# jkulhanek/viewformer

Hardware: AMD Instinct MI355X
Metric: novel views/sec (encode->AR transformer->decode), 128px 6-ctx (higher is better)
Workload: dtype bf16

## Files before the change

include/vf_hip.h:

```cpp
#ifndef VF_HIP_H
#define VF_HIP_H

#include <stddef.h>
#include <stdint.h>

#ifdef __cplusplus
extern "C" {
#endif

#define VF_OK 0
#define VF_ERR_BAD_ARG (-1)
#define VF_ERR_UNSUPPORTED (-2)

int vf_abi_version(void);
size_t vf_sizeof_igemm_args(void);
size_t vf_sizeof_pack_desc(void);
const char* vf_build_arch(void);
int vf_build_flags(void);
const char* vf_build_flag_name(int i);
enum { VF_SEL_ATTN_DMA = 0,
       VF_SEL_GEMM_G256 = 1,
       VF_SEL_LN_BWD_TWO_ROWS = 2,
       VF_SEL_ATTN_Q32 = 3,
       VF_SEL_CONV_X3H_K32 = 4,
       VF_SEL_GEMM_TAIL = 5,
       VF_SEL_COUNT = 6 };
int vf_select(int which, int value);
int vf_selected(int which);

enum { VF_MODE_GEMM = 0, VF_MODE_CONV3_S1 = 1, VF_MODE_CONV3_S2PAD = 2, VF_MODE_CONV3_UP2 = 3 };
enum { VF_EPI_NONE = 0, VF_EPI_GELU_ERF = 1,
       VF_EPI_GELU_BWD = 2,
       VF_EPI_GELU_DUAL = 3 };

typedef struct vf_igemm_args {
    const float* x;
    const float* w_packed;
    const float* bias;
    const float* res;
    float* out;
    const float* pro_mean;
    const float* pro_scale;
    const float* pro_beta;
    int32_t pro_swish;
    int32_t pro_rows_per_img;
    int32_t mode;
    int32_t epilogue;
    int32_t M;
    int32_t Cin, Cout;
    int32_t Hin, Win, Hout, Wout;
    int32_t lda, ldc, ldr;
    int32_t batch;
    int64_t stride_x, stride_w, stride_out, stride_res;
    float* gn_part;
    int32_t gn_slots;
    int32_t reserved0;
    void* out_aux;
    float drop_rate;
    uint32_t drop_seed, drop_site;
    int32_t drop_row0;
} vf_igemm_args;

size_t vf_igemm_packed_floats(int K, int N, int taps);
int vf_igemm_pack_f32(const float* src, float* dst, int K, int N, int taps,
                      int64_t sk, int64_t sn, int64_t st, int batch, int64_t src_bstride, void* stream);
int vf_igemm_f32(const vf_igemm_args* args , void* stream);

int vf_conv_in_u8_f32(const uint8_t* img_u8, const float* img_f32, const float* w_oihw, const float* bias,
                      float* out, int n_img, int H, int W, int Cout, void* stream);
size_t vf_conv_in_x3h_packed_elems(int Cout);
int vf_conv_in_x3h_pack(const float* w_oihw, void* dst, int Cout, void* stream);
int vf_conv_in_x3h(const uint8_t* img_u8, const float* img_f32, const void* w_packed, const float* bias, float* out, float* gn_part,
                   int gn_slots, int n_img, int H, int W, int Cout, void* stream);

int vf_conv3_small_cout_f32(const float* x, const float* w_oihw, const float* bias, const float* pro_mean,
                            const float* pro_scale, const float* pro_beta, int pro_swish, float* out, int n_img, int H, int W,
                            int Cin, int Cout, int x_bf16, void* stream);

size_t vf_groupnorm_workspace_bytes(int n_img, int HW, int C);
int vf_groupnorm_stats_f32(const float* x, const float* gamma, int n_img, int HW, int C, int groups, float eps,
                           float* mean_c, float* scale_c, void* ws, void* stream);
int vf_groupnorm_finalize_f32(const float* part, const float* gamma, int n_img, int HW, int C, int groups, int nslots,
                              float eps, float* mean_c, float* scale_c, void* stream);
int vf_groupnorm_apply_f32(const float* x, const float* mean_c, const float* scale_c, const float* beta,
                           float* out, int n_img, int HW, int C, int swish, void* stream);

size_t vf_vq_packed_floats(int D, int Kc);
int vf_vq_pack_codebook_f32(const float* E , float* dst, int D, int Kc, void* stream);
int vf_colsumsq_f32(const float* E , float* e_sq , int D, int Kc, void* stream);
int vf_vq_argmin_f32(const float* z, const float* E_packed, const float* e_sq, int64_t M, int D, int Kc,
                     int64_t* idx, void* stream);
size_t vf_vq_filter_packed_bytes(int D, int Kc);
int vf_vq_filter_pack(const float* E , void* dst, int D, int Kc, void* stream);
int vf_vq_argmin_filtered_f32(const float* z, const void* packed, int64_t M, int D, int Kc, int64_t* idx, uint32_t* stats4,
                              void* stream);
int vf_codebook_gather_f32(const float* E , const int64_t* idx, float* out ,
                           int64_t M, int D, int Kc, void* stream);

int vf_attn_blockcausal_f32(const float* q, const float* k, const float* v, float* out,
                            int B, int H, int T, int L, int ldq, int ldk, int ldv, int ldo,
                            float scale, int skip_masked, int twin_view, void* stream);
int vf_attn_blockcausal_bf16_v2(const void* q, const void* k, const void* v, int in_bf16, void* out, int out_bf16, int B, int H, int T, int L,
                                int ldq, int ldk, int ldv, int ldo, float scale, int skip_masked, int twin_view, void* stream);
int vf_attn_blockcausal_fp8(const void* q, const void* k, const void* v, int in_bf16, void* out, int out_bf16, int B, int H, int T, int L,
                            int ldq, int ldk, int ldv, int ldo, float scale, int skip_masked, int twin_view, void* stream);
int vf_attn_blockcausal_x6(const float* q, const float* k, const float* v, float* out,
                           int B, int H, int T, int L, int ldq, int ldk, int ldv, int ldo,
                           float scale, int skip_masked, int twin_view, void* stream);
int vf_attn_prefix_bf16(const void* q, const void* k, const void* v, const void* kp, const void* vp, int in_bf16, void* out, int out_bf16,
                        int B, int H, int C, int N, int L, int dh, int ldq, int ldk, int ldv, int ldkp, int ldvp, int64_t prefix_stride,
                        int ldo, void* stream);
int vf_attn_prefix_f32eq(const float* q, const float* k, const float* v, const float* kp, const float* vp, float* out,
                         int B, int H, int C, int N, int L, int dh, int ldq, int ldk, int ldv, int ldkp, int ldvp, int64_t prefix_stride,
                         int ldo, void* stream);
int vf_attn_spatial_f32(const float* qkv, float* out, int n_img, int HW, int C, int64_t ld, int64_t ldo, float scale, void* stream);
int vf_attn_spatial_x3h(const float* qkv, float* out, int n_img, int HW, int C, int64_t ld, int64_t ldo, float scale, void* stream);
int vf_softmax_rows_f32(float* x, int64_t rows, int n, float scale, void* stream);

int vf_layernorm_f32(const float* x, const float* gamma, const float* beta, float* out,
                     int64_t rows, int d, float eps, void* stream);
int vf_layernorm_bf16out_f32(const float* x, const float* gamma, const float* beta, void* out_bf16, int64_t rows, int d, float eps,
                             void* stream);
int vf_embed_sum_f32(const int32_t* ids, const float* wte, const float* wpe, const float* add,
                     float* out, int64_t BS, int L, int d, int vocab, void* stream);
int vf_dense_small_k_gelu_f32(const float* x, const float* W, const float* b, float* out,
                              int64_t rows, int K, int N, int gelu, void* stream);
int vf_argmax_rows_f32(const float* x, int64_t rows, int n, int ld, int64_t* idx, void* stream);
int vf_lmhead_argmax_bf16(const void* h, int h_bf16, int64_t ldh, const void* w_packed, int64_t M, int K, int N, int64_t* idx,
                          float* max_logit, void* stream);
int vf_lmhead_score_bf16(const void* h, int h_bf16, int64_t ldh, const void* w_packed, int64_t M, int K, int N, const int32_t* target,
                         int64_t* idx, float* max_logit, float* lse, float* target_logit, float* entropy, void* stream);
int vf_logits_score_f32(const float* logits, int64_t rows, int N, int64_t ld, const int32_t* target, int64_t* idx, float* max_logit,
                        float* lse, float* target_logit, float* entropy, void* stream);
int vf_score_views_f32(const float* target_logit, const float* lse, const float* max_logit, const int64_t* idx, const int32_t* target,
                       int64_t views, int L, float* token_log_prob, float* confidence, float* log_likelihood, float* accuracy, void* stream);
int vf_sample_rows_f32(const float* logits, int64_t rows, int N, int64_t ld, float temperature, int top_k, float top_p, uint32_t seed,
                       const int64_t* row_id, int S, int64_t* idx, float* logp, int32_t* kept, float* thr, void* stream);
int vf_sample_views_f32(const float* logp, int64_t views, int L, int S, float* log_likelihood, void* stream);
uint32_t vf_crc32c(const void* data, size_t n, uint32_t crc);
int vf_postprocess_u8(const float* x, uint8_t* out, int64_t n, void* stream);
int vf_resize_u8(const uint8_t* src, uint8_t* dst, int n_img, int Hin, int Win, int Hout, int Wout, int C, int bilinear, void* stream);
size_t vf_image_metrics_workspace_bytes(int n_img, int H, int W, int C);
int vf_image_metrics_u8(const uint8_t* a, const uint8_t* b, int n_img, int H, int W, int C, int64_t* sums, double* ssim, void* workspace,
                        void* stream);
size_t vf_camera_knn_workspace_bytes(int64_t N, int Q, int k);
int vf_camera_knn_f32(const float* db, int64_t N, const float* queries, int Q, int k, float pos_weight, int32_t* idx, float* dist,
                      void* workspace, void* stream);
int vf_pose_tail_f32(const float* x, int64_t ldx, const float* W, const float* b, float position_multiplier, int64_t views, int L, int K,
                     float* raw, float* tokens, float* cameras, void* stream);

size_t vf_gemm_bf16_packed_elems(int K, int N);
int vf_gemm_bf16_pack(const float* src, void* dst, int K, int N, int64_t sk, int64_t sn, int batch,
                      int64_t src_bstride, void* stream);
typedef struct vf_pack_desc {
    const float* src;
    void* dst;
    int32_t K, N;
    int64_t sk, sn;
} vf_pack_desc;
int vf_gemm_bf16_pack_multi(const vf_pack_desc* descs_device, int n, void* stream);
int vf_gemm_bf16(const vf_igemm_args* args , void* stream);
size_t vf_conv3_bf16_packed_elems(int Cin, int Cout);
int vf_conv3_bf16_pack(const float* w_oihw, void* dst, int Cin, int Cout, void* stream);
int vf_conv3_halo_bf16(const vf_igemm_args* args , void* stream);

int vf_conv3_halo_gn_slots(int Hout, int Wout);
size_t vf_conv3_x6_packed_elems(int Cin, int Cout);
int vf_conv3_x6_pack(const float* w_oihw, void* dst, int Cin, int Cout, void* stream);
int vf_conv3_halo_x6(const vf_igemm_args* args , void* stream);
size_t vf_conv3_x3h_packed_elems(int Cin, int Cout);
int vf_conv3_x3h_pack(const float* w_oihw, void* dst, int Cin, int Cout, void* stream);
int vf_conv3_halo_x3h(const vf_igemm_args* args , void* stream);
size_t vf_gemm_x3h_packed_elems(int K, int N);
int vf_gemm_x3h_pack(const float* src, void* dst, int K, int N, int64_t sk, int64_t sn, void* stream);
int vf_gemm_x3h(const vf_igemm_args* args , void* stream);
size_t vf_gemm_x6_packed_elems(int K, int N);
int vf_gemm_x6_pack(const float* src, void* dst, int K, int N, int64_t sk, int64_t sn, void* stream);
int vf_gemm_x6(const vf_igemm_args* args , void* stream);
int vf_sum_slabs_f32(const float* slabs, int nslabs, int64_t stride, int64_t n, float* dst, int accumulate, void* stream);

int vf_vq_ema_accumulate_f32(const float* z, const int64_t* idx, int64_t M, int D, int Kc, float* counts, float* embed_sum,
                             void* stream);
int vf_vq_ema_update_f32(const float* counts, const float* embed_sum, float* cluster_size_hidden, float* dw_hidden,
                         float* embeddings, int D, int Kc, float decay, float eps, float corr, void* stream);

int vf_gather_transpose_f32(const float* src, float* dst, int n_img, int Hin, int Win, int C, int Hout, int Wout, int stride, int oy,
                            int ox, int64_t ld_dst, void* stream);
size_t vf_conv3_wgrad_x6_rows(int Cin);
int vf_conv3_wgrad_x6(const float* x, const void* dy_packed, float* slabs, int n_img, int Hin, int Win, int Cin, int Hout, int Wout,
                      int Cout, int mode, int splits, void* stream);
int vf_upsample2_bwd_f32(const float* du, float* dx, int n_img, int H, int W, int C, void* stream);
size_t vf_groupnorm_bwd_workspace_bytes(int n_img, int HW, int C, int groups);
int vf_groupnorm_bwd_f32(const float* x, const float* da, const float* mean_c, const float* scale_c, const float* gamma,
                         const float* beta, float* dx, float* chan_sums, int n_img, int HW, int C, int groups, float eps, int swish,
                         int accumulate, void* ws, void* stream);
int vf_softmax_rows_bwd_f32(const float* p, float* dp, int64_t rows, int n, float scale, void* stream);
int vf_l1_loss_partials(int64_t n);
int vf_l1_loss_f32(const float* x, const float* y, float* dy, float* part, int64_t n, float grad_weight, void* stream);

int vf_lpips_scaling_f32(const float* x, float* y, int64_t npix, const float* shift3, const float* scale3, int backward, void* stream);
int vf_relu_f32(float* x, int64_t n, void* stream);
int vf_relu_bwd_f32(float* dy, const float* y, int64_t n, void* stream);
int vf_maxpool2_f32(const float* x, float* y, int n_img, int Hout, int Wout, int C, void* stream);
int vf_maxpool2_bwd_f32(const float* x, const float* dy, float* dx, int n_img, int Hout, int Wout, int C, void* stream);
int vf_lpips_head_blocks(int HW);
int vf_lpips_head_f32(const float* f0, const float* f1, const float* w, float* part, int n_img, int HW, int C, void* stream);
int vf_lpips_head_bwd_f32(const float* f0, const float* f1, const float* w, float* df1, int64_t npix, int C, float gscale,
                          int accumulate, void* stream);

int vf_attn_blockcausal_lse_f32(const float* q, const float* k, const float* v, float* out, float* lse,
                                int B, int H, int T, int L, int ldq, int ldk, int ldv, int ldo,
                                float scale, int skip_masked, int twin_view, float drop_rate, uint32_t drop_seed,
                                uint32_t drop_site, uint32_t drop_plane0, void* stream);
int vf_attn_bwd_prep_f32(const float* dout, const float* out, float* D, int B, int H, int T, int lddo, int ldo, void* stream);
int vf_attn_bwd_f32(const float* q, const float* k, const float* v, const float* dout, const float* lse, const float* D,
                    float* dq, float* dk, float* dv, int B, int H, int T, int L, int ldq, int ldk, int ldv, int lddo,
                    int lddq, int lddk, int lddv, float scale, int twin_view, float drop_rate, uint32_t drop_seed,
                    uint32_t drop_site, uint32_t drop_plane0, void* stream);
int vf_gemm_tn_bf16(const void* x_bf16, int ldx, const void* dy, int dy_is_bf16, int ldy, int M, int K, int N, int splits, float* w_slabs,
                    float* b_slabs, int64_t slab_stride, void* stream);
int vf_attn_blockcausal_bf16_lse(const void* q, const void* k, const void* v, void* out, float* lse, int B, int H, int T, int L,
                                 int ldq, int ldk, int ldv, int ldo, float scale, int twin_view, float drop_rate, uint32_t drop_seed,
                                 uint32_t drop_site, uint32_t drop_plane0, void* stream);
int vf_attn_bwd_prep_bf16(const void* dout, const void* out, float* D, int B, int H, int T, int lddo, int ldo, void* stream);
int vf_attn_bwd_bf16(const void* q, const void* k, const void* v, const void* dout, const float* lse, const float* D, void* dq, void* dk,
                     void* dv, int out_bf16 , int B, int H, int T, int L,
                     int ldq, int ldk, int ldv, int lddo, int lddq, int lddk, int lddv, float scale, int twin_view, float drop_rate,
                     uint32_t drop_seed, uint32_t drop_site, uint32_t drop_plane0, void* stream);
int vf_dropout_add_f32(const float* x, const float* res, float* out, int64_t rows, int cols, int64_t row0, float rate, uint32_t seed, uint32_t site,
                       void* stream);

int vf_transpose_f32(const float* src, float* dst, int rows, int cols, int64_t ld_src, int64_t ld_dst, int batch,
                     int64_t bs_src, int64_t bs_dst, void* stream);
int vf_transpose_bf16_f32(const void* src_bf16, float* dst, int rows, int cols, int64_t ld_src, int64_t ld_dst, int batch,
                          int64_t bs_src, int64_t bs_dst, void* stream);
size_t vf_colsum_workspace_bytes(int N);
int vf_colsum_f32(const float* x, float* out, int64_t M, int N, int64_t ld, int accumulate, void* ws, void* stream);
size_t vf_layernorm_bwd_workspace_bytes(int64_t rows, int d);
int vf_layernorm_bwd_f32(const float* dy, const float* x, const float* gamma, float* dx, float* dgamma, float* dbeta,
                         int64_t rows, int d, float eps, int accumulate, const float* res ,
                         void* dx_bf16 ,
                         float drop_rate, uint32_t drop_seed, uint32_t drop_site, int64_t drop_row0 , void* ws, void* stream);
int vf_gelu_f32(const float* u, float* f, int64_t n, void* stream);
int vf_gelu_bf16out_f32(const float* u, void* f_bf16, int64_t n, void* stream);
int vf_gelu_bwd_f32(const float* u, const float* df, float* du, int64_t n, void* stream);
int vf_gelu_bwd_bf16out_f32(const float* u, const float* df, void* du_bf16, int64_t n, void* stream);
int vf_softmax_mask_f32(float* s, int64_t batch, int T, int L, int mask_spec, float scale, void* stream);
int vf_softmax_mask_bwd_f32(const float* p, float* dp, int64_t batch, int T, int L, int mask_spec, float scale, void* stream);
int vf_softmax_ce_f32(const float* logits, const int32_t* target, const float* row_weight, float* loss, float* dlogits,
                      int64_t rows, int V, float label_smoothing, void* stream);
int vf_pose_mse_f32(const float* raw, const float* gt, const float* w_pos, const float* w_ori, const float* xyz_div, float* pos_loss,
                    float* ori_loss, float* draw, int64_t rows, int L, float position_multiplier, void* stream);
size_t vf_embed_bwd_workspace_bytes(int d, int vocab);
int vf_embed_bwd_f32(const float* dh, const int32_t* ids, float* dwte, float* dwpe, float* dadd, int64_t BS, int L, int d,
                     int vocab, void* workspace, void* stream);
int vf_dense_small_k_bwd_f32(const float* x, const float* dy, float* dW, float* db, int64_t rows, int K, int N, void* stream);
int vf_dense_small_n_f32(const float* x, const float* W, const float* b, float* out, int64_t rows, int K, int N, int64_t ldx, void* stream);
int vf_dense_small_n_wgrad_slabs(int64_t rows);
int vf_dense_small_n_wgrad_f32(const float* x, const float* dy, float* dW, float* ws, int64_t rows, int K, int N, int64_t ldx, int accumulate,
                               void* stream);
int vf_adamw_f32(float* param, const float* grad, float* m, float* v, int64_t n, float lr_decay, float lr_adam, float beta1,
                 float beta2, float eps, void* stream);
int vf_adamw_flat_f32(float* param, const float* grad, float* m, float* v, int64_t n, const int64_t* nodecay_ranges, int nranges,
                      float lr_decay, float lr_adam, float beta1, float beta2, float eps, void* stream);
typedef struct vf_adamw_pack_desc {
    int64_t offset;
    void* dst_kn;
    void* dst_nk;
    int32_t rows, cols;
    int32_t nodecay;
    int32_t reserved;
} vf_adamw_pack_desc;
size_t vf_sizeof_adamw_pack_desc(void);
int vf_adamw_pack_check(const vf_adamw_pack_desc* descs_host, int ndesc, int64_t n);
int vf_adamw_flat_pack_f32(float* param, const float* grad, float* m, float* v, int64_t n, const int64_t* nodecay_ranges, int nranges,
                           float lr_decay, float lr_adam, float beta1, float beta2, float eps, const vf_adamw_pack_desc* descs_device, int ndesc,
                           void* stream);
int vf_add_inplace_f32(float* a, const float* b, int64_t n, void* stream);
int vf_axpby_f32(float a, const float* x, float b, const float* y, float* out, int64_t n, void* stream);
int vf_clip_scratch_floats(void);
int vf_clip_by_norm_f32(float* x, int64_t n, float clip, float* scratch, void* stream);
int vf_clip_grad_norm_f32(float* x, int64_t n, float max_norm, float* scratch, void* stream);

#ifdef __cplusplus
}
#endif
#endif
```

viewformer_amd/_lib.py:

```python
import ctypes
import os
from ctypes import c_int, c_int32, c_int64, c_float, c_void_p, c_size_t, c_char_p, POINTER

HERE = os.path.dirname(os.path.abspath(__file__))
LIB_PATH = os.environ.get('VF_HIP_LIB') or os.path.join(HERE, 'libvf_hip.so')


class VfIgemmArgs(ctypes.Structure):
    _fields_ = [
        ('x', c_void_p), ('w_packed', c_void_p), ('bias', c_void_p), ('res', c_void_p), ('out', c_void_p),
        ('pro_mean', c_void_p), ('pro_scale', c_void_p), ('pro_beta', c_void_p),
        ('pro_swish', c_int32), ('pro_rows_per_img', c_int32), ('mode', c_int32), ('epilogue', c_int32),
        ('M', c_int32), ('Cin', c_int32), ('Cout', c_int32),
        ('Hin', c_int32), ('Win', c_int32), ('Hout', c_int32), ('Wout', c_int32),
        ('lda', c_int32), ('ldc', c_int32), ('ldr', c_int32), ('batch', c_int32),
        ('stride_x', c_int64), ('stride_w', c_int64), ('stride_out', c_int64), ('stride_res', c_int64),
        ('gn_part', c_void_p), ('gn_slots', c_int32), ('reserved0', c_int32),
        ('out_aux', c_void_p),
        ('drop_rate', c_float), ('drop_seed', ctypes.c_uint32), ('drop_site', ctypes.c_uint32), ('drop_row0', c_int32),
    ]


SEL_ATTN_DMA, SEL_GEMM_G256, SEL_LN_BWD_TWO_ROWS, SEL_ATTN_Q32 = 0, 1, 2, 3
SEL_CONV_X3H_K32 = 4
SEL_GEMM_TAIL = 5
_ENV_SELECT = {'VF_ATTN_DMA': SEL_ATTN_DMA, 'VF_GEMM_G256': SEL_GEMM_G256, 'VF_LN_BWD_TWO_ROWS': SEL_LN_BWD_TWO_ROWS, 'VF_ATTN_Q32': SEL_ATTN_Q32,
               'VF_CONV_X3H_K32': SEL_CONV_X3H_K32, 'VF_GEMM_TAIL': SEL_GEMM_TAIL}

ADAMW_PACK_DESC_BYTES = 40
PACK_DESC_BYTES = 40
P = c_void_p
EXPORTS = {
    'vf_abi_version': (c_int, []),
    'vf_sizeof_igemm_args': (c_size_t, []),
    'vf_sizeof_pack_desc': (c_size_t, []),
    'vf_build_arch': (c_char_p, []),
    'vf_build_flags': (c_int, []),
    'vf_build_flag_name': (c_char_p, [c_int]),
    'vf_select': (c_int, [c_int, c_int]),
    'vf_selected': (c_int, [c_int]),
    'vf_igemm_packed_floats': (c_size_t, [c_int, c_int, c_int]),
    'vf_igemm_pack_f32': (c_int, [P, P, c_int, c_int, c_int, c_int64, c_int64, c_int64, c_int, c_int64, P]),
    'vf_igemm_f32': (c_int, [POINTER(VfIgemmArgs), P]),
    'vf_conv_in_u8_f32': (c_int, [P, P, P, P, P, c_int, c_int, c_int, c_int, P]),
    'vf_conv_in_x3h_packed_elems': (c_size_t, [c_int]),
    'vf_conv_in_x3h_pack': (c_int, [P, P, c_int, P]),
    'vf_conv_in_x3h': (c_int, [P, P, P, P, P, P, c_int, c_int, c_int, c_int, c_int, P]),
    'vf_crc32c': (ctypes.c_uint32, [P, c_size_t, ctypes.c_uint32]),
    'vf_conv3_small_cout_f32': (c_int, [P, P, P, P, P, P, c_int, P, c_int, c_int, c_int, c_int, c_int, c_int, P]),
    'vf_groupnorm_workspace_bytes': (c_size_t, [c_int, c_int, c_int]),
    'vf_groupnorm_stats_f32': (c_int, [P, P, c_int, c_int, c_int, c_int, c_float, P, P, P, P]),
    'vf_groupnorm_finalize_f32': (c_int, [P, P, c_int, c_int, c_int, c_int, c_int, c_float, P, P, P]),
    'vf_conv3_halo_gn_slots': (c_int, [c_int, c_int]),
    'vf_groupnorm_apply_f32': (c_int, [P, P, P, P, P, c_int, c_int, c_int, c_int, P]),
    'vf_vq_packed_floats': (c_size_t, [c_int, c_int]),
    'vf_vq_pack_codebook_f32': (c_int, [P, P, c_int, c_int, P]),
    'vf_colsumsq_f32': (c_int, [P, P, c_int, c_int, P]),
    'vf_vq_argmin_f32': (c_int, [P, P, P, c_int64, c_int, c_int, P, P]),
    'vf_vq_filter_packed_bytes': (c_size_t, [c_int, c_int]),
    'vf_vq_filter_pack': (c_int, [P, P, c_int, c_int, P]),
    'vf_vq_argmin_filtered_f32': (c_int, [P, P, c_int64, c_int, c_int, P, P, P]),
    'vf_gather_transpose_f32': (c_int, [P, P, c_int, c_int, c_int, c_int, c_int, c_int, c_int, c_int, c_int, c_int64, P]),
    'vf_upsample2_bwd_f32': (c_int, [P, P, c_int, c_int, c_int, c_int, P]),
    'vf_groupnorm_bwd_workspace_bytes': (c_size_t, [c_int, c_int, c_int, c_int]),
    'vf_groupnorm_bwd_f32': (c_int, [P, P, P, P, P, P, P, P, c_int, c_int, c_int, c_int, c_float, c_int, c_int, P, P]),
    'vf_softmax_rows_bwd_f32': (c_int, [P, P, c_int64, c_int, c_float, P]),
    'vf_l1_loss_partials': (c_int, [c_int64]),
    'vf_l1_loss_f32': (c_int, [P, P, P, P, c_int64, c_float, P]),
    'vf_conv3_wgrad_x6_rows': (c_size_t, [c_int]),
    'vf_conv3_wgrad_x6': (c_int, [P, P, P, c_int, c_int, c_int, c_int, c_int, c_int, c_int, c_int, c_int, P]),
    'vf_lpips_scaling_f32': (c_int, [P, P, c_int64, P, P, c_int, P]),
    'vf_relu_f32': (c_int, [P, c_int64, P]),
    'vf_relu_bwd_f32': (c_int, [P, P, c_int64, P]),
    'vf_maxpool2_f32': (c_int, [P, P, c_int, c_int, c_int, c_int, P]),
    'vf_maxpool2_bwd_f32': (c_int, [P, P, P, c_int, c_int, c_int, c_int, P]),
    'vf_lpips_head_blocks': (c_int, [c_int]),
    'vf_lpips_head_f32': (c_int, [P, P, P, P, c_int, c_int, c_int, P]),
    'vf_lpips_head_bwd_f32': (c_int, [P, P, P, P, c_int64, c_int, c_float, c_int, P]),
    'vf_vq_ema_accumulate_f32': (c_int, [P, P, c_int64, c_int, c_int, P, P, P]),
    'vf_vq_ema_update_f32': (c_int, [P, P, P, P, P, c_int, c_int, c_float, c_float, c_float, P]),
    'vf_codebook_gather_f32': (c_int, [P, P, P, c_int64, c_int, c_int, P]),
    'vf_attn_blockcausal_f32': (c_int, [P, P, P, P, c_int, c_int, c_int, c_int, c_int, c_int, c_int, c_int,
                                        c_float, c_int, c_int, P]),
    'vf_attn_blockcausal_bf16_v2': (c_int, [P, P, P, c_int, P, c_int] + [c_int] * 8 + [c_float, c_int, c_int, P]),
    'vf_attn_blockcausal_fp8': (c_int, [P, P, P, c_int, P, c_int] + [c_int] * 8 + [c_float, c_int, c_int, P]),
    'vf_attn_blockcausal_x6': (c_int, [P, P, P, P, c_int, c_int, c_int, c_int, c_int, c_int, c_int, c_int,
                                       c_float, c_int, c_int, P]),
    'vf_attn_prefix_bf16': (c_int, [P, P, P, P, P, c_int, P, c_int] + [c_int] * 11 + [c_int64, c_int, P]),
    'vf_attn_prefix_f32eq': (c_int, [P, P, P, P, P, P] + [c_int] * 11 + [c_int64, c_int, P]),
    'vf_attn_blockcausal_lse_f32': (c_int, [P, P, P, P, P, c_int, c_int, c_int, c_int, c_int, c_int, c_int, c_int,
                                            c_float, c_int, c_int, c_float, ctypes.c_uint32, ctypes.c_uint32, ctypes.c_uint32, P]),
    'vf_dropout_add_f32': (c_int, [P, P, P, c_int64, c_int, c_int64, c_float, ctypes.c_uint32, ctypes.c_uint32, P]),
    'vf_attn_bwd_prep_f32': (c_int, [P, P, P, c_int, c_int, c_int, c_int, c_int, P]),
    'vf_attn_bwd_f32': (c_int, [P, P, P, P, P, P, P, P, P, c_int, c_int, c_int, c_int, c_int, c_int, c_int, c_int, c_int,
                                c_int, c_int, c_float, c_int, c_float, ctypes.c_uint32, ctypes.c_uint32, ctypes.c_uint32, P]),
    'vf_gemm_tn_bf16': (c_int, [P, c_int, P, c_int, c_int, c_int, c_int, c_int, c_int, P, P, c_int64, P]),
    'vf_attn_blockcausal_bf16_lse': (c_int, [P, P, P, P, P, c_int, c_int, c_int, c_int, c_int, c_int, c_int, c_int, c_float, c_int,
                                             c_float, ctypes.c_uint32, ctypes.c_uint32, ctypes.c_uint32, P]),
    'vf_attn_bwd_prep_bf16': (c_int, [P, P, P, c_int, c_int, c_int, c_int, c_int, P]),
    'vf_attn_bwd_bf16': (c_int, [P, P, P, P, P, P, P, P, P, c_int, c_int, c_int, c_int, c_int, c_int, c_int, c_int, c_int, c_int, c_int, c_int,
                                 c_float, c_int, c_float, ctypes.c_uint32, ctypes.c_uint32, ctypes.c_uint32, P]),
    'vf_attn_spatial_f32': (c_int, [P, P, c_int, c_int, c_int, c_int64, c_int64, c_float, P]),
    'vf_attn_spatial_x3h': (c_int, [P, P, c_int, c_int, c_int, c_int64, c_int64, c_float, P]),
    'vf_softmax_rows_f32': (c_int, [P, c_int64, c_int, c_float, P]),
    'vf_layernorm_f32': (c_int, [P, P, P, P, c_int64, c_int, c_float, P]),
    'vf_layernorm_bf16out_f32': (c_int, [P, P, P, P, c_int64, c_int, c_float, P]),
    'vf_embed_sum_f32': (c_int, [P, P, P, P, P, c_int64, c_int, c_int, c_int, P]),
    'vf_dense_small_k_gelu_f32': (c_int, [P, P, P, P, c_int64, c_int, c_int, c_int, P]),
    'vf_lmhead_argmax_bf16': (c_int, [P, c_int, c_int64, P, c_int64, c_int, c_int, P, P, P]),
    'vf_lmhead_score_bf16': (c_int, [P, c_int, c_int64, P, c_int64, c_int, c_int, P, P, P, P, P, P, P]),
    'vf_logits_score_f32': (c_int, [P, c_int64, c_int, c_int64, P, P, P, P, P, P, P]),
    'vf_score_views_f32': (c_int, [P, P, P, P, P, c_int64, c_int, P, P, P, P, P]),
    'vf_sample_rows_f32': (c_int, [P, c_int64, c_int, c_int64, c_float, c_int, c_float, ctypes.c_uint32, P, c_int, P, P, P, P, P]),
    'vf_sample_views_f32': (c_int, [P, c_int64, c_int, c_int, P, P]),
    'vf_argmax_rows_f32': (c_int, [P, c_int64, c_int, c_int, P, P]),
    'vf_postprocess_u8': (c_int, [P, P, c_int64, P]),
    'vf_resize_u8': (c_int, [P, P, c_int, c_int, c_int, c_int, c_int, c_int, c_int, P]),
    'vf_image_metrics_workspace_bytes': (c_size_t, [c_int, c_int, c_int, c_int]),
    'vf_image_metrics_u8': (c_int, [P, P, c_int, c_int, c_int, c_int, P, P, P, P]),
    'vf_camera_knn_workspace_bytes': (c_size_t, [c_int64, c_int, c_int]),
    'vf_camera_knn_f32': (c_int, [P, c_int64, P, c_int, c_int, c_float, P, P, P, P]),
    'vf_pose_tail_f32': (c_int, [P, c_int64, P, P, c_float, c_int64, c_int, c_int, P, P, P, P]),
    'vf_gemm_bf16_packed_elems': (c_size_t, [c_int, c_int]),
    'vf_gemm_bf16_pack': (c_int, [P, P, c_int, c_int, c_int64, c_int64, c_int, c_int64, P]),
    'vf_gemm_bf16_pack_multi': (c_int, [P, c_int, P]),
    'vf_gemm_bf16': (c_int, [POINTER(VfIgemmArgs), P]),
    'vf_conv3_bf16_packed_elems': (c_size_t, [c_int, c_int]),
    'vf_conv3_bf16_pack': (c_int, [P, P, c_int, c_int, P]),
    'vf_conv3_halo_bf16': (c_int, [POINTER(VfIgemmArgs), P]),
    'vf_conv3_x6_packed_elems': (c_size_t, [c_int, c_int]),
    'vf_conv3_x6_pack': (c_int, [P, P, c_int, c_int, P]),
    'vf_conv3_halo_x6': (c_int, [POINTER(VfIgemmArgs), P]),
    'vf_conv3_x3h_packed_elems': (c_size_t, [c_int, c_int]),
    'vf_conv3_x3h_pack': (c_int, [P, P, c_int, c_int, P]),
    'vf_conv3_halo_x3h': (c_int, [POINTER(VfIgemmArgs), P]),
    'vf_gemm_x3h_packed_elems': (c_size_t, [c_int, c_int]),
    'vf_gemm_x3h_pack': (c_int, [P, P, c_int, c_int, c_int64, c_int64, P]),
    'vf_gemm_x3h': (c_int, [POINTER(VfIgemmArgs), P]),
    'vf_gemm_x6_packed_elems': (c_size_t, [c_int, c_int]),
    'vf_gemm_x6_pack': (c_int, [P, P, c_int, c_int, c_int64, c_int64, P]),
    'vf_gemm_x6': (c_int, [POINTER(VfIgemmArgs), P]),
    'vf_sum_slabs_f32': (c_int, [P, c_int, c_int64, c_int64, P, c_int, P]),
    'vf_transpose_f32': (c_int, [P, P, c_int, c_int, c_int64, c_int64, c_int, c_int64, c_int64, P]),
    'vf_transpose_bf16_f32': (c_int, [P, P, c_int, c_int, c_int64, c_int64, c_int, c_int64, c_int64, P]),
    'vf_colsum_workspace_bytes': (c_size_t, [c_int]),
    'vf_colsum_f32': (c_int, [P, P, c_int64, c_int, c_int64, c_int, P, P]),
    'vf_layernorm_bwd_workspace_bytes': (c_size_t, [c_int64, c_int]),
    'vf_layernorm_bwd_f32': (c_int, [P, P, P, P, P, P, c_int64, c_int, c_float, c_int, P, P, c_float, ctypes.c_uint32, ctypes.c_uint32, c_int64, P, P]),
    'vf_gelu_f32': (c_int, [P, P, c_int64, P]),
    'vf_gelu_bf16out_f32': (c_int, [P, P, c_int64, P]),
    'vf_gelu_bwd_bf16out_f32': (c_int, [P, P, P, c_int64, P]),
    'vf_gelu_bwd_f32': (c_int, [P, P, P, c_int64, P]),
    'vf_softmax_mask_f32': (c_int, [P, c_int64, c_int, c_int, c_int, c_float, P]),
    'vf_softmax_mask_bwd_f32': (c_int, [P, P, c_int64, c_int, c_int, c_int, c_float, P]),
    'vf_softmax_ce_f32': (c_int, [P, P, P, P, P, c_int64, c_int, c_float, P]),
    'vf_pose_mse_f32': (c_int, [P, P, P, P, P, P, P, P, c_int64, c_int, c_float, P]),
    'vf_embed_bwd_workspace_bytes': (c_size_t, [c_int, c_int]),
    'vf_embed_bwd_f32': (c_int, [P, P, P, P, P, c_int64, c_int, c_int, c_int, P, P]),
    'vf_dense_small_k_bwd_f32': (c_int, [P, P, P, P, c_int64, c_int, c_int, P]),
    'vf_dense_small_n_f32': (c_int, [P, P, P, P, c_int64, c_int, c_int, c_int64, P]),
    'vf_dense_small_n_wgrad_slabs': (c_int, [c_int64]),
    'vf_dense_small_n_wgrad_f32': (c_int, [P, P, P, P, c_int64, c_int, c_int, c_int64, c_int, P]),
    'vf_adamw_f32': (c_int, [P, P, P, P, c_int64, c_float, c_float, c_float, c_float, c_float, P]),
    'vf_adamw_flat_f32': (c_int, [P, P, P, P, c_int64, P, c_int, c_float, c_float, c_float, c_float, c_float, P]),
    'vf_sizeof_adamw_pack_desc': (c_size_t, []),
    'vf_adamw_pack_check': (c_int, [P, c_int, c_int64]),
    'vf_adamw_flat_pack_f32': (c_int, [P, P, P, P, c_int64, P, c_int, c_float, c_float, c_float, c_float, c_float, P, c_int, P]),
    'vf_axpby_f32': (c_int, [c_float, P, c_float, P, P, c_int64, P]),
    'vf_add_inplace_f32': (c_int, [P, P, c_int64, P]),
    'vf_clip_scratch_floats': (c_int, []),
    'vf_clip_by_norm_f32': (c_int, [P, c_int64, c_float, P, P]),
    'vf_clip_grad_norm_f32': (c_int, [P, c_int64, c_float, P, P]),
}

_lib = None


class VfError(RuntimeError):
    pass


def _bind(path):
    lib = ctypes.CDLL(path)
    for name, (res, args) in EXPORTS.items():
        fn = getattr(lib, name)
        fn.restype = res
        fn.argtypes = args
    return lib


def load_variant(path):
    return _bind(os.path.abspath(path))


class use:

    def __init__(self, handle):
        self.handle = handle

    def __enter__(self):
        global _lib
        load()
        self.prev, _lib = _lib, self.handle
        return self.handle

    def __exit__(self, *exc):
        global _lib
        _lib = self.prev
        return False


def load():
    global _lib
    if _lib is not None:
        return _lib
    if not os.path.exists(LIB_PATH):
        raise VfError(f'{LIB_PATH} not found — run `python -m viewformer_amd.build` (hipcc --offload-arch=gfx950). '
                      'There is no CPU/PyTorch fallback for the hot path.')
    lib = _bind(LIB_PATH)
    if int(lib.vf_sizeof_igemm_args()) != ctypes.sizeof(VfIgemmArgs):
        raise VfError(f'vf_igemm_args is {int(lib.vf_sizeof_igemm_args())} bytes in {LIB_PATH} and {ctypes.sizeof(VfIgemmArgs)} in '
                      'viewformer_amd/_lib.py: rebuild the library or update the mirror')
    if int(lib.vf_sizeof_pack_desc()) != PACK_DESC_BYTES:
        raise VfError(f'vf_pack_desc is {int(lib.vf_sizeof_pack_desc())} bytes in {LIB_PATH}, {PACK_DESC_BYTES} expected')
    if int(lib.vf_sizeof_adamw_pack_desc()) != ADAMW_PACK_DESC_BYTES:
        raise VfError(f'vf_adamw_pack_desc is {int(lib.vf_sizeof_adamw_pack_desc())} bytes in {LIB_PATH}, {ADAMW_PACK_DESC_BYTES} expected')
    for env, which in _ENV_SELECT.items():
        if os.environ.get(env) in ('0', '1'):
            lib.vf_select(which, int(os.environ[env]))
    _lib = lib
    return lib


def select(which, value):
    prev = load().vf_select(int(which), 1 if value else 0)
    if prev < 0:
        raise VfError(f'vf_select({which}, {value}): bad argument')
    return prev


def check(status: int, what: str):
    if status == 0:
        return
    if status < 0:
        msg = {-1: 'bad argument', -2: 'unsupported shape'}.get(status, 'error')
        raise VfError(f'{what}: {msg} ({status})')
    raise VfError(f'{what}: HIP error {status}')
```

viewformer_amd/csrc/conv3_halo_x3h.hip:

```cpp
#include <type_traits>
#include "halo_common.h"

namespace {

typedef _Float16 f16x8 __attribute__((ext_vector_type(8)));
typedef _Float16 f16x4 __attribute__((ext_vector_type(4)));

typedef unsigned u32x4_t __attribute__((ext_vector_type(4)));
__device__ __forceinline__ f16x8 wbuf_load(__amdgpu_buffer_rsrc_t r, unsigned voff, unsigned soff) {
    return __builtin_bit_cast(f16x8, __builtin_amdgcn_raw_buffer_load_b128(r, voff, soff, 0));
}

constexpr int CK = 32;
constexpr int P_LDB = 144;
constexpr int TH = 8, TW = 16;
constexpr int BN = 128;
constexpr int PLANE_BYTES = 2 * BN * 16;
constexpr int KS_BYTES = 2 * PLANE_BYTES;
constexpr int TAP_BYTES = 2 * KS_BYTES;
constexpr int TAIL_BYTES = 16;

template <bool UP2, bool PAIR = false>
struct Geo {
    static constexpr int PH = UP2 ? (TH / 2 + 2) : (TH + 2);
    static constexpr int PW = PAIR ? 20 : (UP2 ? (TW / 2 + 2) : (TW + 2));
    static constexpr int NPIX = PH * PW;
    static constexpr int SLOTS = (NPIX * 8 + 255) / 256;
    static constexpr int BUF = (NPIX + 1) * P_LDB;
};

__device__ __forceinline__ void split2(float x, _Float16& h, _Float16& l) {
    h = (_Float16)x;
    l = (_Float16)((x - (float)h) * 2048.f);
}

template <bool UP2, bool PRO, bool SWISH, bool PAIR = false>
__global__ __launch_bounds__(256, 2) void conv3_halo_x3h_kernel(vf_igemm_args p) {
    using G = Geo<UP2, PAIR>;
    extern __shared__ __attribute__((aligned(16))) unsigned char smem_h[];

    const int tid = threadIdx.x;
    const int lane = tid & 63;
    const int wave = __builtin_amdgcn_readfirstlane(tid >> 6);
    constexpr int MI = 4, NJ = 1;
    const int wave_m = 0, wave_n = wave;
    const int half = lane >> 5, l31 = lane & 31;

    const int nb = p.Cout / BN;
    const int tilesX = p.Wout / TW, tilesY = p.Hout / TH;
    int bid = (int)vf_xcd_bid();
    const int nblk = bid % nb; bid /= nb;
    int tx = 0, ty = 0, img;
    if (PAIR) { img = bid * 2; }
    else { tx = bid % tilesX; bid /= tilesX; ty = bid % tilesY; img = bid / tilesY; }
    const int n_img_total = p.M / (p.Hout * p.Wout);
    const int img1 = PAIR ? min(img + 1, n_img_total - 1) : img;
    const int pair_pix = (img1 - img) * p.Hin * p.Win;
    const int y0 = ty * TH, x0 = tx * TW;
    const int sy0 = UP2 ? (y0 / 2 - 1) : (y0 - 1);
    const int sx0 = UP2 ? (x0 / 2 - 1) : (x0 - 1);

    const float* __restrict__ X = p.x + (size_t)img * p.Hin * p.Win * p.Cin;
    const int nchunks = p.Cin / CK;
    const int last_stage = nchunks * 9 - 1;

    const int c4 = tid & 7;
    int s_off[G::SLOTS];
    unsigned ok_mask = 0, sel_mask = 0;
    const int lds0 = (tid >> 3) * P_LDB + c4 * 8;
    int lds_last = 0;
#pragma unroll
    for (int q = 0; q < G::SLOTS; ++q) {
        const int pix = (tid >> 3) + 32 * q;
        const int pixc = pix < G::NPIX ? pix : G::NPIX;
        const int pr = pixc / G::PW, pc0 = pixc - pr * G::PW;
        const int sel = PAIR ? (pc0 >= 10) : 0;
        const int pc = pc0 - 10 * sel;
        sel_mask |= (unsigned)sel << q;
        const int sy = sy0 + pr, sx = sx0 + pc;
        const bool ok = pix < G::NPIX && sy >= 0 && sy < p.Hin && sx >= 0 && sx < p.Win;
        ok_mask |= (unsigned)ok << q;
        s_off[q] = ok ? (sel * pair_pix + sy * p.Win + sx) * p.Cin + c4 * 4 : c4 * 4;
        if (q == G::SLOTS - 1) lds_last = pixc * P_LDB + c4 * 8;
    }

    f32x4 preg[G::SLOTS];
    f32x4 pmean, pscale, pbeta, pmean1, pscale1;
    const __amdgpu_buffer_rsrc_t x_rs = __builtin_amdgcn_make_buffer_rsrc(const_cast<float*>(X), 0, 0x7fffffff, 0x00020000);
    auto patch_load = [&](int chunk) {
#pragma unroll
        for (int q = 0; q < G::SLOTS; ++q)
            preg[q] = __builtin_bit_cast(f32x4, __builtin_amdgcn_raw_buffer_load_b128(x_rs, (unsigned)s_off[q] * 4u, (unsigned)(chunk * CK * 4), 0));
        if (PRO) {
            pmean = *reinterpret_cast<const f32x4*>(p.pro_mean + (size_t)img * p.Cin + chunk * CK + c4 * 4);
            pscale = *reinterpret_cast<const f32x4*>(p.pro_scale + (size_t)img * p.Cin + chunk * CK + c4 * 4);
            pbeta = *reinterpret_cast<const f32x4*>(p.pro_beta + chunk * CK + c4 * 4);
            if (PAIR) {
                pmean1 = *reinterpret_cast<const f32x4*>(p.pro_mean + (size_t)img1 * p.Cin + chunk * CK + c4 * 4);
                pscale1 = *reinterpret_cast<const f32x4*>(p.pro_scale + (size_t)img1 * p.Cin + chunk * CK + c4 * 4);
            }
        }
    };
    auto patch_store_slot = [&](int buf, int q) {
        unsigned char* dst = smem_h + buf * G::BUF + (q == G::SLOTS - 1 ? lds_last : lds0 + q * 32 * P_LDB);
        f16x4 oh, ol;
#pragma unroll
        for (int e = 0; e < 4; ++e) {
            float t = preg[q][e];
            if (PRO) {
                const float mu = (PAIR && ((sel_mask >> q) & 1u)) ? pmean1[e] : pmean[e];
                const float sc = (PAIR && ((sel_mask >> q) & 1u)) ? pscale1[e] : pscale[e];
                t = (t - mu) * sc + pbeta[e];
                if (SWISH) t = vf_swish_1ulp(t);
            }
            _Float16 h, l;
            split2(((ok_mask >> q) & 1u) ? t : 0.f, h, l);
            oh[e] = h; ol[e] = l;
        }
        *reinterpret_cast<f16x4*>(dst) = oh;
        *reinterpret_cast<f16x4*>(dst + 64) = ol;
    };

    const int trow = vf_perm_row(l31), tpx = vf_perm_px(l31);
    int a_base[MI], a_r[MI];
#pragma unroll
    for (int mi = 0; mi < MI; ++mi) {
        const int a0 = wave_m * 4 + mi * 2 + trow;
        a_r[mi] = a0;
        const int tcol = PAIR ? (tpx >> 3) * 10 + (tpx & 7) : tpx;
        a_base[mi] = (a0 * G::PW + tcol) * P_LDB + half * 16;
    }

    const unsigned char* __restrict__ Wb = reinterpret_cast<const unsigned char*>(p.w_packed) + (size_t)nblk * TAP_BYTES;
    const size_t tap_stride = (size_t)nb * TAP_BYTES;
    const int b_lane = (half * BN + wave_n * (32 * NJ) + l31) * 16;
    constexpr int BD = 2, RING = BD + 1;
    static_assert(18 % RING == 0, "ring indices must repeat per chunk");
    f16x8 bring[RING][2][NJ];
    f16x8 aring[2][MI][2];
    const int last_g = nchunks * 18 - 1;
    const __amdgpu_buffer_rsrc_t w_rs = __builtin_amdgcn_make_buffer_rsrc(const_cast<unsigned char*>(Wb), 0, 0x7fffffff, 0x00020000);
    auto b_load = [&](f16x8 (&dst)[2][NJ], int g) {
        g = min(g, last_g);
        const unsigned soff = (unsigned)((size_t)(g >> 1) * tap_stride + (g & 1) * KS_BYTES);
#pragma unroll
        for (int pl = 0; pl < 2; ++pl)
#pragma unroll
            for (int j = 0; j < NJ; ++j) dst[pl][j] = wbuf_load(w_rs, (unsigned)(b_lane + pl * PLANE_BYTES + j * 32 * 16), soff);
    };
    auto a_load = [&](f16x8 (&dst)[MI][2], const unsigned char* patch, int s) {
        const int tap = s >> 1, ks = s & 1;
        const int dy = tap / 3, dx = tap % 3;
#pragma unroll
        for (int mi = 0; mi < MI; ++mi) {
            int aoff;
            if (UP2) {
                const int pr = (a_r[mi] + dy + 1) >> 1, pc = (tpx + dx + 1) >> 1;
                aoff = (pr * G::PW + pc) * P_LDB + half * 16;
            } else {
                aoff = a_base[mi] + (dy * G::PW + dx) * P_LDB;
            }
#pragma unroll
            for (int pl = 0; pl < 2; ++pl) dst[mi][pl] = *reinterpret_cast<const f16x8*>(patch + aoff + pl * 64 + ks * 32);
        }
    };

    f32x16 acc[MI][NJ], accx[MI][NJ];
#pragma unroll
    for (int i = 0; i < MI; ++i)
#pragma unroll
        for (int j = 0; j < NJ; ++j)
#pragma unroll
            for (int r = 0; r < 16; ++r) { acc[i][j][r] = 0.f; accx[i][j][r] = 0.f; }

    patch_load(0);
#pragma unroll
    for (int g = 0; g < BD; ++g) b_load(bring[g], g);
#pragma unroll
    for (int q = 0; q < G::SLOTS; ++q) patch_store_slot(0, q);
    __syncthreads();

    for (int chunk = 0; chunk < nchunks; ++chunk) {
        const unsigned char* patch = smem_h + (chunk & 1) * G::BUF;
        b_load(bring[BD % RING], chunk * 18 + BD);
        const bool more = UP2 || PAIR || chunk + 1 < nchunks;
        if (more) patch_load(min(chunk + 1, nchunks - 1));
        a_load(aring[0], patch, 0);
#pragma unroll
        for (int s = 0; s < 18; ++s) {
            if (s > 0) b_load(bring[(s + BD) % RING], chunk * 18 + s + BD);
            if (s + 1 < 18) a_load(aring[(s + 1) & 1], patch, s + 1);
#pragma unroll
            for (int t = 0; t < 3; ++t) {
#pragma unroll
                for (int mi = 0; mi < MI; ++mi)
#pragma unroll
                    for (int j = 0; j < NJ; ++j) {
                        if (t == 0) accx[mi][j] = __builtin_amdgcn_mfma_f32_32x32x16_f16(aring[s & 1][mi][1], bring[s % RING][0][j], accx[mi][j], 0, 0, 0);
                        else if (t == 1) accx[mi][j] = __builtin_amdgcn_mfma_f32_32x32x16_f16(aring[s & 1][mi][0], bring[s % RING][1][j], accx[mi][j], 0, 0, 0);
                        else acc[mi][j] = __builtin_amdgcn_mfma_f32_32x32x16_f16(aring[s & 1][mi][0], bring[s % RING][0][j], acc[mi][j], 0, 0, 0);
                    }
            }
            __builtin_amdgcn_sched_barrier(0);
            if ((s & 1) && (s >> 1) < G::SLOTS && more) patch_store_slot((chunk + 1) & 1, s >> 1);
        }
        __syncthreads();
    }

    const float inv_s = *reinterpret_cast<const float*>(reinterpret_cast<const unsigned char*>(p.w_packed) + (size_t)nchunks * 9 * nb * TAP_BYTES);
#pragma unroll
    for (int i = 0; i < MI; ++i)
#pragma unroll
        for (int j = 0; j < NJ; ++j)
#pragma unroll
            for (int r = 0; r < 16; ++r) acc[i][j][r] = __builtin_fmaf(accx[i][j][r], 4.8828125e-4f, acc[i][j][r]) * inv_s;
    vf_halo_epilogue_t<PAIR, MI, NJ>(p, acc, img, img1, y0, x0, PAIR ? 0 : (ty * tilesX + tx) * 2, nblk, wave_m, wave_n, half, l31);
}


constexpr int S2_PH = 2 * TH + 1, S2_PW = 2 * TW + 1;
constexpr int S2_NPIX = S2_PH * S2_PW;
constexpr int S2_LDB = 80;
constexpr int S2_SLOTS = (S2_NPIX * 4 + 255) / 256;
constexpr int S2_BUF = (S2_NPIX + 1) * S2_LDB;

template <bool P8>
__global__ __launch_bounds__(256, 2) void conv3_s2_x3h_kernel(vf_igemm_args p) {
    extern __shared__ __attribute__((aligned(16))) unsigned char smem_h[];
    constexpr int PW = P8 ? 34 : S2_PW;
    constexpr int NPIX = S2_PH * PW;
    constexpr int SLOTS = (NPIX * 4 + 255) / 256;
    const int tid = threadIdx.x;
    const int lane = tid & 63;
    const int wave = __builtin_amdgcn_readfirstlane(tid >> 6);
    constexpr int MI = 4, NJ = 1;
    const int wave_m = 0, wave_n = wave;
    const int half = lane >> 5, l31 = lane & 31;

    const int nb = p.Cout / BN;
    const int tilesX = P8 ? 1 : p.Wout / TW, tilesY = P8 ? 1 : p.Hout / TH;
    int bid = (int)vf_xcd_bid();
    const int nblk = bid % nb; bid /= nb;
    const int tx = bid % tilesX; bid /= tilesX;
    const int ty = bid % tilesY;
    const int img = P8 ? (bid / tilesY) * 2 : bid / tilesY;
    const int n_img_total = p.M / (p.Hout * p.Wout);
    const int img1 = P8 ? min(img + 1, n_img_total - 1) : img;
    const int pair_pix = (img1 - img) * p.Hin * p.Win;
    const int y0 = ty * TH, x0 = tx * TW;
    const float* __restrict__ X = p.x + (size_t)img * p.Hin * p.Win * p.Cin;
    const int nchunks = p.Cin / 16;

    const int c4 = tid & 3;
    int s_off[SLOTS], s_lds[SLOTS];
    bool s_ok[SLOTS];
#pragma unroll
    for (int q = 0; q < SLOTS; ++q) {
        const int pix = (tid >> 2) + 64 * q;
        const int pixc = pix < NPIX ? pix : 0;
        const int pr = pixc / PW, pc0 = pixc - pr * PW;
        const int sel = P8 ? (pc0 >= 17) : 0;
        const int pc = pc0 - 17 * sel;
        const int sy = 2 * y0 + pr, sx = 2 * x0 + pc;
        const bool ok = pix < NPIX && sy < p.Hin && sx < p.Win;
        s_ok[q] = ok;
        s_off[q] = ok ? (sel * pair_pix + sy * p.Win + sx) * p.Cin + c4 * 4 : c4 * 4;
        int slot;
        if (P8) slot = pr * PW + ((pc & 1) ? 18 + sel * 8 + (pc >> 1) : sel * 9 + (pc >> 1));
        else slot = pr * PW + (pc & 1) * (TW + 1) + (pc >> 1);
        s_lds[q] = (pix < NPIX ? slot : NPIX) * S2_LDB + c4 * 8;
    }
    f32x4 preg[SLOTS];
    auto patch_load = [&](int chunk) {
#pragma unroll
        for (int q = 0; q < SLOTS; ++q) preg[q] = *reinterpret_cast<const f32x4*>(X + chunk * 16 + s_off[q]);
    };
    auto patch_park = [&]() {
#pragma unroll
        for (int q = 0; q < SLOTS; ++q) {
            f16x4 oh, ol;
#pragma unroll
            for (int e = 0; e < 4; ++e) {
                _Float16 h, l;
                split2(s_ok[q] ? preg[q][e] : 0.f, h, l);
                oh[e] = h; ol[e] = l;
            }
            unsigned char* dst = smem_h + s_lds[q];
            *reinterpret_cast<f16x4*>(dst) = oh;
            *reinterpret_cast<f16x4*>(dst + 32) = ol;
        }
    };

    const int trow = vf_perm_row(l31), tpx = vf_perm_px(l31);
    int a_base[MI], a_base_o[MI];
#pragma unroll
    for (int mi = 0; mi < MI; ++mi) {
        const int row2 = 2 * (wave_m * 4 + mi * 2 + trow) * PW;
        if (P8) {
            a_base[mi] = (row2 + (tpx >> 3) * 9 + (tpx & 7)) * S2_LDB + half * 16;
            a_base_o[mi] = (row2 + 18 + (tpx >> 3) * 8 + (tpx & 7)) * S2_LDB + half * 16;
        } else {
            a_base[mi] = (row2 + tpx) * S2_LDB + half * 16;
            a_base_o[mi] = a_base[mi] + (TW + 1) * S2_LDB;
        }
    }

    const unsigned char* __restrict__ Wb = reinterpret_cast<const unsigned char*>(p.w_packed) + (size_t)nblk * TAP_BYTES;
    const size_t tap_stride = (size_t)nb * TAP_BYTES;
    const int b_lane = (half * BN + wave_n * (32 * NJ) + l31) * 16;
    const int last_g = nchunks * 9 - 1;
    constexpr int S2_BR = 3;
    f16x8 bring[S2_BR][2][NJ];
    f16x8 aring[2][MI][2];
    auto b_load = [&](f16x8 (&dst)[2][NJ], int g) {
        g = min(g, last_g);
        const int c = g / 9, tap = g - c * 9;
        const unsigned char* src = Wb + (size_t)((c >> 1) * 9 + tap) * tap_stride + (c & 1) * KS_BYTES + b_lane;
#pragma unroll
        for (int pl = 0; pl < 2; ++pl)
#pragma unroll
            for (int j = 0; j < NJ; ++j) dst[pl][j] = *reinterpret_cast<const f16x8*>(src + pl * PLANE_BYTES + j * 32 * 16);
    };
    auto a_load = [&](f16x8 (&dst)[MI][2], int tap) {
        const int dy = tap / 3, dx = tap % 3;
        const int off = (dy * PW + (dx >> 1)) * S2_LDB;
#pragma unroll
        for (int mi = 0; mi < MI; ++mi)
#pragma unroll
            for (int pl = 0; pl < 2; ++pl) dst[mi][pl] = *reinterpret_cast<const f16x8*>(smem_h + ((dx & 1) ? a_base_o[mi] : a_base[mi]) + off + pl * 32);
    };

    f32x16 acc[MI][NJ], accx[MI][NJ];
#pragma unroll
    for (int i = 0; i < MI; ++i)
#pragma unroll
        for (int j = 0; j < NJ; ++j)
#pragma unroll
            for (int r = 0; r < 16; ++r) { acc[i][j][r] = 0.f; accx[i][j][r] = 0.f; }

    patch_load(0);
    b_load(bring[0], 0);
    if (S2_BR > 2) b_load(bring[1], 1);
    for (int chunk = 0; chunk < nchunks; ++chunk) {
        __syncthreads();
        patch_park();
        b_load(bring[(S2_BR - 1) % S2_BR], chunk * 9 + S2_BR - 1);
        if (chunk + 1 < nchunks) patch_load(min(chunk + 1, nchunks - 1));
        __syncthreads();
        a_load(aring[0], 0);
#pragma unroll
        for (int t = 0; t < 9; ++t) {
            if (t > 0) b_load(bring[(t + S2_BR - 1) % S2_BR], chunk * 9 + t + S2_BR - 1);
            if (t + 1 < 9) a_load(aring[(t + 1) & 1], t + 1);
#pragma unroll
            for (int mi = 0; mi < MI; ++mi)
#pragma unroll
                for (int j = 0; j < NJ; ++j) accx[mi][j] = __builtin_amdgcn_mfma_f32_32x32x16_f16(aring[t & 1][mi][1], bring[t % S2_BR][0][j], accx[mi][j], 0, 0, 0);
#pragma unroll
            for (int mi = 0; mi < MI; ++mi)
#pragma unroll
                for (int j = 0; j < NJ; ++j) accx[mi][j] = __builtin_amdgcn_mfma_f32_32x32x16_f16(aring[t & 1][mi][0], bring[t % S2_BR][1][j], accx[mi][j], 0, 0, 0);
#pragma unroll
            for (int mi = 0; mi < MI; ++mi)
#pragma unroll
                for (int j = 0; j < NJ; ++j) acc[mi][j] = __builtin_amdgcn_mfma_f32_32x32x16_f16(aring[t & 1][mi][0], bring[t % S2_BR][0][j], acc[mi][j], 0, 0, 0);
            __builtin_amdgcn_sched_barrier(0);
        }
    }
    const float inv_s = *reinterpret_cast<const float*>(reinterpret_cast<const unsigned char*>(p.w_packed) + (size_t)(p.Cin / CK) * 9 * nb * TAP_BYTES);
#pragma unroll
    for (int i = 0; i < MI; ++i)
#pragma unroll
        for (int j = 0; j < NJ; ++j)
#pragma unroll
            for (int r = 0; r < 16; ++r) acc[i][j][r] = __builtin_fmaf(accx[i][j][r], 4.8828125e-4f, acc[i][j][r]) * inv_s;
    vf_halo_epilogue_t<P8, MI, NJ, false>(p, acc, img, img1, y0, x0, P8 ? 0 : (ty * tilesX + tx) * 2, nblk, wave_m, wave_n, half, l31);
}



typedef float f32x4v __attribute__((ext_vector_type(4)));

template <bool PRO, bool SWISH>
__global__ __launch_bounds__(256, 2) void conv3_halo_x3h16_kernel(vf_igemm_args p) {
    using G = Geo<false, false>;
    extern __shared__ __attribute__((aligned(16))) unsigned char smem_h[];
    constexpr int RT = 8, CT = 2;

    const int tid = threadIdx.x;
    const int lane = tid & 63;
    const int wave = __builtin_amdgcn_readfirstlane(tid >> 6);
    const int lm = lane & 15, lg = lane >> 4;

    const int nb = p.Cout / BN;
    const int tilesX = p.Wout / TW, tilesY = p.Hout / TH;
    int bid = (int)vf_xcd_bid();
    const int nblk = bid % nb; bid /= nb;
    const int tx = bid % tilesX; bid /= tilesX;
    const int ty = bid % tilesY;
    const int img = bid / tilesY;
    const int y0 = ty * TH, x0 = tx * TW;
    const int sy0 = y0 - 1, sx0 = x0 - 1;
    const float* __restrict__ X = p.x + (size_t)img * p.Hin * p.Win * p.Cin;
    const int nchunks = p.Cin / CK;

    const int c4 = tid & 7;
    unsigned ok_mask = 0;
    const int c4s = (((c4 >> 1) & 1) * 2 + (c4 >> 2)) * 16 + (c4 & 1) * 8;
    const int lds0 = (tid >> 3) * P_LDB + c4s;
    int lds_last = 0;
    int pix0 = tid >> 3;
    auto slot_src = [&](int q, bool& ok) {
        const int pix = pix0 + 32 * q;
        const int pixc = min(pix, (int)G::NPIX);
        const int pr = (pixc * 3641) >> 16, pc = pixc - pr * G::PW;
        const int sy = sy0 + pr, sx = sx0 + pc;
        ok = (pix < G::NPIX) & ((unsigned)sy < (unsigned)p.Hin) & ((unsigned)sx < (unsigned)p.Win);
        const int off = (sy * p.Win + sx) * p.Cin;
        return (ok ? off : 0) + c4 * 4;
    };
#pragma unroll
    for (int q = 0; q < G::SLOTS; ++q) {
        bool ok;
        (void)slot_src(q, ok);
        ok_mask |= (unsigned)ok << q;
        if (q == G::SLOTS - 1) { const int pix = (tid >> 3) + 32 * q; lds_last = (pix < G::NPIX ? pix : G::NPIX) * P_LDB + c4s; }
    }
    unsigned char* __restrict__ raw_l = smem_h + 2 * G::BUF;
    const __amdgpu_buffer_rsrc_t x_rs = __builtin_amdgcn_make_buffer_rsrc(const_cast<float*>(X), 0, 0x7fffffff, 0x00020000);
    float* __restrict__ pro_l = reinterpret_cast<float*>(smem_h + 2 * G::BUF + G::SLOTS * 4096 - 1024);
    if (PRO) {
        for (int i = tid; i < p.Cin; i += 256) {
            pro_l[i] = p.pro_mean[(size_t)img * p.Cin + i];
            pro_l[p.Cin + i] = p.pro_scale[(size_t)img * p.Cin + i];
            pro_l[2 * p.Cin + i] = p.pro_beta[i];
        }
    }
    int pro_chunk = 0;
    auto patch_load = [&](int chunk) {
        asm volatile("" : "+v"(pix0));
#pragma unroll
        for (int q = 0; q < G::SLOTS; ++q) {
            bool ok;
            const int off = slot_src(q, ok);
            if (q == G::SLOTS - 1 && wave == 3) continue;
            __builtin_amdgcn_raw_ptr_buffer_load_lds(x_rs, (__attribute__((address_space(3))) void*)(raw_l + q * 4096 + wave * 1024), 16, (unsigned)off * 4u,
                                                     (unsigned)(chunk * CK * 4), 0, 0);
        }
        pro_chunk = chunk;
    };
    auto patch_store_slot = [&](int buf, int q) {
        unsigned char* dst = smem_h + buf * G::BUF + (q == G::SLOTS - 1 ? lds_last : lds0 + q * 32 * P_LDB);
        f32x4 pmean, pscale, pbeta;
        if (PRO) {
            const float* pl = pro_l + pro_chunk * CK + c4 * 4;
            pmean = *reinterpret_cast<const f32x4*>(pl);
            pscale = *reinterpret_cast<const f32x4*>(pl + p.Cin);
            pbeta = *reinterpret_cast<const f32x4*>(pl + 2 * p.Cin);
        }
        f32x4 raw = {0.f, 0.f, 0.f, 0.f};
        if (!(q == G::SLOTS - 1 && wave == 3)) raw = *reinterpret_cast<const f32x4*>(raw_l + q * 4096 + tid * 16);
        f16x4 oh, ol;
#pragma unroll
        for (int e = 0; e < 4; ++e) {
            float t = raw[e];
            if (PRO) {
                t = (t - pmean[e]) * pscale[e] + pbeta[e];
                if (SWISH) t = vf_swish_1ulp(t);
            }
            _Float16 h, l;
            split2(((ok_mask >> q) & 1u) ? t : 0.f, h, l);
            oh[e] = h; ol[e] = l;
        }
        *reinterpret_cast<f16x4*>(dst) = oh;
        *reinterpret_cast<f16x4*>(dst + 64) = ol;
    };

    const int lpix = lm < 4 ? 2 * lm : lm < 12 ? 2 * lm - 7 : 2 * lm - 16;
    const int a_lane = lpix * P_LDB + (((lg & 1) * 2) + (lg >> 1)) * 16;
    const unsigned char* __restrict__ Wb = reinterpret_cast<const unsigned char*>(p.w_packed) + (size_t)nblk * TAP_BYTES;
    const size_t tap_stride = (size_t)nb * TAP_BYTES;
    const int b_lane = ((lg >> 1) * 4 + (lg & 1)) * (BN * 16) + (wave * 32 + lm) * 16;
    const int last_tap = nchunks * 9 - 1;
    const __amdgpu_buffer_rsrc_t w_rs = __builtin_amdgcn_make_buffer_rsrc(const_cast<unsigned char*>(Wb), 0, 0x7fffffff, 0x00020000);
    f16x8 bring[2][4];
    constexpr int AR = 3;
    f16x8 aring[AR][2];
    auto b_load = [&](f16x8 (&dst)[4], int gtap) {
        const unsigned soff = (unsigned)((size_t)min(gtap, last_tap) * tap_stride);
#pragma unroll
        for (int pl = 0; pl < 2; ++pl)
#pragma unroll
            for (int ct = 0; ct < CT; ++ct) dst[pl * 2 + ct] = wbuf_load(w_rs, (unsigned)(b_lane + pl * PLANE_BYTES + ct * 256), soff);
    };
    auto a_load = [&](f16x8 (&dst)[2], const unsigned char* patch, int step) {
        const int tap = step >> 3, rt = step & 7;
        const int off = ((rt + tap / 3) * G::PW + tap % 3) * P_LDB;
        dst[0] = *reinterpret_cast<const f16x8*>(patch + a_lane + off);
        dst[1] = *reinterpret_cast<const f16x8*>(patch + a_lane + off + 64);
    };

    f32x4v acc[RT][CT], accx[RT][CT];
#pragma unroll
    for (int i = 0; i < RT; ++i)
#pragma unroll
        for (int j = 0; j < CT; ++j)
#pragma unroll
            for (int r = 0; r < 4; ++r) { acc[i][j][r] = 0.f; accx[i][j][r] = 0.f; }

    patch_load(0);
    b_load(bring[0], 0);
    asm volatile("s_waitcnt vmcnt(0)" ::: "memory");
    if (PRO) __syncthreads();
#pragma unroll
    for (int q = 0; q < G::SLOTS; ++q) patch_store_slot(0, q);
    __syncthreads();

    auto chunk_body = [&](int chunk, auto parity) {
        constexpr int P0 = decltype(parity)::value;
        const unsigned char* patch = smem_h + P0 * G::BUF;
        const bool more = chunk + 1 < nchunks;
        b_load(bring[(P0 + 1) & 1], chunk * 9 + 1);
        unsigned pad[G::SLOTS];
#pragma unroll
        for (int q = 0; q < G::SLOTS; ++q) pad[q] = __builtin_amdgcn_raw_buffer_load_b32(w_rs, (unsigned)(q * 256), 0u, 0);
        if (more) patch_load(chunk + 1);
#pragma unroll
        for (int i = 0; i < AR - 1; ++i) a_load(aring[i], patch, i);
#pragma unroll
        for (int t = 0; t < 9; ++t) {
            if (t > 0) b_load(bring[(P0 + t + 1) & 1], chunk * 9 + t + 1);
            if (t == 2) {
#pragma unroll
                for (int q = 0; q < G::SLOTS; ++q) asm volatile("" :: "v"(pad[q]));
            }
            const f16x8 (&B)[4] = bring[(P0 + t) & 1];
#pragma unroll
            for (int rt = 0; rt < RT; ++rt) {
                const int step = t * 8 + rt;
                if (step + AR - 1 < 72) a_load(aring[(step + AR - 1) % AR], patch, step + AR - 1);
                const f16x8 ah = aring[step % AR][0], al = aring[step % AR][1];
                accx[rt][0] = __builtin_amdgcn_mfma_f32_16x16x32_f16(al, B[0], accx[rt][0], 0, 0, 0);
                accx[rt][1] = __builtin_amdgcn_mfma_f32_16x16x32_f16(al, B[1], accx[rt][1], 0, 0, 0);
                acc[rt][0] = __builtin_amdgcn_mfma_f32_16x16x32_f16(ah, B[0], acc[rt][0], 0, 0, 0);
                acc[rt][1] = __builtin_amdgcn_mfma_f32_16x16x32_f16(ah, B[1], acc[rt][1], 0, 0, 0);
                accx[rt][0] = __builtin_amdgcn_mfma_f32_16x16x32_f16(ah, B[2], accx[rt][0], 0, 0, 0);
                accx[rt][1] = __builtin_amdgcn_mfma_f32_16x16x32_f16(ah, B[3], accx[rt][1], 0, 0, 0);
                __builtin_amdgcn_sched_barrier(0);
            }
            if (t >= 1 && t <= G::SLOTS && more) {
                if (t == 1) asm volatile("s_waitcnt vmcnt(8)" ::: "memory");
                patch_store_slot((P0 + 1) & 1, t - 1);
            }
        }
        __syncthreads();
    };
    for (int chunk = 0; chunk < nchunks; chunk += 2) {
        chunk_body(chunk, std::integral_constant<int, 0>{});
        chunk_body(chunk + 1, std::integral_constant<int, 1>{});
    }

    const float inv_s = *reinterpret_cast<const float*>(reinterpret_cast<const unsigned char*>(p.w_packed) + (size_t)nchunks * 9 * nb * TAP_BYTES);
    const __amdgpu_buffer_rsrc_t o_rs = __builtin_amdgcn_make_buffer_rsrc(p.out + (size_t)img * p.Hout * p.Wout * p.ldc, 0, 0x7fffffff, 0x00020000);
    const __amdgpu_buffer_rsrc_t r_rs = __builtin_amdgcn_make_buffer_rsrc(const_cast<float*>(p.res ? p.res + (size_t)img * p.Hout * p.Wout * p.ldr : p.out), 0, 0x7fffffff, 0x00020000);
    const bool Res = p.res != nullptr;
    const bool stats = p.gn_part != nullptr;
    const int cg = p.Cout >> 5;
    const int tile_slot = (ty * tilesX + tx) * 2;
    const int pbase = lg == 0 ? 0 : lg == 1 ? 1 : lg == 2 ? 9 : 8;
    auto spix = [&](int rt, int r) { return (y0 + rt) * p.Wout + x0 + 2 * r; };
#pragma unroll
    for (int rt = 0; rt < RT; ++rt)
#pragma unroll
        for (int ct = 0; ct < CT; ++ct)
#pragma unroll
            for (int r = 0; r < 4; ++r) acc[rt][ct][r] = __builtin_fmaf(accx[rt][ct][r], 4.8828125e-4f, acc[rt][ct][r]) * inv_s;
    __builtin_amdgcn_sched_barrier(0);
    float rr[CT][RT][4];
    if (Res) {
#pragma unroll
        for (int ct = 0; ct < CT; ++ct) {
            const int n = nblk * BN + wave * 32 + ct * 16 + lm;
            const unsigned rv = (unsigned)(pbase * p.ldr + n) * 4u;
#pragma unroll
            for (int rt = 0; rt < RT; ++rt)
#pragma unroll
                for (int r = 0; r < 4; ++r)
                    rr[ct][rt][r] = __builtin_bit_cast(float, __builtin_amdgcn_raw_buffer_load_b32(r_rs, rv, (unsigned)(spix(rt, r) * p.ldr) * 4u, 0));
        }
    }
#pragma unroll
    for (int ct = 0; ct < CT; ++ct) {
        const int n = nblk * BN + wave * 32 + ct * 16 + lm;
        const float bias = p.bias ? p.bias[n] : 0.f;
        const unsigned ov = (unsigned)(pbase * p.ldc + n) * 4u;
#pragma unroll
        for (int sl = 0; sl < 2; ++sl) {
            float s32 = 0.f, q32 = 0.f;
#pragma unroll
            for (int k = 0; k < 4; ++k) {
                const int rt = sl * 4 + k;
#pragma unroll
                for (int r = 0; r < 4; ++r) {
                    float v = acc[rt][ct][r] + bias;
                    if (Res) v += rr[ct][rt][r];
                    __builtin_amdgcn_raw_buffer_store_b32(__builtin_bit_cast(unsigned, v), o_rs, ov, (unsigned)(spix(rt, r) * p.ldc) * 4u, 0);
                    s32 += v;
                    q32 = __builtin_fmaf(v, v, q32);
                }
            }
            if (stats) {
                vf_gn_acc_t s = (vf_gn_acc_t)s32, q = (vf_gn_acc_t)q32;
                for (int o = 1; o < cg; o <<= 1) { s += __shfl_xor(s, o, 64); q += __shfl_xor(q, o, 64); }
                s += __shfl_xor(s, 16, 64); q += __shfl_xor(q, 16, 64);
                s += __shfl_xor(s, 32, 64); q += __shfl_xor(q, 32, 64);
                if (lg == 0 && (lm & (cg - 1)) == 0) {
                    float* dst = p.gn_part + ((((size_t)img * p.gn_slots) + tile_slot + sl) * 32 + n / cg) * 2;
                    dst[0] = (float)s;
                    dst[1] = (float)q;
                }
            }
        }
    }
}

__global__ void absmax_kernel(const float* __restrict__ w, long long n, unsigned* __restrict__ out) {
    float m = 0.f;
    for (long long i = blockIdx.x * (long long)blockDim.x + threadIdx.x; i < n; i += (long long)gridDim.x * blockDim.x) m = fmaxf(m, fabsf(w[i]));
    vf_block_max_atomic(m, out);
}

__global__ void pack_conv_x3h_kernel(const float* __restrict__ w, _Float16* __restrict__ dst, int Cin, int Cout, int nb, int nchunks,
                                     unsigned char* __restrict__ tail) {
    const float amax = __uint_as_float(*reinterpret_cast<const unsigned*>(tail + 4));
    const int ex = amax > 0.f ? ilogbf(amax) : 13;
    const float S = ldexpf(1.f, 13 - ex);
    if (blockIdx.x == 0 && threadIdx.x == 0) *reinterpret_cast<float*>(tail) = ldexpf(1.f, ex - 13);
    const long long total = (long long)nchunks * 9 * nb * CK * BN;
    for (long long idx = blockIdx.x * (long long)blockDim.x + threadIdx.x; idx < total; idx += (long long)gridDim.x * blockDim.x) {
        const int e = (int)(idx & 7);
        long long t = idx >> 3;
        const int nl = (int)(t % BN); t /= BN;
        const int half = (int)(t & 1);
        const int ks = (int)((t >> 1) & 1);
        t >>= 2;
        const int nblk = (int)(t % nb); t /= nb;
        const int tap = (int)(t % 9);
        const int chunk = (int)(t / 9);
        const int c = chunk * CK + ks * 16 + half * 8 + e;
        const int n = nblk * BN + nl;
        float v = 0.f;
        if (c < Cin && n < Cout) v = w[((size_t)n * Cin + c) * 9 + tap] * S;
        _Float16 h, l;
        split2(v, h, l);
        const size_t base = ((((size_t)(chunk * 9 + tap) * nb + nblk) * 2 + ks) * 2) * (2 * BN * 8) + ((size_t)half * BN + nl) * 8 + e;
        dst[base] = h;
        dst[base + 2 * BN * 8] = l;
    }
}

template <bool UP2, bool PRO, bool SWISH, bool PAIR>
int launch_halo(const vf_igemm_args& a, hipStream_t stream) {
    using G = Geo<UP2, PAIR>;
    const size_t smem = (size_t)2 * G::BUF;
    const int n_img = a.M / (a.Hout * a.Wout);
    const long long blocks = PAIR ? (long long)((n_img + 1) / 2) * (a.Cout / BN)
                                  : (long long)n_img * (a.Hout / TH) * (a.Wout / TW) * (a.Cout / BN);
    hipLaunchKernelGGL((conv3_halo_x3h_kernel<UP2, PRO, SWISH, PAIR>), dim3((unsigned)blocks), dim3(256), smem, stream, a);
    return vf_last_status();
}

static inline size_t vf_x3h16_lds_bytes(int pro_cin) { return (size_t)2 * Geo<false, false>::BUF + Geo<false, false>::SLOTS * 4096 - 1024 + (size_t)3 * pro_cin * 4; }

template <bool PRO, bool SWISH>
int launch_halo16(const vf_igemm_args& a, hipStream_t stream) {
    using G = Geo<false, false>;
    const int n_img = a.M / (a.Hout * a.Wout);
    const long long blocks = (long long)n_img * (a.Hout / TH) * (a.Wout / TW) * (a.Cout / BN);
    const size_t smem = vf_x3h16_lds_bytes(PRO ? a.Cin : 0);
    static unsigned long long attr_devs = 0;
    if (vf_attr_needed(&attr_devs)) {
        const hipError_t e = hipFuncSetAttribute(reinterpret_cast<const void*>(conv3_halo_x3h16_kernel<PRO, SWISH>), hipFuncAttributeMaxDynamicSharedMemorySize, 80 * 1024);
        if (e != hipSuccess) return (int)e;
        vf_attr_done(&attr_devs);
    }
    hipLaunchKernelGGL((conv3_halo_x3h16_kernel<PRO, SWISH>), dim3((unsigned)blocks), dim3(256), smem, stream, a);
    return vf_last_status();
}

template <bool UP2, bool PAIR>
int dispatch_pro(const vf_igemm_args& a, hipStream_t s) {
    if (!UP2 && !PAIR && (a.Cin / CK) % 2 == 0 && (!a.gn_part || a.Cout / 32 <= 16) && vf_x3h16_lds_bytes(a.pro_mean ? a.Cin : 0) <= 80 * 1024 &&
        vf_selected(VF_SEL_CONV_X3H_K32)) {
        if (!a.pro_mean) return launch_halo16<false, false>(a, s);
        return a.pro_swish ? launch_halo16<true, true>(a, s) : launch_halo16<true, false>(a, s);
    }
    if (!a.pro_mean) return launch_halo<UP2, false, false, PAIR>(a, s);
    return a.pro_swish ? launch_halo<UP2, true, true, PAIR>(a, s) : launch_halo<UP2, true, false, PAIR>(a, s);
}

}

extern "C" {

size_t vf_conv3_x3h_packed_elems(int Cin, int Cout) {
    if (Cin <= 0 || Cout <= 0) return 0;
    return (size_t)((Cin + CK - 1) / CK) * 9 * ((Cout + BN - 1) / BN) * CK * BN * 2 + TAIL_BYTES / 2;
}

int vf_conv3_x3h_pack(const float* w_oihw, void* dst, int Cin, int Cout, void* stream) {
    if (!w_oihw || !dst || Cin <= 0 || Cout <= 0) return VF_ERR_BAD_ARG;
    const int nb = (Cout + BN - 1) / BN, nchunks = (Cin + CK - 1) / CK;
    const long long total = (long long)nchunks * 9 * nb * CK * BN;
    unsigned char* tail = reinterpret_cast<unsigned char*>(dst) + (size_t)total * 2 * sizeof(_Float16);
    hipStream_t s = (hipStream_t)stream;
    if (hipMemsetAsync(tail, 0, TAIL_BYTES, s) != hipSuccess) return vf_last_status();
    const long long nw = (long long)Cout * Cin * 9;
    hipLaunchKernelGGL(absmax_kernel, dim3((unsigned)((nw + 2047) / 2048 > 128 ? 128 : (nw + 2047) / 2048)), dim3(256), 0, s, w_oihw, nw,
                       reinterpret_cast<unsigned*>(tail + 4));
    const int blocks = (int)((total + 255) / 256 > 4096 ? 4096 : (total + 255) / 256);
    hipLaunchKernelGGL(pack_conv_x3h_kernel, dim3(blocks), dim3(256), 0, s, w_oihw, (_Float16*)dst, Cin, Cout, nb, nchunks, tail);
    return vf_last_status();
}

int vf_conv3_halo_x3h(const vf_igemm_args* args, void* stream) {
    if (!args) return VF_ERR_BAD_ARG;
    const vf_igemm_args& a = *args;
    if (!a.x || !a.w_packed || !a.out || a.M <= 0) return VF_ERR_BAD_ARG;
    if (a.drop_rate != 0.f || a.out_aux) return VF_ERR_UNSUPPORTED;
    if (a.mode == VF_MODE_CONV3_S2PAD) {
        const bool p8 = a.Hout == 8 && a.Wout == 8;
        if (a.Cout % BN != 0 || a.Cin % CK != 0 || (!p8 && (a.Hout % TH != 0 || a.Wout % TW != 0)) || a.pro_mean) return VF_ERR_UNSUPPORTED;
        if (a.Hin != a.Hout * 2 || a.Win != a.Wout * 2 || a.M % (a.Hout * a.Wout) != 0) return VF_ERR_BAD_ARG;
        if (a.batch > 1 || a.epilogue != VF_EPI_NONE || a.ldc < a.Cout || (a.res && a.ldr < a.Cout)) return VF_ERR_BAD_ARG;
        if ((long long)a.Hin * a.Win * a.Cin >= (1ll << 31)) return VF_ERR_UNSUPPORTED;
        if (int st = vf_halo_gn_check(a)) return st;
        if (p8) {
            const long long blocks = (long long)((a.M / 64 + 1) / 2) * (a.Cout / BN);
            hipLaunchKernelGGL(conv3_s2_x3h_kernel<true>, dim3((unsigned)blocks), dim3(256), (size_t)(S2_PH * 34 + 1) * S2_LDB, (hipStream_t)stream, a);
            return vf_last_status();
        }
        const long long blocks = (long long)(a.M / (a.Hout * a.Wout)) * (a.Hout / TH) * (a.Wout / TW) * (a.Cout / BN);
        hipLaunchKernelGGL(conv3_s2_x3h_kernel<false>, dim3((unsigned)blocks), dim3(256), (size_t)S2_BUF, (hipStream_t)stream, a);
        return vf_last_status();
    }
    if (a.mode != VF_MODE_CONV3_S1 && a.mode != VF_MODE_CONV3_UP2) return VF_ERR_UNSUPPORTED;
    const bool pair = a.mode == VF_MODE_CONV3_S1 && a.Hout == 8 && a.Wout == 8;
    if (a.Cout % BN != 0 || a.Cin % CK != 0 || (!pair && (a.Hout % TH != 0 || a.Wout % TW != 0))) return VF_ERR_UNSUPPORTED;
    if (a.Hin <= 0 || a.Win <= 0 || a.M % (a.Hout * a.Wout) != 0) return VF_ERR_BAD_ARG;
    if (a.mode == VF_MODE_CONV3_S1 && (a.Hout != a.Hin || a.Wout != a.Win)) return VF_ERR_BAD_ARG;
    if (a.mode == VF_MODE_CONV3_UP2 && (a.Hout != a.Hin * 2 || a.Wout != a.Win * 2)) return VF_ERR_BAD_ARG;
    if (a.batch > 1 || a.epilogue != VF_EPI_NONE || a.ldc < a.Cout || (a.res && a.ldr < a.Cout)) return VF_ERR_BAD_ARG;
    if ((a.pro_mean || a.pro_scale || a.pro_beta) && !(a.pro_mean && a.pro_scale && a.pro_beta)) return VF_ERR_BAD_ARG;
    if ((long long)a.Hin * a.Win * a.Cin >= (1ll << 31)) return VF_ERR_UNSUPPORTED;
    if (int st = vf_halo_gn_check(a)) return st;
    hipStream_t s = (hipStream_t)stream;
    if (pair) return dispatch_pro<false, true>(a, s);
    return (a.mode == VF_MODE_CONV3_UP2) ? dispatch_pro<true, false>(a, s) : dispatch_pro<false, false>(a, s);
}

}
```

viewformer_amd/csrc/gemm_bf16.hip:

```cpp
#include "vf_common.h"
#include "epilogue.h"
#include "../../include/vf_hip.h"

namespace {

typedef __bf16 bf16x8 __attribute__((ext_vector_type(8)));
typedef __bf16 bf16x4 __attribute__((ext_vector_type(4)));

constexpr int CK = 64;
constexpr int BM = 128, BN = 128;
constexpr int A_LDB = 144;
constexpr int A_BYTES = BM * A_LDB;
constexpr int B_BYTES = CK * BN * 2;

__global__ __launch_bounds__(256, 2) void gemm_bf16_kernel(vf_igemm_args p) {
    extern __shared__ __attribute__((aligned(16))) unsigned char smem_b[];
    unsigned char* As = smem_b;
    unsigned char* Bs = smem_b + 2 * A_BYTES;

    const int tid = threadIdx.x;
    const int lane = tid & 63;
    const int wave = __builtin_amdgcn_readfirstlane(tid >> 6);
    const int wave_m = wave >> 1, wave_n = wave & 1;
    const int half = lane >> 5, l31 = lane & 31;

    const int nb = (p.Cout + BN - 1) / BN;
    const unsigned lbid = vf_xcd_bid();
    const int nblk = lbid % nb;
    const int mtile = lbid / nb;
    const int bz = blockIdx.z;
    const float* __restrict__ X = p.x + (size_t)bz * p.stride_x;
    const unsigned char* __restrict__ Wp = reinterpret_cast<const unsigned char*>(p.w_packed) + (size_t)bz * p.stride_w * 2
                                           + (size_t)nblk * B_BYTES;
    const size_t stage_stride = (size_t)nb * B_BYTES;
    const int nstages = p.Cin / CK;

    const int a_c4 = tid & 15, a_r0 = tid >> 4;
    const float* arow[8];
#pragma unroll
    for (int q = 0; q < 8; ++q) {
        int m = mtile * BM + a_r0 + 16 * q;
        m = m < p.M ? m : p.M - 1;
        arow[q] = X + (size_t)m * p.lda + a_c4 * 4;
    }
    f32x4 areg[8];
    f32x4 breg[4];
    auto load_stage = [&](int s) {
#pragma unroll
        for (int q = 0; q < 8; ++q) areg[q] = *reinterpret_cast<const f32x4*>(arow[q] + s * CK);
        const unsigned char* src = Wp + (size_t)s * stage_stride;
#pragma unroll
        for (int q = 0; q < 4; ++q) breg[q] = *reinterpret_cast<const f32x4*>(src + (size_t)(tid + 256 * q) * 16);
    };
    auto store_stage = [&](int buf) {
        unsigned char* a_dst = As + buf * A_BYTES;
#pragma unroll
        for (int q = 0; q < 8; ++q) {
            bf16x4 v;
#pragma unroll
            for (int e = 0; e < 4; ++e) v[e] = (__bf16)areg[q][e];
            *reinterpret_cast<bf16x4*>(a_dst + (a_r0 + 16 * q) * A_LDB + a_c4 * 8) = v;
        }
        unsigned char* b_dst = Bs + buf * B_BYTES;
#pragma unroll
        for (int q = 0; q < 4; ++q) *reinterpret_cast<f32x4*>(b_dst + (size_t)(tid + 256 * q) * 16) = breg[q];
    };

    f32x16 acc[2][2];
#pragma unroll
    for (int i = 0; i < 2; ++i)
#pragma unroll
        for (int j = 0; j < 2; ++j)
#pragma unroll
            for (int r = 0; r < 16; ++r) acc[i][j][r] = 0.f;

    load_stage(0);
    store_stage(0);
    __syncthreads();
    for (int s = 0; s < nstages; ++s) {
        load_stage(min(s + 1, nstages - 1));
        const unsigned char* a_src = As + (s & 1) * A_BYTES + (wave_m * 64 + l31) * A_LDB + half * 16;
        const unsigned char* b_src = Bs + (s & 1) * B_BYTES + (half * BN + wave_n * 64 + l31) * 16;
#pragma unroll
        for (int ks = 0; ks < 4; ++ks) {
            bf16x8 a[2], b[2];
#pragma unroll
            for (int i = 0; i < 2; ++i) a[i] = *reinterpret_cast<const bf16x8*>(a_src + i * 32 * A_LDB + ks * 32);
#pragma unroll
            for (int j = 0; j < 2; ++j) b[j] = *reinterpret_cast<const bf16x8*>(b_src + (ks * 2 * BN + j * 32) * 16);
#pragma unroll
            for (int i = 0; i < 2; ++i)
#pragma unroll
                for (int j = 0; j < 2; ++j)
                    acc[i][j] = __builtin_amdgcn_mfma_f32_32x32x16_bf16(a[i], b[j], acc[i][j], 0, 0, 0);
        }
        store_stage((s + 1) & 1);
        __syncthreads();
    }

    float* __restrict__ Out = p.out + (size_t)bz * p.stride_out;
    const float* __restrict__ Res = p.res ? p.res + (size_t)bz * p.stride_res : nullptr;
    const bool full = (mtile * BM + BM <= p.M) && (nblk * BN + BN <= p.Cout);
    const long long ldc = p.ldc, ldr = p.ldr;
    const bool gelu = p.epilogue == VF_EPI_GELU_ERF;
#pragma unroll
    for (int j = 0; j < 2; ++j) {
        const int n = nblk * BN + wave_n * 64 + j * 32 + l31;
        const bool nok = n < p.Cout;
        const float bias = (nok && p.bias) ? p.bias[n] : 0.f;
#pragma unroll
        for (int i = 0; i < 2; ++i) {
            const int m0 = mtile * BM + wave_m * 64 + i * 32 + 4 * half;
            const int nn = nok ? n : 0;
            float* o = Out + (size_t)(m0 < p.M ? m0 : 0) * ldc + nn;
            const float* rs = Res ? Res + (size_t)(m0 < p.M ? m0 : 0) * ldr + nn : nullptr;
            const int rows_left = nok ? p.M - m0 : 0;
            if (full) {
                auto oo = [&](int r) { return (long long)((r & 3) + 8 * (r >> 2)) * ldc; };
                auto ro = [&](int r) { return (long long)((r & 3) + 8 * (r >> 2)) * ldr; };
                if (gelu) {
                    if (Res) vf_store_tile<2, true>(acc[i][j], bias, o, rs, oo, ro);
                    else vf_store_tile<2, false>(acc[i][j], bias, o, rs, oo, ro);
                } else {
                    if (Res) vf_store_tile<0, true>(acc[i][j], bias, o, rs, oo, ro);
                    else vf_store_tile<0, false>(acc[i][j], bias, o, rs, oo, ro);
                }
            } else if (gelu) {
                if (Res) vf_store_tile_ragged<2, true>(acc[i][j], bias, o, rs, ldc, ldr, rows_left);
                else vf_store_tile_ragged<2, false>(acc[i][j], bias, o, rs, ldc, ldr, rows_left);
            } else {
                if (Res) vf_store_tile_ragged<0, true>(acc[i][j], bias, o, rs, ldc, ldr, rows_left);
                else vf_store_tile_ragged<0, false>(acc[i][j], bias, o, rs, ldc, ldr, rows_left);
            }
        }
    }
}

template <bool A16, bool O16>
__global__ __launch_bounds__(256, 2) void gemm_bf16_direct_kernel(vf_igemm_args p) {
    extern __shared__ __attribute__((aligned(16))) unsigned char smem_b[];
    unsigned char* As = smem_b;

    const int tid = threadIdx.x;
    const int lane = tid & 63;
    const int wave = __builtin_amdgcn_readfirstlane(tid >> 6);
    constexpr int MI = 2, NJ = 2;
    const int wave_m = wave >> 1, wave_n = wave & 1;
    const int half = lane >> 5, l31 = lane & 31;

    const int nb = (p.Cout + BN - 1) / BN;
    const unsigned lbid = vf_xcd_bid();
    const int nblk = lbid % nb;
    const int mtile = lbid / nb;
    const float* __restrict__ X = p.x;
    const unsigned char* __restrict__ Wp = reinterpret_cast<const unsigned char*>(p.w_packed) + (size_t)nblk * B_BYTES;
    const size_t stage_stride = (size_t)nb * B_BYTES;
    const int nstages = p.Cin / CK;

    const int a_c4 = A16 ? (tid & 7) : (tid & 15), a_r0 = A16 ? (tid >> 3) : (tid >> 4);
    constexpr int NQ = A16 ? 4 : 8, RSTEP = A16 ? 32 : 16;
    const float* arow[NQ];
#pragma unroll
    for (int q = 0; q < NQ; ++q) {
        int m = mtile * BM + a_r0 + RSTEP * q;
        m = m < p.M ? m : p.M - 1;
        arow[q] = A16 ? reinterpret_cast<const float*>(reinterpret_cast<const __bf16*>(X) + (size_t)m * p.lda + a_c4 * 8)
                      : X + (size_t)m * p.lda + a_c4 * 4;
    }
    f32x4 areg[NQ];
    auto a_fetch = [&](int s) {
#pragma unroll
        for (int q = 0; q < NQ; ++q)
            areg[q] = A16 ? *reinterpret_cast<const f32x4*>(reinterpret_cast<const __bf16*>(arow[q]) + s * CK)
                          : *reinterpret_cast<const f32x4*>(arow[q] + s * CK);
    };
    auto a_park = [&](int buf, int q) {
        if (A16) {
            if (q < NQ) *reinterpret_cast<f32x4*>(As + buf * A_BYTES + (a_r0 + RSTEP * q) * A_LDB + a_c4 * 16) = areg[q < NQ ? q : 0];
        } else {
            bf16x4 v;
#pragma unroll
            for (int e = 0; e < 4; ++e) v[e] = (__bf16)areg[q < NQ ? q : 0][e];
            *reinterpret_cast<bf16x4*>(As + buf * A_BYTES + (a_r0 + RSTEP * q) * A_LDB + a_c4 * 8) = v;
        }
    };
    const int b_lane = (half * BN + wave_n * (32 * NJ) + l31) * 16;
    bf16x8 bring[2][4][NJ];
    auto b_load = [&](bf16x8 (&dst)[4][NJ], int s) {
        const unsigned char* src = Wp + (size_t)min(s, nstages - 1) * stage_stride + b_lane;
#pragma unroll
        for (int ks = 0; ks < 4; ++ks)
#pragma unroll
            for (int j = 0; j < NJ; ++j) dst[ks][j] = *reinterpret_cast<const bf16x8*>(src + (ks * 2 * BN + j * 32) * 16);
    };

    f32x16 acc[MI][NJ];
#pragma unroll
    for (int i = 0; i < MI; ++i)
#pragma unroll
        for (int j = 0; j < NJ; ++j)
#pragma unroll
            for (int r = 0; r < 16; ++r) acc[i][j][r] = 0.f;

    a_fetch(0);
    b_load(bring[0], 0);
#pragma unroll
    for (int q = 0; q < NQ; ++q) a_park(0, q);
    __syncthreads();

    auto stage_body = [&](int s, bf16x8 (&bcur)[4][NJ], bf16x8 (&bnext)[4][NJ]) {
        const unsigned char* a_src = As + (s & 1) * A_BYTES + (wave_m * 64 + l31) * A_LDB + half * 16;
        a_fetch(min(s + 1, nstages - 1));
        b_load(bnext, s + 1);
        bf16x8 a[4][MI];
#pragma unroll
        for (int ks = 0; ks < 4; ++ks)
#pragma unroll
            for (int i = 0; i < MI; ++i) a[ks][i] = *reinterpret_cast<const bf16x8*>(a_src + i * 32 * A_LDB + ks * 32);
#pragma unroll
        for (int ks = 0; ks < 4; ++ks) {
#pragma unroll
            for (int i = 0; i < MI; ++i)
#pragma unroll
                for (int j = 0; j < NJ; ++j)
                    acc[i][j] = __builtin_amdgcn_mfma_f32_32x32x16_bf16(a[ks][i], bcur[ks][j], acc[i][j], 0, 0, 0);
            if (A16) a_park((s + 1) & 1, ks);
            else { a_park((s + 1) & 1, ks * 2); a_park((s + 1) & 1, ks * 2 + 1); }
        }
        __builtin_amdgcn_sched_barrier(0);
        __syncthreads();
    };
    for (int s = 0; s < nstages; s += 2) {
        stage_body(s, bring[0], bring[1]);
        stage_body(s + 1, bring[1], bring[0]);
    }

    if (O16) {
        typedef __bf16 bf16x2_t __attribute__((ext_vector_type(2)));
        const bool gelu16 = p.epilogue == VF_EPI_GELU_ERF;
        const bool gbwd = p.epilogue == VF_EPI_GELU_BWD;
        __bf16* __restrict__ O = reinterpret_cast<__bf16*>(p.out);
        const bool pairs = (p.ldc & 1) == 0 && (p.Cout & 1) == 0;
        const int odd = l31 & 1;
#pragma unroll
        for (int j = 0; j < NJ; ++j) {
            const int n = nblk * BN + wave_n * (32 * NJ) + j * 32 + l31;
            const float bias = (n < p.Cout && p.bias) ? p.bias[n] : 0.f;
#pragma unroll
            for (int i = 0; i < MI; ++i) {
                const int m0 = mtile * BM + wave_m * 64 + i * 32 + 4 * half;
                float t[16];
                if (gbwd) {
                    float uu[16];
#pragma unroll
                    for (int r = 0; r < 16; ++r) {
                        const int m = m0 + (r & 3) + 8 * (r >> 2);
                        uu[r] = p.res[(size_t)(m < p.M ? m : 0) * p.ldr + (n < p.Cout ? n : 0)];
                    }
#pragma unroll
                    for (int r = 0; r < 16; ++r) t[r] = __fmul_rn(__fadd_rn(acc[i][j][r], bias), vf_gelu_grad_fast(uu[r]));
                } else {
#pragma unroll
                    for (int r = 0; r < 16; ++r) {
                        t[r] = acc[i][j][r] + bias;
                        if (gelu16) t[r] = vf_gelu_erf_fast(t[r]);
                    }
                }
                if (pairs) {
#pragma unroll
                    for (int r = 0; r < 16; r += 2) {
                        const float give = odd ? t[r] : t[r + 1];
                        const float got = vf_lane_xor1(give);
                        const int m = m0 + ((r + odd) & 3) + 8 * ((r + odd) >> 2);
                        bf16x2_t v;
                        v[0] = (__bf16)(odd ? got : t[r]);
                        v[1] = (__bf16)(odd ? t[r + 1] : got);
                        const int n0 = n - odd;
                        if (m < p.M && n0 < p.Cout) *reinterpret_cast<bf16x2_t*>(O + (size_t)m * p.ldc + n0) = v;
                    }
                } else {
#pragma unroll
                    for (int r = 0; r < 16; ++r) {
                        const int m = m0 + (r & 3) + 8 * (r >> 2);
                        if (m < p.M && n < p.Cout) O[(size_t)m * p.ldc + n] = (__bf16)t[r];
                    }
                }
            }
        }
        return;
    }
    float* __restrict__ Out = p.out;
    const float* __restrict__ Res = p.res;
    const bool full = (mtile * BM + BM <= p.M) && (nblk * BN + BN <= p.Cout);
    const long long ldc = p.ldc, ldr = p.ldr;
    const bool gelu = p.epilogue == VF_EPI_GELU_ERF;
#pragma unroll
    for (int j = 0; j < NJ; ++j) {
        const int n = nblk * BN + wave_n * (32 * NJ) + j * 32 + l31;
        const bool nok = n < p.Cout;
        const float bias = (nok && p.bias) ? p.bias[n] : 0.f;
#pragma unroll
        for (int i = 0; i < MI; ++i) {
            const int m0 = mtile * BM + wave_m * 64 + i * 32 + 4 * half;
            const int nn = nok ? n : 0;
            float* o = Out + (size_t)(m0 < p.M ? m0 : 0) * ldc + nn;
            const float* rs = Res ? Res + (size_t)(m0 < p.M ? m0 : 0) * ldr + nn : nullptr;
            const int rows_left = nok ? p.M - m0 : 0;
            if (full) {
                auto oo = [&](int r) { return (long long)((r & 3) + 8 * (r >> 2)) * ldc; };
                auto ro = [&](int r) { return (long long)((r & 3) + 8 * (r >> 2)) * ldr; };
                if (gelu) {
                    if (Res) vf_store_tile<2, true>(acc[i][j], bias, o, rs, oo, ro);
                    else vf_store_tile<2, false>(acc[i][j], bias, o, rs, oo, ro);
                } else {
                    if (Res) vf_store_tile<0, true>(acc[i][j], bias, o, rs, oo, ro);
                    else vf_store_tile<0, false>(acc[i][j], bias, o, rs, oo, ro);
                }
            } else if (gelu) {
                if (Res) vf_store_tile_ragged<2, true>(acc[i][j], bias, o, rs, ldc, ldr, rows_left);
                else vf_store_tile_ragged<2, false>(acc[i][j], bias, o, rs, ldc, ldr, rows_left);
            } else {
                if (Res) vf_store_tile_ragged<0, true>(acc[i][j], bias, o, rs, ldc, ldr, rows_left);
                else vf_store_tile_ragged<0, false>(acc[i][j], bias, o, rs, ldc, ldr, rows_left);
            }
        }
    }
}

__global__ void pack_bf16_kernel(const float* __restrict__ src, __bf16* __restrict__ dst, int K, int N, long long sk,
                                 long long sn, int nb, int nchunks, long long src_bstride, long long dst_bstride) {
    const long long total = (long long)nchunks * nb * CK * BN;
    const int bz = blockIdx.y;
    for (long long idx = blockIdx.x * (long long)blockDim.x + threadIdx.x; idx < total; idx += (long long)gridDim.x * blockDim.x) {
        const int e = (int)(idx & 7);
        long long t = idx >> 3;
        const int nl = (int)(t % BN); t /= BN;
        const int half = (int)(t & 1);
        const int ks = (int)((t >> 1) & 3);
        t >>= 3;
        const int nblk = (int)(t % nb);
        const int chunk = (int)(t / nb);
        const int k = chunk * CK + ks * 16 + half * 8 + e;
        const int n = nblk * BN + nl;
        float v = 0.f;
        if (k < K && n < N) v = src[(size_t)bz * src_bstride + k * sk + n * sn];
        dst[(size_t)bz * dst_bstride + idx] = (__bf16)v;
    }
}

__global__ void pack_bf16_multi_kernel(const vf_pack_desc* __restrict__ descs) {
    const vf_pack_desc d = descs[blockIdx.y];
    const int nb = (d.N + BN - 1) / BN, nchunks = (d.K + CK - 1) / CK;
    const long long groups = (long long)nchunks * nb * (CK * BN / 8);
    __bf16* __restrict__ dst = reinterpret_cast<__bf16*>(d.dst);
    typedef __bf16 bf16x8_t __attribute__((ext_vector_type(8)));
    for (long long gi = blockIdx.x * (long long)blockDim.x + threadIdx.x; gi < groups; gi += (long long)gridDim.x * blockDim.x) {
        long long t = gi;
        const int nl = (int)(t % BN); t /= BN;
        const int half = (int)(t & 1);
        const int ks = (int)((t >> 1) & 3);
        t >>= 3;
        const int nblk = (int)(t % nb);
        const int chunk = (int)(t / nb);
        const int k0 = chunk * CK + ks * 16 + half * 8;
        const int n = nblk * BN + nl;
        float v[8];
#pragma unroll
        for (int e = 0; e < 8; ++e) v[e] = 0.f;
        if (n < d.N) {
            const float* sp = d.src + (long long)k0 * d.sk + (long long)n * d.sn;
            if (d.sk == 1 && k0 + 8 <= d.K && ((reinterpret_cast<uintptr_t>(sp) & 15) == 0)) {
                const f32x4 a = *reinterpret_cast<const f32x4*>(sp), b = *reinterpret_cast<const f32x4*>(sp + 4);
#pragma unroll
                for (int e = 0; e < 4; ++e) { v[e] = a[e]; v[4 + e] = b[e]; }
            } else {
#pragma unroll
                for (int e = 0; e < 8; ++e)
                    if (k0 + e < d.K) v[e] = sp[(long long)e * d.sk];
            }
        }
        bf16x8_t o;
#pragma unroll
        for (int e = 0; e < 8; ++e) o[e] = (__bf16)v[e];
        *reinterpret_cast<bf16x8_t*>(dst + gi * 8) = o;
    }
}

}

int vf_gemm_bf16_g256_launch(const vf_igemm_args& a, hipStream_t stream);

extern "C" {

size_t vf_gemm_bf16_packed_elems(int K, int N) {
    if (K <= 0 || N <= 0) return 0;
    return (size_t)((K + CK - 1) / CK) * ((N + BN - 1) / BN) * CK * BN;
}

int vf_gemm_bf16_pack(const float* src, void* dst, int K, int N, int64_t sk, int64_t sn, int batch, int64_t src_bstride,
                      void* stream) {
    if (!src || !dst || K <= 0 || N <= 0 || batch < 1) return VF_ERR_BAD_ARG;
    const int nb = (N + BN - 1) / BN, nchunks = (K + CK - 1) / CK;
    const long long total = (long long)nchunks * nb * CK * BN;
    const int blocks = (int)((total + 255) / 256 > 4096 ? 4096 : (total + 255) / 256);
    hipLaunchKernelGGL(pack_bf16_kernel, dim3(blocks, batch), dim3(256), 0, (hipStream_t)stream, src, (__bf16*)dst, K, N,
                       (long long)sk, (long long)sn, nb, nchunks, (long long)src_bstride, total);
    return vf_last_status();
}

int vf_gemm_bf16_pack_multi(const vf_pack_desc* descs_device, int n, void* stream) {
    if (!descs_device || n <= 0) return VF_ERR_BAD_ARG;
    hipLaunchKernelGGL(pack_bf16_multi_kernel, dim3(128, (unsigned)n), dim3(256), 0, (hipStream_t)stream, descs_device);
    return vf_last_status();
}

int vf_gemm_bf16(const vf_igemm_args* args, void* stream) {
    if (!args) return VF_ERR_BAD_ARG;
    const vf_igemm_args& a = *args;
    if (!a.x || !a.w_packed || !a.out || a.M <= 0 || a.Cin <= 0 || a.Cout <= 0) return VF_ERR_BAD_ARG;
    if (a.gn_part) return VF_ERR_UNSUPPORTED;
    if (a.mode != VF_MODE_GEMM || a.pro_mean) return VF_ERR_UNSUPPORTED;
    if (a.Cin % CK != 0) return VF_ERR_UNSUPPORTED;
    if (a.epilogue == VF_EPI_GELU_BWD && !(a.reserved0 & 2)) return VF_ERR_UNSUPPORTED;
    if ((a.epilogue == VF_EPI_GELU_DUAL) != (a.out_aux != nullptr)) return VF_ERR_BAD_ARG;
    if (a.lda < a.Cin || (a.lda & 3) || a.ldc < a.Cout || (a.res && a.ldr < a.Cout)) return VF_ERR_BAD_ARG;
    if (a.epilogue == VF_EPI_GELU_DUAL) {
        if (!(a.reserved0 & 1) || a.batch > 1 || a.Cin % (2 * CK) != 0) return VF_ERR_UNSUPPORTED;
        const int rc = vf_gemm_bf16_g256_launch(a, (hipStream_t)stream);
        return rc;
    }
    if (a.drop_rate != 0.f) {
        if (!(a.reserved0 & 1) || (a.reserved0 & 2) || a.batch > 1 || a.Cin % (2 * CK) != 0) return VF_ERR_UNSUPPORTED;
        return vf_gemm_bf16_g256_launch(a, (hipStream_t)stream);
    }
    const size_t smem = (size_t)2 * (A_BYTES + B_BYTES);
    static unsigned long long attr_devs = 0;
    if (vf_attr_needed(&attr_devs)) {
        hipError_t e = hipFuncSetAttribute(reinterpret_cast<const void*>(gemm_bf16_kernel),
                                           hipFuncAttributeMaxDynamicSharedMemorySize, (int)smem);
        if (e != hipSuccess) return (int)e;
        vf_attr_done(&attr_devs);
    }
    const int nb = (a.Cout + BN - 1) / BN, mt = (a.M + BM - 1) / BM;
    const bool a16 = a.reserved0 & 1, o16 = a.reserved0 & 2;
    if (a16 || o16) {
        if (a.Cin % (2 * CK) != 0 || a.batch > 1) return VF_ERR_UNSUPPORTED;
        if ((a16 && (a.lda & 7)) || (o16 && a.res && a.epilogue != VF_EPI_GELU_BWD)) return VF_ERR_BAD_ARG;
        if (a.epilogue == VF_EPI_GELU_BWD && !(o16 && a.res && a.ldr >= a.Cout)) return VF_ERR_BAD_ARG;
        if (a.reserved0 & 4) {
            if (a.epilogue != VF_EPI_GELU_BWD) return VF_ERR_BAD_ARG;
            return vf_gemm_bf16_g256_launch(a, (hipStream_t)stream);
        }
        if (vf_selected(VF_SEL_GEMM_G256)) {
            const int rc = vf_gemm_bf16_g256_launch(a, (hipStream_t)stream);
            if (rc != VF_ERR_UNSUPPORTED) return rc;
        }
        const dim3 g((unsigned)(mt * nb));
        hipStream_t st = (hipStream_t)stream;
        if (a16 && o16) hipLaunchKernelGGL((gemm_bf16_direct_kernel<true, true>), g, dim3(256), (size_t)2 * A_BYTES, st, a);
        else if (a16) hipLaunchKernelGGL((gemm_bf16_direct_kernel<true, false>), g, dim3(256), (size_t)2 * A_BYTES, st, a);
        else hipLaunchKernelGGL((gemm_bf16_direct_kernel<false, true>), g, dim3(256), (size_t)2 * A_BYTES, st, a);
        return vf_last_status();
    }
    if (a.Cin % (2 * CK) == 0 && a.batch <= 1) {
        hipLaunchKernelGGL((gemm_bf16_direct_kernel<false, false>), dim3((unsigned)(mt * nb)), dim3(256), (size_t)2 * A_BYTES, (hipStream_t)stream, a);
        return vf_last_status();
    }
    dim3 grid((unsigned)(mt * nb), 1, (unsigned)(a.batch > 0 ? a.batch : 1));
    hipLaunchKernelGGL(gemm_bf16_kernel, grid, dim3(256), smem, (hipStream_t)stream, a);
    return vf_last_status();
}

}
```

viewformer_amd/csrc/gemm_bf16_g256.hip:

```cpp
#include "vf_common.h"
#include "epilogue.h"
#include "../../include/vf_hip.h"

namespace {

typedef __bf16 bf16x8 __attribute__((ext_vector_type(8)));
typedef __bf16 bf16x2_t __attribute__((ext_vector_type(2)));

constexpr int GM = 256, GN = 256, GK = 64;
constexpr int GA_BYTES = GM * GK * 2;
constexpr int GB_BYTES = GN * GK * 2;
constexpr int GSTAGE = GA_BYTES + GB_BYTES;

__device__ __forceinline__ void bufds16(__amdgpu_buffer_rsrc_t r, void* l, unsigned voff, unsigned soff) {
    __builtin_amdgcn_raw_ptr_buffer_load_lds(r, (__attribute__((address_space(3))) void*)l, 16, voff, soff, 0, 0);
}

template <bool DROP, int IC>
__device__ __forceinline__ void g256_store_f32(const vf_igemm_args& p, const f32x16 (&acc)[IC][2], int m_tile0, int n_tile0, int wrow0,
                                               int wave_n, int half, int l31, bool full, bool gelu) {
    const long long ldc = p.ldc, ldr = p.ldr;
    const bool has_res = p.res != nullptr;
    const bool dual = p.epilogue == VF_EPI_GELU_DUAL;
    const int odd = l31 & 1;
    const uint32_t drop_thresh = vf_dropout_thresh(p.drop_rate), drop_key = vf_dropout_key(p.drop_seed, p.drop_site, 0u);
    const float drop_scale = 1.0f / (1.0f - p.drop_rate);
#pragma unroll
    for (int j = 0; j < 2; ++j) {
        const int n = n_tile0 + wave_n * 64 + j * 32 + l31;
        const float bias = p.bias ? p.bias[n] : 0.f;
#pragma unroll
        for (int i = 0; i < IC; ++i) {
            int m0 = m_tile0 + wrow0 + i * 32 + 4 * half;
            if constexpr (DROP) asm volatile("" : "+v"(m0) :: "memory");
            const int rows_left = p.M - m0;
            float* o = p.out + (size_t)(rows_left > 0 ? m0 : 0) * ldc + n;
            float v[16];
#pragma unroll
            for (int r = 0; r < 16; ++r) v[r] = acc[i][j][r] + bias;
            if (gelu) {
#pragma unroll
                for (int r = 0; r < 16; ++r) v[r] = vf_gelu_erf_fast(v[r]);
            }
            if constexpr (DROP) {
#pragma unroll
                for (int g = 0; g < 4; ++g) {
                    const uint32_t w = vf_dropout_word(drop_key, (uint32_t)(((m0 + p.drop_row0) >> 2) + 2 * g) * (uint32_t)p.Cout + (uint32_t)n);
#pragma unroll
                    for (int e = 0; e < 4; ++e) v[4 * g + e] = vf_dropout_keep(w, e, drop_thresh) ? v[4 * g + e] * drop_scale : 0.f;
                }
            }
            if (has_res) {
                const float* rs = p.res + (size_t)(rows_left > 0 ? m0 : 0) * ldr + n;
                float rr[16];
#pragma unroll
                for (int r = 0; r < 16; ++r) {
                    const int row = (r & 3) + 8 * (r >> 2);
                    rr[r] = rs[(long long)(full || row < rows_left ? row : 0) * ldr];
                }
#pragma unroll
                for (int r = 0; r < 16; ++r) v[r] += rr[r];
            }
            if (full) {
#pragma unroll
                for (int r = 0; r < 16; ++r) o[(long long)((r & 3) + 8 * (r >> 2)) * ldc] = v[r];
            } else if (rows_left > 0) {
#pragma unroll
                for (int r = 0; r < 16; ++r) {
                    const int row = (r & 3) + 8 * (r >> 2);
                    if (row < rows_left) o[(long long)row * ldc] = v[r];
                }
            }
            if (dual) {
                __builtin_amdgcn_sched_barrier(0);
                __bf16* o16 = reinterpret_cast<__bf16*>(p.out_aux) + (size_t)(rows_left > 0 ? m0 : 0) * ldc + (n - odd);
#pragma unroll
                for (int r = 0; r < 16; ++r) v[r] = vf_gelu_erf_fast(v[r]);
#pragma unroll
                for (int r = 0; r < 16; r += 2) {
                    const float give = odd ? v[r] : v[r + 1];
                    const float got = vf_lane_xor1(give);
                    const int row = ((r + odd) & 3) + 8 * ((r + odd) >> 2);
                    bf16x2_t h;
                    h[0] = (__bf16)(odd ? got : v[r]);
                    h[1] = (__bf16)(odd ? v[r + 1] : got);
                    if (full || row < rows_left) *reinterpret_cast<bf16x2_t*>(o16 + (long long)row * ldc) = h;
                }
            }
            __builtin_amdgcn_sched_barrier(0);
        }
    }
}

template <int EPI, bool FULL, int IC>
__device__ __forceinline__ void g256_store_bf16(const vf_igemm_args& p, const f32x16 (&acc)[IC][2], int m_tile0, int n_tile0, int wrow0,
                                                int wave_n, int half, int l31) {
    __bf16* __restrict__ O = reinterpret_cast<__bf16*>(p.out);
    const int odd = l31 & 1;
#pragma unroll
    for (int j = 0; j < 2; ++j) {
        const int n = n_tile0 + wave_n * 64 + j * 32 + l31;
        const float bias = p.bias ? p.bias[n] : 0.f;
#pragma unroll
        for (int i = 0; i < IC; ++i) {
            const int m0 = m_tile0 + wrow0 + i * 32 + 4 * half;
            float t[16];
            if (EPI == 2 || EPI == 4) {
                const bool u16 = p.reserved0 & 4;
                const unsigned esz = u16 ? 2u : 4u;
                const __amdgpu_buffer_rsrc_t u_rs = __builtin_amdgcn_make_buffer_rsrc(
                    const_cast<unsigned char*>(reinterpret_cast<const unsigned char*>(p.res) + (size_t)m_tile0 * p.ldr * esz), 0,
                    (int)min((long long)0x7fffffff, (long long)(p.M - m_tile0) * p.ldr * esz), 0x00020000);
                float uu[16];
                if (u16) {
                    const unsigned voff = ((unsigned)(m0 - m_tile0) * (unsigned)p.ldr + (unsigned)(n - odd)) * 2u;
                    unsigned w[8];
#pragma unroll
                    for (int r = 0; r < 16; r += 2) {
                        const int row = ((r + odd) & 3) + 8 * ((r + odd) >> 2);
                        w[r >> 1] = __builtin_amdgcn_raw_buffer_load_b32(u_rs, voff + (unsigned)row * (unsigned)p.ldr * 2u, 0, 0);
                    }
#pragma unroll
                    for (int r = 0; r < 16; r += 2) {
                        const unsigned mine = w[r >> 1];
                        const unsigned give = odd ? (mine << 16) : (mine & 0xffff0000u);
                        const unsigned got = vf_lane_xor1(give);
                        uu[r] = __builtin_bit_cast(float, odd ? got : (mine << 16));
                        uu[r + 1] = __builtin_bit_cast(float, odd ? (mine & 0xffff0000u) : got);
                    }
                } else {
                    const unsigned voff = ((unsigned)(m0 - m_tile0) * (unsigned)p.ldr + (unsigned)n) * 4u;
#pragma unroll
                    for (int r = 0; r < 16; ++r) {
                        const unsigned soff = (unsigned)((r & 3) + 8 * (r >> 2)) * (unsigned)p.ldr * 4u;
                        uu[r] = __builtin_bit_cast(float, __builtin_amdgcn_raw_buffer_load_b32(u_rs, voff, soff, 0));
                    }
                }
                __builtin_amdgcn_sched_barrier(0);
#pragma unroll
                for (int q = 0; q < 4; ++q) {
#pragma unroll
                    for (int e = 0; e < 4; ++e)
                        t[4 * q + e] = __fmul_rn(__fadd_rn(acc[i][j][4 * q + e], bias), EPI == 4 ? uu[4 * q + e] : vf_gelu_grad_fast(uu[4 * q + e]));
                    __builtin_amdgcn_sched_barrier(0);
                }
            } else {
#pragma unroll
                for (int r = 0; r < 16; ++r) {
                    t[r] = acc[i][j][r] + bias;
                    if (EPI == 1) t[r] = vf_gelu_erf_fast(t[r]);
                }
            }
            float gq[EPI == 5 ? 16 : 1];
            if (EPI == 5) {
#pragma unroll
                for (int r = 0; r < 16; ++r) { float f, g; vf_gelu_and_grad_fast(t[r], f, g); t[r] = f; gq[r] = g; }
            }
#pragma unroll
            for (int pass = 0; pass < ((EPI == 3 || EPI == 5) ? 2 : 1); ++pass) {
                __bf16* __restrict__ dst = pass == 0 ? O : reinterpret_cast<__bf16*>(p.out_aux);
                if (EPI == 3 && pass == 1) {
                    __builtin_amdgcn_sched_barrier(0);
#pragma unroll
                    for (int r = 0; r < 16; ++r) t[r] = vf_gelu_erf_fast(t[r]);
                }
#pragma unroll
                for (int r = 0; r < 16; r += 2) {
                    const float lo = (EPI == 5 && pass == 0) ? gq[r] : t[r], hi = (EPI == 5 && pass == 0) ? gq[r + 1] : t[r + 1];
                    const float give = odd ? lo : hi;
                    const float got = vf_lane_xor1(give);
                    const int m = m0 + ((r + odd) & 3) + 8 * ((r + odd) >> 2);
                    bf16x2_t v;
                    v[0] = (__bf16)(odd ? got : lo);
                    v[1] = (__bf16)(odd ? hi : got);
                    if (FULL || m < p.M) *reinterpret_cast<bf16x2_t*>(dst + (size_t)m * p.ldc + (n - odd)) = v;
                }
            }
        }
    }
}

template <bool O16, bool DROP, int IC>
__device__ __forceinline__ void g256_tile(const vf_igemm_args& p, unsigned char* smem_b, int m_tile0, int nblk, int tid) {
    constexpr int TROWS = 2 * IC * 32;
    const int lane = tid & 63;
    const int wave = __builtin_amdgcn_readfirstlane(tid >> 6);
    const int wave_m = wave >> 2, wave_n = wave & 3;
    const int half = lane >> 5, l31 = lane & 31;
    const int wrow0 = wave_m * (IC * 32);
    const int n_tile0 = nblk * GN;
    const int nstages = p.Cin / GK;

    const bool a_mover = wave * 32 < TROWS;
    const __amdgpu_buffer_rsrc_t a_rsrc = __builtin_amdgcn_make_buffer_rsrc(const_cast<float*>(p.x), 0, 0x7fffffff, 0x00020000);
    const __amdgpu_buffer_rsrc_t w_rsrc = __builtin_amdgcn_make_buffer_rsrc(const_cast<float*>(p.w_packed), 0, 0x7fffffff, 0x00020000);
    unsigned avoff[4];
#pragma unroll
    for (int q = 0; q < 4; ++q) {
        const int r = wave * 32 + q * 8 + (lane >> 3);
        const int c = (lane & 7) ^ ((r >> 1) & 7);
        int m = m_tile0 + r;
        m = m < p.M ? m : p.M - 1;
        avoff[q] = (unsigned)(((size_t)m * p.lda) * 2 + c * 16);
    }
    const unsigned wvoff = (unsigned)((size_t)nblk * GB_BYTES + wave * 4096 + lane * 16);
    const size_t w_stage_stride = (size_t)(p.Cout / 128) * (GK * 128 * 2);
    auto issue = [&](int s) {
        unsigned char* dst = smem_b + (s & 1) * GSTAGE;
        if (IC == 4 || a_mover) {
#pragma unroll
            for (int q = 0; q < 4; ++q) bufds16(a_rsrc, dst + (wave * 32 + q * 8) * 128, avoff[q], (unsigned)(s * (GK * 2)));
        }
#pragma unroll
        for (int q = 0; q < 4; ++q) bufds16(w_rsrc, dst + GA_BYTES + wave * 4096 + q * 1024, wvoff + q * 1024, (unsigned)((size_t)s * w_stage_stride));
    };

    const unsigned a_row_off = (unsigned)((wrow0 + l31) * 128);
    const unsigned a_swz = (unsigned)((l31 >> 1) & 7);
    unsigned a_off[4];
#pragma unroll
    for (int ks = 0; ks < 4; ++ks) a_off[ks] = a_row_off + ((((unsigned)(ks * 2 + half)) ^ a_swz) << 4);
    const unsigned b_off = (unsigned)(GA_BYTES + (wave_n >> 1) * (GK * 128 * 2) + ((half * 128) + (wave_n & 1) * 64 + l31) * 16);

    f32x16 acc[IC][2];
#pragma unroll
    for (int i = 0; i < IC; ++i)
#pragma unroll
        for (int j = 0; j < 2; ++j)
#pragma unroll
            for (int r = 0; r < 16; ++r) acc[i][j][r] = 0.f;

    issue(0);
    for (int s = 0; s < nstages; ++s) {
        asm volatile("s_waitcnt vmcnt(0) lgkmcnt(0)" ::: "memory");
        __builtin_amdgcn_s_barrier();
        if (s + 1 < nstages) issue(s + 1);
        const unsigned char* buf = smem_b + (s & 1) * GSTAGE;
        bf16x8 a[2][IC], b[2][2];
        auto frags = [&](int ks, bf16x8 (&af)[IC], bf16x8 (&bf)[2]) {
#pragma unroll
            for (int j = 0; j < 2; ++j) bf[j] = *reinterpret_cast<const bf16x8*>(buf + b_off + (ks * 2 * 128 + j * 32) * 16);
#pragma unroll
            for (int i = 0; i < IC; ++i) af[i] = *reinterpret_cast<const bf16x8*>(buf + a_off[ks] + i * (32 * 128));
        };
        frags(0, a[0], b[0]);
#pragma unroll
        for (int ks = 0; ks < 4; ++ks) {
            if (ks < 3) frags(ks + 1, a[(ks + 1) & 1], b[(ks + 1) & 1]);
            __builtin_amdgcn_sched_barrier(0);
#pragma unroll
            for (int i = 0; i < IC; ++i)
#pragma unroll
                for (int j = 0; j < 2; ++j)
                    acc[i][j] = __builtin_amdgcn_mfma_f32_32x32x16_bf16(a[ks & 1][i], b[ks & 1][j], acc[i][j], 0, 0, 0);
            __builtin_amdgcn_sched_barrier(0);
        }
    }

    const bool full = m_tile0 + TROWS <= p.M;
    const bool gelu = p.epilogue == VF_EPI_GELU_ERF;
    if (O16) {
        const bool gbwd = p.epilogue == VF_EPI_GELU_BWD;
        const bool dual16 = p.epilogue == VF_EPI_GELU_DUAL;
        const bool deriv = p.reserved0 & 8;
        if (dual16 && deriv) {
            if (full) g256_store_bf16<5, true, IC>(p, acc, m_tile0, n_tile0, wrow0, wave_n, half, l31);
            else g256_store_bf16<5, false, IC>(p, acc, m_tile0, n_tile0, wrow0, wave_n, half, l31);
        } else if (gbwd && deriv) {
            if (full) g256_store_bf16<4, true, IC>(p, acc, m_tile0, n_tile0, wrow0, wave_n, half, l31);
            else g256_store_bf16<4, false, IC>(p, acc, m_tile0, n_tile0, wrow0, wave_n, half, l31);
        } else if (dual16) {
            if (full) g256_store_bf16<3, true, IC>(p, acc, m_tile0, n_tile0, wrow0, wave_n, half, l31);
            else g256_store_bf16<3, false, IC>(p, acc, m_tile0, n_tile0, wrow0, wave_n, half, l31);
        } else if (full) {
            if (gbwd) g256_store_bf16<2, true, IC>(p, acc, m_tile0, n_tile0, wrow0, wave_n, half, l31);
            else if (gelu) g256_store_bf16<1, true, IC>(p, acc, m_tile0, n_tile0, wrow0, wave_n, half, l31);
            else g256_store_bf16<0, true, IC>(p, acc, m_tile0, n_tile0, wrow0, wave_n, half, l31);
        } else {
            if (gbwd) g256_store_bf16<2, false, IC>(p, acc, m_tile0, n_tile0, wrow0, wave_n, half, l31);
            else if (gelu) g256_store_bf16<1, false, IC>(p, acc, m_tile0, n_tile0, wrow0, wave_n, half, l31);
            else g256_store_bf16<0, false, IC>(p, acc, m_tile0, n_tile0, wrow0, wave_n, half, l31);
        }
    } else {
        g256_store_f32<DROP, IC>(p, acc, m_tile0, n_tile0, wrow0, wave_n, half, l31, full, gelu);
    }
}

__device__ __forceinline__ void g256_panel_order(unsigned lbid, int mt, int nb, int& mtile, int& nblk) {
    constexpr int PANEL = 4;
    const int sn = nb <= PANEL ? nb : nb % PANEL == 0 ? PANEL : nb % 3 == 0 ? 3 : nb % 2 == 0 ? 2 : 1;
    const int per_panel = mt * sn;
    const int panel = (int)(lbid / (unsigned)per_panel);
    const int in_panel = (int)(lbid - (unsigned)panel * per_panel);
    nblk = panel * sn + in_panel % sn;
    mtile = in_panel / sn;
}

template <bool O16, bool DROP = false, bool TAIL = false>
__global__ __launch_bounds__(512, 1) void gemm_bf16_g256_kernel(vf_igemm_args p, int f_rows, int h_rows, int tail_ic) {
    extern __shared__ __attribute__((aligned(16))) unsigned char smem_b[];
    const int tid = threadIdx.x;
    const int nb = p.Cout / GN;
    int mtile, nblk;
    if constexpr (!TAIL) {
        g256_panel_order(vf_xcd_bid(), (p.M + GM - 1) / GM, nb, mtile, nblk);
        g256_tile<O16, DROP, 4>(p, smem_b, mtile * GM, nblk, tid);
    } else {
        const unsigned F = (unsigned)(f_rows * nb), tot = gridDim.x;
        const unsigned x = blockIdx.x & 7u, i = blockIdx.x >> 3;
        const unsigned nF = F / 8u + (x < (F & 7u) ? 1u : 0u);
        const unsigned baseF = x * (F / 8u) + (x < (F & 7u) ? x : (F & 7u));
        if (i < nF) {
            g256_panel_order(baseF + i, f_rows, nb, mtile, nblk);
            g256_tile<O16, DROP, 4>(p, smem_b, mtile * GM, nblk, tid);
            return;
        }
        const unsigned baseT = x * (tot / 8u) + (x < (tot & 7u) ? x : (tot & 7u));
        g256_panel_order(baseT - baseF + (i - nF), h_rows, nb, mtile, nblk);
        const int m_tile0 = f_rows * GM + mtile * (tail_ic * 64);
        if (tail_ic == 3) g256_tile<O16, DROP, 3>(p, smem_b, m_tile0, nblk, tid);
        else g256_tile<O16, DROP, 2>(p, smem_b, m_tile0, nblk, tid);
    }
}

}

struct G256Tail { int f_rows, h_rows, ic; };
static G256Tail g256_tail_policy(int M, int nb) {
    const int mt = (M + GM - 1) / GM;
    const long long ntiles = (long long)mt * nb;
    constexpr int CUS = 256;
    G256Tail none{0, 0, 0};
    if (ntiles <= CUS || !vf_selected(VF_SEL_GEMM_TAIL)) return none;
    const int last = (int)(ntiles % CUS);
    if (last == 0 || last > (CUS * 3) / 4 - 8 || last < 16) return none;
    const int f_rows = (int)((ntiles / CUS) * CUS / nb);
    if (f_rows <= 0 || f_rows >= mt) return none;
    const int rem_blocks = (M - f_rows * GM + 31) / 32;
    for (int ic = 2; ic <= 3; ++ic) {
        const int h_rows = (rem_blocks + 2 * ic - 1) / (2 * ic);
        if ((long long)h_rows * nb <= CUS) return G256Tail{f_rows, h_rows, ic};
    }
    return none;
}

int vf_gemm_bf16_g256_launch(const vf_igemm_args& a, hipStream_t stream) {
    const bool a16 = a.reserved0 & 1, o16 = a.reserved0 & 2;
    if (!a16 || a.batch > 1 || a.Cout % GN != 0 || a.Cin % GK != 0 || a.M < GM || (a.lda & 7)) return VF_ERR_UNSUPPORTED;
    if (o16 && ((a.res && a.epilogue != VF_EPI_GELU_BWD) || (a.ldc & 1))) return VF_ERR_UNSUPPORTED;
    if (a.epilogue == VF_EPI_GELU_BWD && !(o16 && a.res)) return VF_ERR_UNSUPPORTED;
    if (a.epilogue == VF_EPI_GELU_DUAL && (a.res || !a.out_aux || (a.ldc & 1))) return VF_ERR_UNSUPPORTED;
    if ((a.reserved0 & 4) && a.epilogue != VF_EPI_GELU_BWD) return VF_ERR_BAD_ARG;
    if (a.reserved0 & 8) {
        if (a.epilogue == VF_EPI_GELU_BWD ? !(a.reserved0 & 4) : !(a.epilogue == VF_EPI_GELU_DUAL && o16)) return VF_ERR_BAD_ARG;
    }
    if (a.res && a.epilogue == VF_EPI_GELU_ERF) return VF_ERR_UNSUPPORTED;
    if (a.drop_rate != 0.f && (!(a.drop_rate > 0.f && a.drop_rate < 1.f) || o16 || a.epilogue != VF_EPI_NONE || a.drop_row0 < 0 || (a.drop_row0 & 3) ||
                               (((unsigned long long)a.M + (unsigned long long)a.drop_row0 + 3) / 4) * (unsigned long long)a.Cout >= (1ull << 32)))
        return VF_ERR_UNSUPPORTED;
    if ((size_t)a.M * a.lda * 2 >= (1ull << 31) || (size_t)a.Cin * a.Cout * 2 >= (1ull << 31)) return VF_ERR_UNSUPPORTED;
    const int mt = (a.M + GM - 1) / GM, nb = a.Cout / GN;
    const G256Tail t = g256_tail_policy(a.M, nb);
    const dim3 g((unsigned)(t.f_rows ? (t.f_rows + t.h_rows) * nb : mt * nb));
    auto launch = [&](auto kernel, unsigned long long* devs) -> int {
        if (vf_attr_needed(devs)) {
            const hipError_t e = hipFuncSetAttribute(reinterpret_cast<const void*>(kernel), hipFuncAttributeMaxDynamicSharedMemorySize, 2 * GSTAGE);
            if (e != hipSuccess) return (int)e;
            vf_attr_done(devs);
        }
        hipLaunchKernelGGL(kernel, g, dim3(512), (size_t)2 * GSTAGE, stream, a, t.f_rows, t.h_rows, t.ic);
        return vf_last_status();
    };
    static unsigned long long d0 = 0, d1 = 0, d2 = 0, d3 = 0, d4 = 0, d5 = 0;
    const bool drop = a.drop_rate > 0.f;
    if (t.f_rows) {
        if (o16) return launch(gemm_bf16_g256_kernel<true, false, true>, &d3);
        return drop ? launch(gemm_bf16_g256_kernel<false, true, true>, &d5) : launch(gemm_bf16_g256_kernel<false, false, true>, &d4);
    }
    if (o16) return launch(gemm_bf16_g256_kernel<true, false, false>, &d0);
    return drop ? launch(gemm_bf16_g256_kernel<false, true, false>, &d2) : launch(gemm_bf16_g256_kernel<false, false, false>, &d1);
}
```

viewformer_amd/csrc/vf_common.h:

```cpp
#pragma once
#include <hip/hip_runtime.h>
#include <stdint.h>

typedef float f32x4 __attribute__((ext_vector_type(4)));
typedef float f32x16 __attribute__((ext_vector_type(16)));

#define VF_OK 0
#define VF_ERR_BAD_ARG (-1)
#define VF_ERR_UNSUPPORTED (-2)

#define VF_WAVE 64

static inline int vf_last_status() {
    hipError_t e = hipGetLastError();
    return e == hipSuccess ? VF_OK : (int)e;
}

static inline bool vf_attr_needed(unsigned long long* mask) {
    int d = 0;
    (void)hipGetDevice(&d);
    return !((__atomic_load_n(mask, __ATOMIC_RELAXED) >> (d & 63)) & 1ull);
}
static inline void vf_attr_done(unsigned long long* mask) {
    int d = 0;
    (void)hipGetDevice(&d);
    __atomic_fetch_or(mask, 1ull << (d & 63), __ATOMIC_RELAXED);
}

__device__ __forceinline__ float vf_swish(float v) {
    return v / (1.0f + expf(-v));
}

__device__ __forceinline__ float vf_swish_1ulp(float v) {
    const float LH = -1.4426950408889634f, LL = -1.9259629911266175e-8f;
    float th = v * LH;
    const float tl = __builtin_fmaf(v, LH, -th) + v * LL;
    th = fminf(th, 126.0f);
    const float e0 = __builtin_amdgcn_exp2f(th);
    const float d = 1.0f + __builtin_fmaf(e0 * tl, 0.6931471805599453f, e0);
    float r = __builtin_amdgcn_rcpf(d);
    r = __builtin_fmaf(__builtin_fmaf(-d, r, 1.0f), r, r);
    return v * r;
}

__device__ __forceinline__ float vf_exp_neg(float d) {
    const float LH = 1.4426950408889634f, LL = 1.9259629911266175e-8f;
    const float th = __fmul_rn(d, LH);
    const float tl = __builtin_fmaf(d, LH, -th) + d * LL;
    const float e0 = __builtin_amdgcn_exp2f(th);
    return __builtin_fmaf(e0 * tl, 0.6931471805599453f, e0);
}

__device__ __forceinline__ float vf_gelu_erf(float v) {
    return 0.5f * v * (1.0f + erff(v * 0.70710678118654752440f));
}

__device__ __forceinline__ float vf_gelu_grad(float x) {
    const float cdf = __fmul_rn(0.5f, __fadd_rn(1.0f, erff(__fmul_rn(x, 0.70710678118654752440f))));
    const float pdf = __fmul_rn(0.39894228040143267794f, expf(__fmul_rn(-0.5f, __fmul_rn(x, x))));
    return __fmaf_rn(x, pdf, cdf);
}

__device__ __forceinline__ float vf_gelu_grad_fast(float x) {
    const float z = __fmul_rn(fabsf(x), 0.70710678118654752440f);
    const float t = __builtin_amdgcn_rcpf(__fmaf_rn(0.3275911f, z, 1.0f));
    float p = __fmaf_rn(1.061405429f, t, -1.453152027f);
    p = __fmaf_rn(p, t, 1.421413741f);
    p = __fmaf_rn(p, t, -0.284496736f);
    p = __fmaf_rn(p, t, 0.254829592f);
    const float e = __builtin_amdgcn_exp2f(__fmul_rn(-1.4426950408889634f, __fmul_rn(z, z)));
    const float erf_abs = __fmaf_rn(-__fmul_rn(p, t), e, 1.0f);
    const float cdf = __fmul_rn(0.5f, __fadd_rn(1.0f, copysignf(erf_abs, x)));
    return __fmaf_rn(x, __fmul_rn(0.39894228040143267794f, e), cdf);
}

__device__ __forceinline__ float vf_gelu_erf_fast(float v) {
    const float z = fabsf(v) * 0.70710678118654752440f;
    float t = __builtin_amdgcn_rcpf(__builtin_fmaf(0.3275911f, z, 1.0f));
    float p = __builtin_fmaf(1.061405429f, t, -1.453152027f);
    p = __builtin_fmaf(p, t, 1.421413741f);
    p = __builtin_fmaf(p, t, -0.284496736f);
    p = __builtin_fmaf(p, t, 0.254829592f);
    const float e = __builtin_amdgcn_exp2f(-1.4426950408889634f * z * z);
    const float erf_abs = __builtin_fmaf(-p * t, e, 1.0f);
    return 0.5f * v * (1.0f + copysignf(erf_abs, v));
}

__device__ __forceinline__ void vf_gelu_and_grad_fast(float v, float& f, float& g) {
    const float z = fabsf(v) * 0.70710678118654752440f;
    float t = __builtin_amdgcn_rcpf(__builtin_fmaf(0.3275911f, z, 1.0f));
    float p = __builtin_fmaf(1.061405429f, t, -1.453152027f);
    p = __builtin_fmaf(p, t, 1.421413741f);
    p = __builtin_fmaf(p, t, -0.284496736f);
    p = __builtin_fmaf(p, t, 0.254829592f);
    const float e = __builtin_amdgcn_exp2f(-1.4426950408889634f * z * z);
    const float erf_abs = __builtin_fmaf(-p * t, e, 1.0f);
    const float one_plus = 1.0f + copysignf(erf_abs, v);
    f = 0.5f * v * one_plus;
    g = __builtin_fmaf(v, 0.39894228040143267794f * e, 0.5f * one_plus);
}

__device__ __forceinline__ int vf_lane_xor1(int v) { return __builtin_amdgcn_mov_dpp(v, 0xB1, 0xF, 0xF, true); }
__device__ __forceinline__ unsigned vf_lane_xor1(unsigned v) { return (unsigned)__builtin_amdgcn_mov_dpp((int)v, 0xB1, 0xF, 0xF, true); }
__device__ __forceinline__ float vf_lane_xor1(float v) { return __int_as_float(__builtin_amdgcn_mov_dpp(__float_as_int(v), 0xB1, 0xF, 0xF, true)); }

__device__ __forceinline__ float vf_wave_sum(float v) {
#pragma unroll
    for (int o = 32; o > 0; o >>= 1) v += __shfl_xor(v, o, 64);
    return v;
}

__device__ __forceinline__ float vf_wave_sum_dpp(float v) {
#define VF_DPP_ADD(ctrl, rmask) v += __int_as_float(__builtin_amdgcn_update_dpp(0, __float_as_int(v), ctrl, rmask, 0xF, false))
    VF_DPP_ADD(0x111, 0xF);
    VF_DPP_ADD(0x112, 0xF);
    VF_DPP_ADD(0x114, 0xF);
    VF_DPP_ADD(0x118, 0xF);
    VF_DPP_ADD(0x142, 0xA);
    VF_DPP_ADD(0x143, 0xC);
#undef VF_DPP_ADD
    return __int_as_float(__builtin_amdgcn_readlane(__float_as_int(v), 63));
}

__device__ __forceinline__ float vf_wave_max(float v) {
#pragma unroll
    for (int o = 32; o > 0; o >>= 1) v = fmaxf(v, __shfl_xor(v, o, 64));
    return v;
}

__device__ __forceinline__ void vf_block_max_atomic(float m, unsigned* out) {
    __shared__ float vf_bm_red[4];
    m = vf_wave_max(m);
    if ((threadIdx.x & 63) == 0) vf_bm_red[threadIdx.x >> 6] = m;
    __syncthreads();
    if (threadIdx.x == 0) atomicMax(out, __float_as_uint(fmaxf(fmaxf(vf_bm_red[0], vf_bm_red[1]), fmaxf(vf_bm_red[2], vf_bm_red[3]))));
}

__host__ __device__ __forceinline__ uint32_t vf_dropout_hash(uint32_t seed, uint32_t site, uint64_t idx) {
    uint32_t h = seed ^ (site * 0x9E3779B9u);
    h ^= (uint32_t)idx;
    h *= 0x85EBCA6Bu;
    h ^= h >> 13;
    h += (uint32_t)(idx >> 32) * 0xC2B2AE35u + 0x27D4EB2Fu;
    h ^= h >> 16;
    h *= 0x165667B1u;
    h ^= h >> 15;
    h *= 0xD3A2646Cu;
    h ^= h >> 16;
    return h;
}
__host__ __device__ __forceinline__ uint32_t vf_lowbias32(uint32_t x) {
    x ^= x >> 16;
    x *= 0x7FEB352Du;
    x ^= x >> 15;
    x *= 0x846CA68Bu;
    x ^= x >> 16;
    return x;
}
__host__ __device__ __forceinline__ uint32_t vf_dropout_key(uint32_t seed, uint32_t site, uint32_t hi) { return vf_dropout_hash(seed, site, (uint64_t)hi); }
__host__ __device__ __forceinline__ uint32_t vf_dropout_word(uint32_t key, uint32_t lo) { return vf_lowbias32(lo ^ key); }
__host__ __device__ __forceinline__ bool vf_dropout_keep(uint32_t word, int j, uint32_t thresh) {
    const uint32_t s = 8u * ((uint32_t)j & 3u);
    return ((word << s) | (word >> ((32u - s) & 31u))) >= thresh;
}
__device__ __forceinline__ uint32_t vf_dropout_rotr(int j) { return (32u - 8u * ((uint32_t)j & 3u)) & 31u; }
__device__ __forceinline__ bool vf_dropout_keep_rotr(uint32_t word, uint32_t rr, uint32_t thresh) { return __builtin_amdgcn_alignbit(word, word, rr) >= thresh; }
__host__ __device__ __forceinline__ bool vf_dropout_keep_elem(uint32_t seed, uint32_t site, uint64_t m, uint32_t n, uint32_t N, uint32_t thresh) {
    const uint64_t g = (m >> 2) * (uint64_t)N + n;
    return vf_dropout_keep(vf_dropout_word(vf_dropout_key(seed, site, (uint32_t)(g >> 32)), (uint32_t)g), (int)(m & 3), thresh);
}
__host__ __device__ __forceinline__ uint32_t vf_dropout_thresh(float rate) { return (uint32_t)((double)rate * 4294967296.0); }

__device__ __forceinline__ unsigned vf_xcd_bid() {
    const unsigned n = gridDim.x, b = blockIdx.x;
    const unsigned q = n >> 3, r = n & 7u, x = b & 7u, i = b >> 3;
    return x * q + (x < r ? x : r) + i;
}

__device__ __forceinline__ float vf_vq_sq4(const f32x4 v) {
    return __builtin_fmaf(v[0], v[0], v[1] * v[1]) + __builtin_fmaf(v[2], v[2], v[3] * v[3]);
}

extern "C" int vf_register_build_flag(const char* name);
#define VF_REG_FLAG(m) namespace { const int vf_flagreg_##m = vf_register_build_flag(#m); }
#ifdef VF_X_TRINTRIN
VF_REG_FLAG(VF_X_TRINTRIN)
#endif

int vf_pack_b_impl(const float* src, float* dst, int K, int N, int taps, long long sk, long long sn, long long st,
                   int BN, int batch, long long src_bstride, hipStream_t stream);

struct vf_attn_order { unsigned char blk[64]; };
static inline bool vf_attn_visible(int qv, int kv, int twin) {
    if (twin <= -2) {
        const int Sv = -twin, qs = qv / Sv, qi = qv - qs * Sv, ks = kv / Sv, ki = kv - ks * Sv;
        return qs == 0 ? (ks == 0 && ki <= qi) : ((ks == 0 && ki < qi) || kv == qv);
    }
    const int Vc = twin >= 0 ? twin : 0x3fffffff;
    return kv == qv || (kv < Vc ? kv : Vc) < (qv < Vc ? qv : Vc);
}
static inline vf_attn_order vf_attn_block_order(int nviews, int vpb, int nblocks, int twin, bool by_key) {
    vf_attn_order o;
    int w[64];
    if (nblocks > 64) nblocks = 64;
    for (int b = 0; b < 64; ++b) o.blk[b] = (unsigned char)b;
    for (int b = 0; b < nblocks; ++b) {
        int cnt = 0;
        for (int t = 0; t < nviews; ++t) {
            bool any = false;
            for (int v = b * vpb; v < (b + 1) * vpb && v < nviews && !any; ++v) any = by_key ? vf_attn_visible(t, v, twin) : vf_attn_visible(v, t, twin);
            cnt += any;
        }
        w[b] = cnt;
    }
    for (int i = 1; i < nblocks; ++i) {
        const unsigned char bi = o.blk[i];
        int j = i - 1;
        while (j >= 0 && w[o.blk[j]] < w[bi]) { o.blk[j + 1] = o.blk[j]; --j; }
        o.blk[j + 1] = bi;
    }
    return o;
}

struct vf_attn_groups { unsigned char view[64][4]; int n; };
static inline vf_attn_groups vf_attn_query_groups(int nviews, int twin) {
    vf_attn_groups g;
    for (int i = 0; i < 64; ++i) for (int j = 0; j < 4; ++j) g.view[i][j] = 0xFF;
    g.n = 0;
    unsigned char list[256];
    int nl = 0;
    const int Sv = twin <= -2 ? -twin : 0;
    if (Sv > 0 && nviews % Sv == 0 && nviews / Sv >= 2 && nviews <= 255) {
        const int NS = nviews / Sv;
        for (int v = 0; v < Sv; ++v) list[nl++] = (unsigned char)v;
        const int pad = (4 - Sv % 4) % 4;
        int taken = 0;
        unsigned char br[256];
        int nb = 0;
        for (int i = Sv - 1; i >= 0; --i)
            for (int s_ = 1; s_ < NS; ++s_) br[nb++] = (unsigned char)(s_ * Sv + i);
        for (; taken < pad && taken < nb; ++taken) list[nl++] = br[taken];
        while (nl % 4) list[nl++] = 0xFF;
        for (int i = taken; i < nb; ++i) list[nl++] = br[i];
    } else {
        for (int v = 0; v < nviews && v < 256; ++v) list[nl++] = (unsigned char)v;
    }
    while (nl % 4) list[nl++] = 0xFF;
    g.n = nl / 4 > 64 ? 64 : nl / 4;
    int w[64];
    for (int b = 0; b < g.n; ++b) {
        int cnt = 0;
        for (int t = 0; t < nviews; ++t) {
            bool any = false;
            for (int j = 0; j < 4 && !any; ++j) { const int v = list[4 * b + j]; any = v != 0xFF && vf_attn_visible(v, t, twin); }
            cnt += any;
        }
        w[b] = cnt;
    }
    int ord[64];
    for (int b = 0; b < g.n; ++b) ord[b] = b;
    for (int i = 1; i < g.n; ++i) {
        const int bi = ord[i];
        int j = i - 1;
        while (j >= 0 && w[ord[j]] < w[bi]) { ord[j + 1] = ord[j]; --j; }
        ord[j + 1] = bi;
    }
    for (int b = 0; b < g.n; ++b) for (int j = 0; j < 4; ++j) g.view[b][j] = list[4 * ord[b] + j];
    return g;
}

typedef __bf16 vf_bf16x8 __attribute__((ext_vector_type(8)));
typedef short vf_s16x4 __attribute__((ext_vector_type(4)));
__device__ __forceinline__ unsigned vf_lds_addr(const void* p) {
    return (unsigned)(size_t)(__attribute__((address_space(3))) const void*)p;
}
__device__ __forceinline__ vf_bf16x8 vf_tr_join(vf_s16x4 lo, vf_s16x4 hi) {
    return __builtin_bit_cast(vf_bf16x8, __builtin_shufflevector(lo, hi, 0, 1, 2, 3, 4, 5, 6, 7));
}
__device__ __forceinline__ void vf_tr_frag2_wait(vf_bf16x8& a, vf_bf16x8& b, unsigned addr, int offA, int offB, int gap) {
    vf_s16x4 a0, a1, b0, b1;
    asm volatile("ds_read_b64_tr_b16 %0, %4 offset:%5\n\tds_read_b64_tr_b16 %1, %4 offset:%6\n\tds_read_b64_tr_b16 %2, %4 offset:%7\n\t"
                 "ds_read_b64_tr_b16 %3, %4 offset:%8\n\ts_waitcnt lgkmcnt(0)"
                 : "=&v"(a0), "=&v"(a1), "=&v"(b0), "=&v"(b1) : "v"(addr), "i"(offA), "i"(offA + gap), "i"(offB), "i"(offB + gap) : "memory");
    a = vf_tr_join(a0, a1);
    b = vf_tr_join(b0, b1);
}
```

viewformer_amd/ops.py:

```python
import ctypes
import os

import torch

from . import _lib
from ._lib import VfIgemmArgs, check

MODE_GEMM, MODE_CONV3_S1, MODE_CONV3_S2PAD, MODE_CONV3_UP2 = 0, 1, 2, 3
EPI_NONE, EPI_GELU, EPI_GELU_BWD, EPI_GELU_DUAL = 0, 1, 2, 3


def _stream():
    return ctypes.c_void_p(torch.cuda.current_stream().cuda_stream)


def _p(t):
    if t is None:
        return None
    return ctypes.c_void_p(t.data_ptr())


def _chk(t, dtype=torch.float32, name='tensor'):
    if not t.is_cuda:
        raise _lib.VfError(f'{name} must live on the GPU (no CPU fallback for the hot path)')
    if t.dtype != dtype:
        raise TypeError(f'{name} must be {dtype}, got {t.dtype}')
    return t


def _f32(t, name='tensor'):
    return _chk(t, torch.float32, name)


def packed_floats(K, N, taps=1):
    return int(_lib.load().vf_igemm_packed_floats(K, N, taps))


def pack(src, K, N, taps, sk, sn, st, batch=1, src_bstride=0, out=None):
    lib = _lib.load()
    n = packed_floats(K, N, taps)
    if out is None:
        out = torch.empty(batch * n, dtype=torch.float32, device=src.device)
    check(lib.vf_igemm_pack_f32(_p(_f32(src)), _p(out), K, N, taps, sk, sn, st, batch, src_bstride, _stream()),
          'vf_igemm_pack_f32')
    return out


def pack_conv_oihw(w):
    w = _f32(w).contiguous()
    cout, cin, kh, kw = w.shape
    taps = kh * kw
    return pack(w, cin, cout, taps, sk=taps, sn=cin * taps, st=1)


def pack_dense_kn(w):
    w = _f32(w).contiguous()
    k, n = w.shape
    return pack(w, k, n, 1, sk=n, sn=1, st=0)


def pack_dense_nk(w, n_rows=None):
    w = _f32(w).contiguous()
    n, k = w.shape
    n = n if n_rows is None else n_rows
    return pack(w, k, n, 1, sk=1, sn=k, st=0)


def pack_dense_kn_bf16(w):
    lib = _lib.load()
    w = _f32(w).contiguous()
    k, n = w.shape
    out = torch.empty(int(lib.vf_gemm_bf16_packed_elems(k, n)), dtype=torch.bfloat16, device=w.device)
    check(lib.vf_gemm_bf16_pack(_p(w), _p(out), k, n, n, 1, 1, 0, _stream()), 'vf_gemm_bf16_pack')
    return out


def pack_bf16_multi(items):
    import numpy as np
    lib = _lib.load()
    dt = np.dtype([('src', '<u8'), ('dst', '<u8'), ('K', '<i4'), ('N', '<i4'), ('sk', '<i8'), ('sn', '<i8')])
    assert dt.itemsize == _lib.PACK_DESC_BYTES
    a = np.zeros(len(items), dtype=dt)
    for i, (w, tr, out) in enumerate(items):
        _f32(w); _chk(out, torch.bfloat16)
        assert w.is_contiguous() and w.dim() == 2
        r, c = w.shape
        K, N, sk, sn = (c, r, 1, c) if tr else (r, c, c, 1)
        assert out.numel() >= int(lib.vf_gemm_bf16_packed_elems(K, N))
        a[i] = (w.data_ptr(), out.data_ptr(), K, N, sk, sn)
    descs = torch.from_numpy(a.view(np.uint8).copy()).to(items[0][0].device)
    n = len(items)

    def run(first=0, count=None):
        count = n - first if count is None else count
        if count <= 0:
            return
        assert 0 <= first and first + count <= n
        check(lib.vf_gemm_bf16_pack_multi(descs.data_ptr() + first * _lib.PACK_DESC_BYTES, count, _stream()), 'vf_gemm_bf16_pack_multi')
    run()
    return run


def pack_dense_nk_bf16(w, n_rows=None):
    lib = _lib.load()
    w = _f32(w).contiguous()
    n, k = w.shape
    n = n if n_rows is None else n_rows
    out = torch.empty(int(lib.vf_gemm_bf16_packed_elems(k, n)), dtype=torch.bfloat16, device=w.device)
    check(lib.vf_gemm_bf16_pack(_p(w), _p(out), k, n, 1, k, 1, 0, _stream()), 'vf_gemm_bf16_pack')
    return out


def pack_conv3_bf16(w_oihw):
    lib = _lib.load()
    w = _f32(w_oihw).contiguous()
    cout, cin = w.shape[:2]
    out = torch.empty(int(lib.vf_conv3_bf16_packed_elems(cin, cout)), dtype=torch.bfloat16, device=w.device)
    check(lib.vf_conv3_bf16_pack(_p(w), _p(out), cin, cout, _stream()), 'vf_conv3_bf16_pack')
    return out


def pack_conv3_x6(w_oihw):
    lib = _lib.load()
    w = _f32(w_oihw).contiguous()
    cout, cin = w.shape[:2]
    out = torch.empty(int(lib.vf_conv3_x6_packed_elems(cin, cout)), dtype=torch.bfloat16, device=w.device)
    check(lib.vf_conv3_x6_pack(_p(w), _p(out), cin, cout, _stream()), 'vf_conv3_x6_pack')
    return out


def pack_conv3_x3h(w_oihw):
    lib = _lib.load()
    w = _f32(w_oihw).contiguous()
    cout, cin = w.shape[:2]
    out = torch.empty(int(lib.vf_conv3_x3h_packed_elems(cin, cout)), dtype=torch.float16, device=w.device)
    check(lib.vf_conv3_x3h_pack(_p(w), _p(out), cin, cout, _stream()), 'vf_conv3_x3h_pack')
    return out


def conv3_x3h_supported(mode, Cin, Cout, Hout, Wout):
    if mode == MODE_CONV3_S2PAD and Hout == 8 and Wout == 8 and Cin % 32 == 0 and Cout % 128 == 0:
        return True
    return conv3_x6_supported(mode, Cin, Cout, Hout, Wout)


def pack_dense_kn_x6(w):
    lib = _lib.load()
    w = _f32(w).contiguous()
    k, n = w.shape
    out = torch.empty(int(lib.vf_gemm_x6_packed_elems(k, n)), dtype=torch.bfloat16, device=w.device)
    check(lib.vf_gemm_x6_pack(_p(w), _p(out), k, n, n, 1, _stream()), 'vf_gemm_x6_pack')
    return out


def pack_dense_nk_x6(w, n_rows=None):
    lib = _lib.load()
    w = _f32(w).contiguous()
    n, k = w.shape
    n = n if n_rows is None else n_rows
    out = torch.empty(int(lib.vf_gemm_x6_packed_elems(k, n)), dtype=torch.bfloat16, device=w.device)
    check(lib.vf_gemm_x6_pack(_p(w), _p(out), k, n, 1, k, _stream()), 'vf_gemm_x6_pack')
    return out


def pack_dense_kn_x3h(w):
    lib = _lib.load()
    w = _f32(w).contiguous()
    k, n = w.shape
    out = torch.empty(int(lib.vf_gemm_x3h_packed_elems(k, n)), dtype=torch.float16, device=w.device)
    check(lib.vf_gemm_x3h_pack(_p(w), _p(out), k, n, n, 1, _stream()), 'vf_gemm_x3h_pack')
    return out


def pack_dense_nk_x3h(w, n_rows=None):
    lib = _lib.load()
    w = _f32(w).contiguous()
    n, k = w.shape
    n = n if n_rows is None else n_rows
    out = torch.empty(int(lib.vf_gemm_x3h_packed_elems(k, n)), dtype=torch.float16, device=w.device)
    check(lib.vf_gemm_x3h_pack(_p(w), _p(out), k, n, 1, k, _stream()), 'vf_gemm_x3h_pack')
    return out


def gemm_x6_splitk(x, w_packed, M, Cin, Cout, dst, splits, lda=None, accumulate=True):
    lib = _lib.load()
    slabs = torch.empty((splits, M, Cout), dtype=torch.float32, device=x.device)
    igemm(x, w_packed, M, Cin, Cout, slabs, lda=lda, x6=True, split_k=splits, stride_out=M * Cout)
    check(lib.vf_sum_slabs_f32(_p(slabs), splits, M * Cout, M * Cout, _p(_f32(dst)), 1 if accumulate else 0, _stream()),
          'vf_sum_slabs_f32')
    return dst


def conv3_x6_supported(mode, Cin, Cout, Hout, Wout):
    if mode not in (MODE_CONV3_S1, MODE_CONV3_UP2, MODE_CONV3_S2PAD) or Cin % 32 or Cout % 128:
        return False
    return (Hout % 8 == 0 and Wout % 16 == 0) or (mode == MODE_CONV3_S1 and Hout == 8 and Wout == 8)


def gemm_bf16_splitk(x, w_packed, M, Cin, Cout, dst, splits, lda=None, accumulate=True):
    lib = _lib.load()
    ks = Cin // splits
    if splits < 1 or ks * splits != Cin or ks % 64:
        raise _lib.VfError(f'gemm_bf16_splitk: Cin = {Cin} does not split into {splits} ranges of whole 64-deep chunks')
    nb = (Cout + 127) // 128
    slabs = torch.empty((splits, M, Cout), dtype=torch.float32, device=x.device)
    igemm(x, w_packed, M, ks, Cout, slabs, lda=Cin if lda is None else lda, bf16=True, batch=splits, stride_x=ks,
          stride_w=(ks // 64) * nb * 64 * 128, stride_out=M * Cout)
    check(lib.vf_sum_slabs_f32(_p(slabs), splits, M * Cout, M * Cout, _p(_f32(dst)), 1 if accumulate else 0, _stream()),
          'vf_sum_slabs_f32')
    return dst


TN_TARGET_WORKGROUPS = 256
TN_TARGET_WORKGROUPS_BESIDE = 192


def gemm_tn_bf16_supported(x, M, K, N):
    return x.dtype == torch.bfloat16 and gemm_tn_bf16_shape_ok(M, K, N)


def gemm_tn_bf16_shape_ok(M, K, N):
    return K % 256 == 0 and N % 256 == 0 and M % 64 == 0 and M * K * 2 < 2 ** 31


def gemm_g256_shape_ok(M, K, N):
    return N % 256 == 0 and K % 64 == 0 and M >= 256 and M * K * 2 < 2 ** 31 and K * N * 2 < 2 ** 31


def gemm_drop_supported(M, K, N, row0=0):
    return gemm_g256_shape_ok(M, K, N) and row0 % 4 == 0 and ((M + row0 + 3) // 4) * N < 2 ** 32


def gemm_tn_bf16(x16, dy, M, K, N, dw, db=None, accumulate=True, beside_another_gemm=False):
    lib = _lib.load()
    _chk(x16, torch.bfloat16, 'x16')
    tiles = (K // 256) * (N // 256)
    target = TN_TARGET_WORKGROUPS_BESIDE if beside_another_gemm else TN_TARGET_WORKGROUPS
    splits = max(1, min(M // 64, target // tiles if tiles <= target else 1))
    rec = K * N + (N if db is not None else 0)
    ws = torch.empty((splits, rec), dtype=torch.float32, device=dy.device)
    y16 = dy.dtype == torch.bfloat16
    check(lib.vf_gemm_tn_bf16(_p(x16), x16.stride(0), _p(dy if y16 else _f32(dy)), 1 if y16 else 0, dy.stride(0), M, K, N, splits, _p(ws),
                              ws.data_ptr() + K * N * 4 if db is not None else None, rec, _stream()), 'vf_gemm_tn_bf16')
    acc = 1 if accumulate else 0
    _f32(dw)
    if db is not None and _f32(db).data_ptr() == dw.data_ptr() + K * N * 4 and dw.is_contiguous():
        check(lib.vf_sum_slabs_f32(_p(ws), splits, rec, rec, _p(dw), acc, _stream()), 'vf_sum_slabs_f32')
    else:
        check(lib.vf_sum_slabs_f32(_p(ws), splits, rec, K * N, _p(dw), acc, _stream()), 'vf_sum_slabs_f32')
        if db is not None:
            check(lib.vf_sum_slabs_f32(ws.data_ptr() + K * N * 4, splits, rec, N, _p(db), acc, _stream()), 'vf_sum_slabs_f32')
    return dw


def igemm(x, w_packed, M, Cin, Cout, out, bias=None, res=None, mode=MODE_GEMM, epilogue=EPI_NONE,
          pro=None, pro_swish=False, pro_rows_per_img=0, Hin=0, Win=0, Hout=0, Wout=0,
          lda=None, ldc=None, ldr=None, batch=1, stride_x=0, stride_w=0, stride_out=0, stride_res=0, bf16=False, x6=False, gn_part=None, split_k=0,
          x3h=False, a16=False, o16=False, out_aux=None, res16=False, drop=None, gelu_grad=False):
    lib = _lib.load()
    if not 0 <= M < 2 ** 31 or max(Cin, Cout, Hin, Win, Hout, Wout, batch) >= 2 ** 31:
        raise _lib.VfError(f'igemm: M = {M} rows do not fit the int32 fields of vf_igemm_args — split the launch '
                           '(VQGAN(max_images_per_call=...))')
    a = VfIgemmArgs()
    a.x = x.data_ptr()
    a.w_packed = w_packed.data_ptr()
    a.bias = bias.data_ptr() if bias is not None else None
    a.res = res.data_ptr() if res is not None else None
    a.out = out.data_ptr()
    if out_aux is not None:
        _chk(out_aux, torch.bfloat16, 'out_aux')
        if out_aux.shape != out.shape or not (out_aux.is_contiguous() or out_aux.stride() == out.stride()):
            raise _lib.VfError('out_aux must have the shape and row stride of out')
        a.out_aux = out_aux.data_ptr()
    if pro is not None:
        mean_c, scale_c, beta = pro
        a.pro_mean, a.pro_scale, a.pro_beta = mean_c.data_ptr(), scale_c.data_ptr(), beta.data_ptr()
    a.pro_swish = 1 if pro_swish else 0
    a.pro_rows_per_img = pro_rows_per_img
    a.mode, a.epilogue = mode, epilogue
    a.M, a.Cin, a.Cout = M, Cin, Cout
    a.Hin, a.Win, a.Hout, a.Wout = Hin, Win, Hout, Wout
    a.lda = Cin if lda is None else lda
    a.ldc = Cout if ldc is None else ldc
    a.ldr = (Cout if ldr is None else ldr)
    a.batch = batch
    a.stride_x, a.stride_w, a.stride_out, a.stride_res = stride_x, stride_w, stride_out, stride_res
    a.reserved0 = split_k
    if gn_part is not None:
        a.gn_part = _f32(gn_part).data_ptr()
        a.gn_slots = gn_part.shape[1]
    conv16 = False
    if a16 or o16:
        if not bf16 or mode not in (MODE_GEMM, MODE_CONV3_S1, MODE_CONV3_UP2):
            raise _lib.VfError('a16 / o16 need bf16=True and a GEMM or 3x3 stride-1 / upsample convolution')
        _chk(x, torch.bfloat16 if a16 else torch.float32, 'x')
        _chk(out, torch.bfloat16 if o16 else torch.float32, 'out')
        a.reserved0 = (1 if a16 else 0) | (2 if o16 else 0)
        conv16 = mode != MODE_GEMM
        if conv16:
            if a16 and not o16:
                raise _lib.VfError('the bf16 convolution takes bf16 activations in only together with bf16 out')
            if res is not None:
                _chk(res, torch.bfloat16 if o16 else torch.float32, 'res')
    if drop is not None and drop[0]:
        if not (bf16 and a16 and not o16 and mode == MODE_GEMM and epilogue == EPI_NONE):
            raise _lib.VfError('drop needs the bf16 GEMM with bf16 x, fp32 out and no epilogue function')
        a.drop_rate, a.drop_seed, a.drop_site = float(drop[0]), int(drop[1]) & 0xFFFFFFFF, int(drop[2])
        a.drop_row0 = int(drop[3]) if len(drop) > 3 else 0
    if res16:
        if not (a16 and o16 and epilogue == EPI_GELU_BWD and res is not None):
            raise _lib.VfError('res16 is the bf16 pre-activation of EPI_GELU_BWD (bf16 in, bf16 out)')
        _chk(res, torch.bfloat16, 'res')
        a.reserved0 |= 4
    if gelu_grad:
        if not ((epilogue == EPI_GELU_DUAL and a16 and o16) or (epilogue == EPI_GELU_BWD and res16)):
            raise _lib.VfError('gelu_grad: EPI_GELU_DUAL with bf16 in / out, or EPI_GELU_BWD with res16')
        a.reserved0 |= 8
    for t in ((None if a16 else x), (None if o16 else out), bias, (None if (res16 or conv16) else res)):
        if t is not None:
            _f32(t)
    if x3h:
        _chk(w_packed, torch.float16, 'w_packed')
        if mode == MODE_GEMM:
            check(lib.vf_gemm_x3h(ctypes.byref(a), _stream()), 'vf_gemm_x3h')
        else:
            check(lib.vf_conv3_halo_x3h(ctypes.byref(a), _stream()), 'vf_conv3_halo_x3h')
        return out
    if x6:
        _chk(w_packed, torch.bfloat16, 'w_packed')
        if mode == MODE_GEMM:
            check(lib.vf_gemm_x6(ctypes.byref(a), _stream()), 'vf_gemm_x6')
        else:
            check(lib.vf_conv3_halo_x6(ctypes.byref(a), _stream()), 'vf_conv3_halo_x6')
        return out
    if bf16:
        _chk(w_packed, torch.bfloat16, 'w_packed')
        if mode == MODE_GEMM:
            check(lib.vf_gemm_bf16(ctypes.byref(a), _stream()), 'vf_gemm_bf16')
        else:
            check(lib.vf_conv3_halo_bf16(ctypes.byref(a), _stream()), 'vf_conv3_halo_bf16')
        return out
    _f32(w_packed)
    check(lib.vf_igemm_f32(ctypes.byref(a), _stream()), 'vf_igemm_f32')
    return out


def conv3_small_cout_supported(mode, Cin, Cout, H, W):
    return mode == MODE_CONV3_S1 and 1 <= Cout <= 4 and Cin % 32 == 0 and Cin // 32 * 4608 <= 96 * 1024 and H % 8 == 0 and W % 32 == 0


def conv3_small_cout(x, w_oihw, bias, n_img, H, W, Cin, Cout, pro=None, pro_swish=True, out=None):
    lib = _lib.load()
    if out is None:
        out = torch.empty((n_img * H * W, Cout), dtype=torch.float32, device=x.device)
    pm, ps, pb = (None, None, None) if pro is None else pro
    x16 = x.dtype == torch.bfloat16
    check(lib.vf_conv3_small_cout_f32(_p(x if x16 else _f32(x)), _p(_f32(w_oihw)), _p(_f32(bias)) if bias is not None else None,
                                      _p(pm) if pm is not None else None, _p(ps) if ps is not None else None,
                                      _p(pb) if pb is not None else None, 1 if pro_swish else 0, _p(out), n_img, H, W, Cin, Cout,
                                      1 if x16 else 0, _stream()), 'vf_conv3_small_cout_f32')
    return out


def pack_conv_in_x3h(w_oihw):
    lib = _lib.load()
    w = _f32(w_oihw).contiguous()
    out = torch.empty(int(lib.vf_conv_in_x3h_packed_elems(w.shape[0])), dtype=torch.float16, device=w.device)
    check(lib.vf_conv_in_x3h_pack(_p(w), _p(out), w.shape[0], _stream()), 'vf_conv_in_x3h_pack')
    return out


def conv_in_x3h_supported(H, W, Cout):
    return H % 8 == 0 and W % 16 == 0 and Cout % 128 == 0


def conv_in(img, w_oihw, bias, n_img, H, W, Cout, out=None, wp3h=None, gn_part=None):
    lib = _lib.load()
    if out is None:
        out = torch.empty((n_img, H, W, Cout), dtype=torch.float32, device=img.device)
    if img.dtype == torch.uint8:
        u8, f32 = _p(_chk(img, torch.uint8)), None
    else:
        u8, f32 = None, _p(_f32(img))
    if wp3h is not None:
        _chk(wp3h, torch.float16, 'wp3h')
        check(lib.vf_conv_in_x3h(u8, f32, _p(wp3h), _p(bias), _p(out), _p(gn_part) if gn_part is not None else None,
                                 gn_part.shape[1] if gn_part is not None else 0, n_img, H, W, Cout, _stream()), 'vf_conv_in_x3h')
        return out
    if gn_part is not None:
        raise _lib.VfError('conv_in: fused GroupNorm statistics need the x3h form (wp3h)')
    check(lib.vf_conv_in_u8_f32(u8, f32, _p(_f32(w_oihw)), _p(bias), _p(out), n_img, H, W, Cout, _stream()),
          'vf_conv_in_u8_f32')
    return out


def groupnorm_stats(x, gamma, n_img, HW, C, groups=32, eps=1e-6):
    lib = _lib.load()
    mean_c = torch.empty((n_img, C), dtype=torch.float32, device=x.device)
    scale_c = torch.empty((n_img, C), dtype=torch.float32, device=x.device)
    ws = torch.empty(int(lib.vf_groupnorm_workspace_bytes(n_img, HW, C)), dtype=torch.uint8, device=x.device)
    check(lib.vf_groupnorm_stats_f32(_p(_f32(x)), _p(_f32(gamma)), n_img, HW, C, groups, eps, _p(mean_c), _p(scale_c),
                                     _p(ws), _stream()), 'vf_groupnorm_stats_f32')
    return mean_c, scale_c


def halo_gn_slots(Hout, Wout):
    return int(_lib.load().vf_conv3_halo_gn_slots(Hout, Wout))


def new_gn_part(n_img, Hout, Wout, device):
    return torch.empty((n_img, halo_gn_slots(Hout, Wout), 32, 2), dtype=torch.float32, device=device)


def groupnorm_finalize(part, gamma, n_img, HW, C, groups=32, eps=1e-6):
    lib = _lib.load()
    mean_c = torch.empty((n_img, C), dtype=torch.float32, device=part.device)
    scale_c = torch.empty((n_img, C), dtype=torch.float32, device=part.device)
    check(lib.vf_groupnorm_finalize_f32(_p(_f32(part)), _p(_f32(gamma)), n_img, HW, C, groups, part.shape[1], eps,
                                        _p(mean_c), _p(scale_c), _stream()), 'vf_groupnorm_finalize_f32')
    return mean_c, scale_c


def groupnorm_apply(x, mean_c, scale_c, beta, n_img, HW, C, swish, out=None):
    lib = _lib.load()
    if out is None:
        out = torch.empty_like(x)
    check(lib.vf_groupnorm_apply_f32(_p(_f32(x)), _p(mean_c), _p(scale_c), _p(_f32(beta)), _p(out), n_img, HW, C,
                                     1 if swish else 0, _stream()), 'vf_groupnorm_apply_f32')
    return out


def vq_pack_codebook(E):
    lib = _lib.load()
    E = _f32(E).contiguous()
    D, Kc = E.shape
    out = torch.empty(int(lib.vf_vq_packed_floats(D, Kc)), dtype=torch.float32, device=E.device)
    check(lib.vf_vq_pack_codebook_f32(_p(E), _p(out), D, Kc, _stream()), 'vf_vq_pack_codebook_f32')
    e_sq = torch.empty(Kc, dtype=torch.float32, device=E.device)
    check(lib.vf_colsumsq_f32(_p(E), _p(e_sq), D, Kc, _stream()), 'vf_colsumsq_f32')
    return out, e_sq


def vq_argmin(z_rows, E_packed, e_sq, D, Kc):
    lib = _lib.load()
    z_rows = _f32(z_rows)
    M = z_rows.numel() // D
    idx = torch.empty(M, dtype=torch.int64, device=z_rows.device)
    check(lib.vf_vq_argmin_f32(_p(z_rows), _p(E_packed), _p(e_sq), M, D, Kc, _p(idx), _stream()), 'vf_vq_argmin_f32')
    return idx


def vq_filter_supported(D, Kc):
    return int(_lib.load().vf_vq_filter_packed_bytes(D, Kc)) > 0


def vq_filter_pack(E):
    lib = _lib.load()
    E = _f32(E).contiguous()
    D, Kc = E.shape
    n = int(lib.vf_vq_filter_packed_bytes(D, Kc))
    if n == 0:
        raise _lib.VfError(f'vq_filter_pack: unsupported codebook shape D={D}, Kc={Kc} (need D == 256, Kc % 32 == 0, Kc <= 1024)')
    out = torch.empty(n, dtype=torch.uint8, device=E.device)
    check(lib.vf_vq_filter_pack(_p(E), _p(out), D, Kc, _stream()), 'vf_vq_filter_pack')
    return out


def vq_argmin_filtered(z_rows, blob, D, Kc, stats=None):
    lib = _lib.load()
    z_rows = _f32(z_rows)
    M = z_rows.numel() // D
    idx = torch.empty(M, dtype=torch.int64, device=z_rows.device)
    check(lib.vf_vq_argmin_filtered_f32(_p(z_rows), _p(_chk(blob, torch.uint8, 'blob')), M, D, Kc, _p(idx),
                                        _p(_chk(stats, torch.int32, 'stats')) if stats is not None else None, _stream()),
          'vf_vq_argmin_filtered_f32')
    return idx


def codebook_gather(E, idx, D, Kc):
    lib = _lib.load()
    idx = _chk(idx, torch.int64, 'codes').contiguous()
    M = idx.numel()
    out = torch.empty((M, D), dtype=torch.float32, device=idx.device)
    check(lib.vf_codebook_gather_f32(_p(_f32(E)), _p(idx), _p(out), M, D, Kc, _stream()), 'vf_codebook_gather_f32')
    return out


def attn_blockcausal(q, k, v, out, B, H, T, L, ldq, ldk, ldv, ldo, scale=1.0, skip_masked=True, twin_view=-1, bf16=False, x6=False,
                     fp8=False):
    lib = _lib.load()
    if fp8:
        bf16 = True
    if x6:
        check(lib.vf_attn_blockcausal_x6(_p(_f32(q)), _p(_f32(k)), _p(_f32(v)), _p(_f32(out)), B, H, T, L, ldq, ldk, ldv,
                                         ldo, scale, 1 if skip_masked else 0, twin_view, _stream()),
              'vf_attn_blockcausal_x6')
        return out
    if bf16:
        o16 = out.dtype == torch.bfloat16
        i16 = q.dtype == torch.bfloat16
        for t in (q, k, v):
            _chk(t, torch.bfloat16 if i16 else torch.float32, 'q/k/v')
        fn = lib.vf_attn_blockcausal_fp8 if fp8 else lib.vf_attn_blockcausal_bf16_v2
        check(fn(_p(q), _p(k), _p(v), 1 if i16 else 0, _p(out if o16 else _f32(out)), 1 if o16 else 0, B, H, T, L,
                 ldq, ldk, ldv, ldo, scale, 1 if skip_masked else 0, twin_view, _stream()), 'vf_attn_blockcausal_lp')
        return out
    check(lib.vf_attn_blockcausal_f32(_p(_f32(q)), _p(_f32(k)), _p(_f32(v)), _p(_f32(out)), B, H, T, L, ldq, ldk, ldv,
                                      ldo, scale, 1 if skip_masked else 0, twin_view, _stream()),
          'vf_attn_blockcausal_f32')
    return out


def attn_prefix(q, k, v, kp, vp, out, B, H, C, N, L, ldq, ldk, ldv, ldkp, ldvp, prefix_stride, ldo, bf16=False, dh=64):
    lib = _lib.load()
    if bf16:
        o16 = out.dtype == torch.bfloat16
        i16 = q.dtype == torch.bfloat16
        for t in (q, k, v, kp, vp):
            _chk(t, torch.bfloat16 if i16 else torch.float32, 'q/k/v/prefix')
        check(lib.vf_attn_prefix_bf16(_p(q), _p(k), _p(v), _p(kp), _p(vp), 1 if i16 else 0, _p(out if o16 else _f32(out)), 1 if o16 else 0,
                                      B, H, C, N, L, dh, ldq, ldk, ldv, ldkp, ldvp, prefix_stride, ldo, _stream()), 'vf_attn_prefix_bf16')
        return out
    check(lib.vf_attn_prefix_f32eq(_p(_f32(q)), _p(_f32(k)), _p(_f32(v)), _p(_f32(kp)), _p(_f32(vp)), _p(_f32(out)), B, H, C, N, L, dh,
                                   ldq, ldk, ldv, ldkp, ldvp, prefix_stride, ldo, _stream()), 'vf_attn_prefix_f32eq')
    return out


def attn_spatial_supported(HW, C):
    return (HW, C) in ((256, 256), (64, 512), (64, 256))


def attn_spatial(qkv, n_img, HW, C, scale, out=None, x3h=False):
    if out is None:
        out = torch.empty((n_img * HW, C), dtype=torch.float32, device=qkv.device)
    fn = _lib.load().vf_attn_spatial_x3h if x3h else _lib.load().vf_attn_spatial_f32
    check(fn(_p(_f32(qkv)), _p(_f32(out)), n_img, HW, C, qkv.stride(0), out.stride(0), scale, _stream()),
          'vf_attn_spatial_x3h' if x3h else 'vf_attn_spatial_f32')
    return out


def softmax_rows_(x, rows, n, scale=1.0):
    check(_lib.load().vf_softmax_rows_f32(_p(_f32(x)), rows, n, scale, _stream()), 'vf_softmax_rows_f32')
    return x


def layernorm(x, gamma, beta, rows, d, eps=1e-5, out=None, out_bf16=False):
    if out_bf16:
        out = torch.empty(x.shape, dtype=torch.bfloat16, device=x.device) if out is None else _chk(out, torch.bfloat16, 'out')
        check(_lib.load().vf_layernorm_bf16out_f32(_p(_f32(x)), _p(_f32(gamma)), _p(_f32(beta)), _p(out), rows, d, eps, _stream()),
              'vf_layernorm_bf16out_f32')
        return out
    if out is None:
        out = torch.empty_like(x)
    check(_lib.load().vf_layernorm_f32(_p(_f32(x)), _p(_f32(gamma)), _p(_f32(beta)), _p(out), rows, d, eps, _stream()),
          'vf_layernorm_f32')
    return out


def embed_sum(ids_i32, wte, wpe, add, BS, L, d, vocab):
    out = torch.empty((BS * L, d), dtype=torch.float32, device=wte.device)
    check(_lib.load().vf_embed_sum_f32(_p(_chk(ids_i32, torch.int32, 'ids')), _p(_f32(wte)), _p(_f32(wpe)),
                                       _p(_f32(add)), _p(out), BS, L, d, vocab, _stream()), 'vf_embed_sum_f32')
    return out


def dense_small_k(x, W, b, rows, K, N, gelu):
    out = torch.empty((rows, N), dtype=torch.float32, device=x.device)
    check(_lib.load().vf_dense_small_k_gelu_f32(_p(_f32(x)), _p(_f32(W)), _p(b), _p(out), rows, K, N,
                                                1 if gelu else 0, _stream()), 'vf_dense_small_k_gelu_f32')
    return out


def argmax_rows(x, rows, n, ld=None):
    idx = torch.empty(rows, dtype=torch.int64, device=x.device)
    check(_lib.load().vf_argmax_rows_f32(_p(_f32(x)), rows, n, n if ld is None else ld, _p(idx), _stream()),
          'vf_argmax_rows_f32')
    return idx


def lmhead_argmax_supported(K, N):
    return K in (128, 768) and N % 128 == 0


def lmhead_argmax_bf16(h, w_packed_bf16, M, K, N, want_max=False):
    idx = torch.empty(M, dtype=torch.int64, device=h.device)
    mx = torch.empty(M, dtype=torch.float32, device=h.device) if want_max else None
    h16 = h.dtype == torch.bfloat16
    _chk(h, torch.bfloat16 if h16 else torch.float32, 'h')
    check(_lib.load().vf_lmhead_argmax_bf16(_p(h), 1 if h16 else 0, h.stride(0), _p(_chk(w_packed_bf16, torch.bfloat16, 'w_packed')), M, K, N,
                                            _p(idx), _p(mx) if mx is not None else None, _stream()), 'vf_lmhead_argmax_bf16')
    return (idx, mx) if want_max else idx


SCORE_OUTPUTS = ('idx', 'max_logit', 'lse', 'target_logit', 'entropy')


def _score_want(want, target):
    want = tuple(want)
    if not want or any(w not in SCORE_OUTPUTS for w in want):
        raise ValueError(f'want: a non-empty subset of {SCORE_OUTPUTS} expected, got {want}')
    if 'target_logit' in want and target is None:
        raise ValueError("want 'target_logit': target expected")
    return want


def _score_outputs(want, rows, dev, target):
    if target is not None:
        _chk(target, torch.int32, 'target')
        if target.numel() != rows or not target.is_contiguous():
            raise ValueError(f'target: {rows} contiguous int32 expected, got {tuple(target.shape)}')
    return {w: torch.empty(rows, dtype=torch.int64 if w == 'idx' else torch.float32, device=dev) for w in want}


def lmhead_score_supported(K, N):
    return K in (128, 768) and N % 128 == 0


def lmhead_score_bf16(h, w_packed_bf16, M, K, N, target=None, want=SCORE_OUTPUTS):
    want = _score_want(want, target)
    h16 = h.dtype == torch.bfloat16
    _chk(h, torch.bfloat16 if h16 else torch.float32, 'h')
    out = _score_outputs(want, M, h.device, target)
    check(_lib.load().vf_lmhead_score_bf16(_p(h), 1 if h16 else 0, h.stride(0), _p(_chk(w_packed_bf16, torch.bfloat16, 'w_packed')), M, K, N,
                                           _p(target), *(_p(out.get(w)) for w in SCORE_OUTPUTS), _stream()), 'vf_lmhead_score_bf16')
    return out


def logits_score(logits, rows, N, target=None, want=SCORE_OUTPUTS, ld=None):
    want = _score_want(want, target)
    _f32(logits, 'logits')
    out = _score_outputs(want, rows, logits.device, target)
    check(_lib.load().vf_logits_score_f32(_p(logits), rows, N, N if ld is None else ld, _p(target), *(_p(out.get(w)) for w in SCORE_OUTPUTS),
                                          _stream()), 'vf_logits_score_f32')
    return out


def score_views(stats, target, views, L):
    dev = target.device
    tlp, conf = (torch.empty(views * L, dtype=torch.float32, device=dev) for _ in range(2))
    ll, acc = (torch.empty(views, dtype=torch.float32, device=dev) for _ in range(2))
    check(_lib.load().vf_score_views_f32(_p(_f32(stats['target_logit'])), _p(_f32(stats['lse'])), _p(_f32(stats['max_logit'])),
                                         _p(_chk(stats['idx'], torch.int64, 'idx')), _p(_chk(target, torch.int32, 'target')), views, L,
                                         _p(tlp), _p(conf), _p(ll), _p(acc), _stream()), 'vf_score_views_f32')
    return tlp, conf, ll, acc


SAMPLE_OUTPUTS = ('idx', 'logp', 'kept', 'thr')


def sample_rows(logits, rows, N, temperature=1.0, top_k=0, top_p=1.0, seed=0, row_id=None, n_samples=1, ld=None, want=('idx', 'logp')):
    want = tuple(want)
    if not want or any(w not in SAMPLE_OUTPUTS for w in want):
        raise ValueError(f'want: a non-empty subset of {SAMPLE_OUTPUTS} expected, got {want}')
    _f32(logits, 'logits')
    S = int(n_samples)
    ldv = N if ld is None else int(ld)
    if rows < 0 or N < 1 or ldv < N or not logits.is_contiguous() or logits.numel() < (rows - 1) * ldv + N * (rows > 0):
        raise ValueError(f'logits: {rows} contiguous rows of {N} with ld {ldv} expected, got {tuple(logits.shape)}')
    if row_id is not None:
        _chk(row_id, torch.int64, 'row_id')
        if row_id.numel() != rows or not row_id.is_contiguous():
            raise ValueError(f'row_id: {rows} contiguous int64 expected, got {tuple(row_id.shape)}')
    dev = logits.device
    shapes = dict(idx=((rows, max(S, 0)), torch.int64), logp=((rows, max(S, 0)), torch.float32), kept=((rows,), torch.int32),
                  thr=((rows,), torch.float32))
    out = {w: torch.empty(shapes[w][0], dtype=shapes[w][1], device=dev) for w in SAMPLE_OUTPUTS if w == 'idx' or w in want}
    check(_lib.load().vf_sample_rows_f32(_p(logits), rows, N, N if ld is None else ld, float(temperature), int(top_k), float(top_p),
                                         int(seed) & 0xFFFFFFFF, _p(row_id), S, *(_p(out.get(w)) for w in SAMPLE_OUTPUTS), _stream()),
          'vf_sample_rows_f32')
    return {w: out[w] for w in want}


def sample_views(logp, views, L, n_samples):
    _f32(logp, 'logp')
    S = int(n_samples)
    if logp.numel() != views * L * S or not logp.is_contiguous():
        raise ValueError(f'logp: contiguous [{views * L}, {S}] expected, got {tuple(logp.shape)}')
    ll = torch.empty((views, S), dtype=torch.float32, device=logp.device)
    check(_lib.load().vf_sample_views_f32(_p(logp), views, L, S, _p(ll), _stream()), 'vf_sample_views_f32')
    return ll


def postprocess_u8(x):
    x = _f32(x).contiguous()
    out = torch.empty(x.shape, dtype=torch.uint8, device=x.device)
    check(_lib.load().vf_postprocess_u8(_p(x), _p(out), x.numel(), _stream()), 'vf_postprocess_u8')
    return out


def resize_u8(images, image_size, method=None):
    if method not in (None, 'nearest', 'bilinear'):
        raise ValueError("method must be None, 'nearest' or 'bilinear'")
    n, H, W, C = images.shape
    if W == image_size or H == image_size:
        return images
    if method is None:
        method = 'nearest' if image_size > H else 'bilinear'
    src = _chk(images.contiguous(), torch.uint8, 'images')
    out = torch.empty((n, image_size, image_size, C), dtype=torch.uint8, device=images.device)
    check(_lib.load().vf_resize_u8(_p(src), _p(out), n, H, W, image_size, image_size, C, 1 if method == 'bilinear' else 0, _stream()),
          'vf_resize_u8')
    return out


def image_metrics_u8(a, b):
    if a.shape != b.shape or a.dim() != 4:
        raise ValueError(f'image_metrics_u8: two [n,H,W,C] batches of one shape expected, got {tuple(a.shape)} and {tuple(b.shape)}')
    a = _chk(a, torch.uint8, 'a').contiguous()
    b = _chk(b, torch.uint8, 'b').contiguous()
    n, H, W, C = a.shape
    if n == 0:
        return torch.empty((0, 2), dtype=torch.int64, device=a.device), torch.empty(0, dtype=torch.float64, device=a.device)
    lib = _lib.load()
    ws =torch.empty(max(int(lib.vf_image_metrics_workspace_bytes(n, H, W, C)), 8), dtype=torch.uint8, device=a.device)
    sums = torch.empty((n, 2), dtype=torch.int64, device=a.device)
    ssim = torch.empty(n, dtype=torch.float64, device=a.device)
    check(lib.vf_image_metrics_u8(_p(a), _p(b), n, H, W, C, _p(sums), _p(ssim), _p(ws), _stream()), 'vf_image_metrics_u8')
    return sums, ssim


def camera_knn(db, queries, k, pos_weight=0.3, return_dist=False):
    if db.dim() != 2 or db.shape[1] != 7 or queries.dim() != 2 or queries.shape[1] != 7:
        raise ValueError(f'camera_knn: db [N,7] and queries [Q,7] expected, got {tuple(db.shape)} and {tuple(queries.shape)}')
    db = _f32(db, 'db').contiguous()
    queries = _f32(queries, 'queries').contiguous()
    N, Q, k = db.shape[0], queries.shape[0], int(k)
    idx = torch.empty((Q, k), dtype=torch.int32, device=db.device)
    dist = torch.empty((Q, k), dtype=torch.float32, device=db.device) if return_dist else None
    lib = _lib.load()
    ws = torch.empty(max(int(lib.vf_camera_knn_workspace_bytes(N, Q, k)), 8), dtype=torch.uint8, device=db.device)
    check(lib.vf_camera_knn_f32(_p(db), N, _p(queries), Q, k, float(pos_weight), _p(idx), _p(dist), _p(ws), _stream()), 'vf_camera_knn_f32')
    return (idx, dist) if return_dist else idx


def pose_tail_supported(K, L):
    return K % 4 == 0 and 4 <= K <= 2048 and 1 <= L <= 256


def pose_tail(x, W, b, position_multiplier, views, L, want_raw=False, want_tokens=False):
    if x.dim() != 2 or x.shape[0] != views * L or x.stride(1) != 1 or W.dim() != 2 or tuple(W.shape) != (x.shape[1], 7):
        raise ValueError(f'pose_tail: x [views*L = {views * L}, K] with unit column stride and W [K,7] expected, got {tuple(x.shape)} '
                         f'(strides {tuple(x.stride())}) and {tuple(W.shape)}')
    if b is not None and b.numel() != 7:
        raise ValueError(f'pose_tail: b [7] expected, got {tuple(b.shape)}')
    K = x.shape[1]
    W = _f32(W, 'W').contiguous()
    b = _f32(b, 'b').contiguous() if b is not None else None
    dev = x.device
    cameras = torch.empty((views, 7), dtype=torch.float32, device=dev)
    tokens = torch.empty((views, L, 7), dtype=torch.float32, device=dev) if want_tokens else None
    raw = torch.empty((views, L, 7), dtype=torch.float32, device=dev) if want_raw else None
    check(_lib.load().vf_pose_tail_f32(_p(_f32(x, 'x')), x.stride(0) if views * L > 1 else max(x.stride(0), K), _p(W), _p(b),
                                       float(position_multiplier), views, L, K, _p(raw), _p(tokens), _p(cameras), _stream()), 'vf_pose_tail_f32')
    return cameras, tokens, raw
```

Baseline: 1160.

## Add small-M bf16 GEMM kernel and latency-form pair conv for undersubscribed launches

Adds a new 64-row-tile bf16 GEMM kernel with a 4-deep LDS ring. It is chosen automatically when a 256-tile grid would fill only a small fraction of the CUs. It also adds a latency form of the paired x3h conv: it splits each block's output channels across two blocks and uses deeper buffering when the grid has no more than half as many blocks as CUs. Both target small-batch decode shapes where few blocks leave most of the GPU idle, at the cost of more blocks re-reading the A operand. Plan/query entry points and Python wrappers are added for inspection.

After: 1159. About the same (-0.1%).

```diff
diff --git a/include/vf_hip.h b/include/vf_hip.h
--- a/include/vf_hip.h
+++ b/include/vf_hip.h
@@ -160,6 +160,8 @@
 } vf_pack_desc;
 int vf_gemm_bf16_pack_multi(const vf_pack_desc* descs_device, int n, void* stream);
 int vf_gemm_bf16(const vf_igemm_args* args , void* stream);
+int vf_gemm_bf16_small(const vf_igemm_args* args , void* stream);
+int vf_gemm_bf16_plan(const vf_igemm_args* args );
 size_t vf_conv3_bf16_packed_elems(int Cin, int Cout);
 int vf_conv3_bf16_pack(const float* w_oihw, void* dst, int Cin, int Cout, void* stream);
 int vf_conv3_halo_bf16(const vf_igemm_args* args , void* stream);
@@ -171,6 +173,8 @@
 size_t vf_conv3_x3h_packed_elems(int Cin, int Cout);
 int vf_conv3_x3h_pack(const float* w_oihw, void* dst, int Cin, int Cout, void* stream);
 int vf_conv3_halo_x3h(const vf_igemm_args* args , void* stream);
+int vf_conv3_halo_x3h_form(const vf_igemm_args* args , int form, void* stream);
+int vf_conv3_halo_x3h_plan(const vf_igemm_args* args );
 size_t vf_gemm_x3h_packed_elems(int K, int N);
 int vf_gemm_x3h_pack(const float* src, void* dst, int K, int N, int64_t sk, int64_t sn, void* stream);
 int vf_gemm_x3h(const vf_igemm_args* args , void* stream);
diff --git a/viewformer_amd/_lib.py b/viewformer_amd/_lib.py
--- a/viewformer_amd/_lib.py
+++ b/viewformer_amd/_lib.py
@@ -125,6 +125,8 @@
     'vf_gemm_bf16_pack': (c_int, [P, P, c_int, c_int, c_int64, c_int64, c_int, c_int64, P]),
     'vf_gemm_bf16_pack_multi': (c_int, [P, c_int, P]),
     'vf_gemm_bf16': (c_int, [POINTER(VfIgemmArgs), P]),
+    'vf_gemm_bf16_small': (c_int, [POINTER(VfIgemmArgs), P]),
+    'vf_gemm_bf16_plan': (c_int, [POINTER(VfIgemmArgs)]),
     'vf_conv3_bf16_packed_elems': (c_size_t, [c_int, c_int]),
     'vf_conv3_bf16_pack': (c_int, [P, P, c_int, c_int, P]),
     'vf_conv3_halo_bf16': (c_int, [POINTER(VfIgemmArgs), P]),
@@ -134,6 +136,8 @@
     'vf_conv3_x3h_packed_elems': (c_size_t, [c_int, c_int]),
     'vf_conv3_x3h_pack': (c_int, [P, P, c_int, c_int, P]),
     'vf_conv3_halo_x3h': (c_int, [POINTER(VfIgemmArgs), P]),
+    'vf_conv3_halo_x3h_form': (c_int, [POINTER(VfIgemmArgs), c_int, P]),
+    'vf_conv3_halo_x3h_plan': (c_int, [POINTER(VfIgemmArgs)]),
     'vf_gemm_x3h_packed_elems': (c_size_t, [c_int, c_int]),
     'vf_gemm_x3h_pack': (c_int, [P, P, c_int, c_int, c_int64, c_int64, P]),
     'vf_gemm_x3h': (c_int, [POINTER(VfIgemmArgs), P]),
diff --git a/viewformer_amd/csrc/conv3_halo_x3h.hip b/viewformer_amd/csrc/conv3_halo_x3h.hip
--- a/viewformer_amd/csrc/conv3_halo_x3h.hip
+++ b/viewformer_amd/csrc/conv3_halo_x3h.hip
@@ -34,22 +34,24 @@
     l = (_Float16)((x - (float)h) * 2048.f);
 }
 
-template <bool UP2, bool PRO, bool SWISH, bool PAIR = false>
-__global__ __launch_bounds__(256, 2) void conv3_halo_x3h_kernel(vf_igemm_args p) {
+template <bool UP2, bool PRO, bool SWISH, bool PAIR = false, int BD = 2, int WM = 1>
+__global__ __launch_bounds__(256, BD == 2 ? 2 : 1) void conv3_halo_x3h_kernel(vf_igemm_args p) {
+    static_assert(WM == 1 || WM == 2, "waves along the tile's pixel rows");
     using G = Geo<UP2, PAIR>;
     extern __shared__ __attribute__((aligned(16))) unsigned char smem_h[];
 
     const int tid = threadIdx.x;
     const int lane = tid & 63;
     const int wave = __builtin_amdgcn_readfirstlane(tid >> 6);
-    constexpr int MI = 4, NJ = 1;
-    const int wave_m = 0, wave_n = wave;
+    constexpr int MI = 4 / WM, NJ = 1;
+    const int wave_m = WM == 1 ? 0 : wave >> 1, wave_n = WM == 1 ? wave : wave & 1;
     const int half = lane >> 5, l31 = lane & 31;
 
     const int nb = p.Cout / BN;
     const int tilesX = p.Wout / TW, tilesY = p.Hout / TH;
     int bid = (int)vf_xcd_bid();
-    const int nblk = bid % nb; bid /= nb;
+    const int nblk_w = bid % (nb * WM); bid /= nb * WM;
+    const int nblk = nblk_w / WM, wblk = nblk_w % WM;
     int tx = 0, ty = 0, img;
     if (PAIR) { img = bid * 2; }
     else { tx = bid % tilesX; bid /= tilesX; ty = bid % tilesY; img = bid / tilesY; }
@@ -133,8 +135,8 @@
 
     const unsigned char* __restrict__ Wb = reinterpret_cast<const unsigned char*>(p.w_packed) + (size_t)nblk * TAP_BYTES;
     const size_t tap_stride = (size_t)nb * TAP_BYTES;
-    const int b_lane = (half * BN + wave_n * (32 * NJ) + l31) * 16;
-    constexpr int BD = 2, RING = BD + 1;
+    const int b_lane = (half * BN + (wblk * (4 / WM) + wave_n) * (32 * NJ) + l31) * 16;
+    constexpr int RING = BD + 1;
     static_assert(18 % RING == 0, "ring indices must repeat per chunk");
     f16x8 bring[RING][2][NJ];
     f16x8 aring[2][MI][2];
@@ -214,8 +216,10 @@
         for (int j = 0; j < NJ; ++j)
 #pragma unroll
             for (int r = 0; r < 16; ++r) acc[i][j][r] = __builtin_fmaf(accx[i][j][r], 4.8828125e-4f, acc[i][j][r]) * inv_s;
-    vf_halo_epilogue_t<PAIR, MI, NJ>(p, acc, img, img1, y0, x0, PAIR ? 0 : (ty * tilesX + tx) * 2, nblk, wave_m, wave_n, half, l31);
-}
+    vf_halo_epilogue_t<PAIR, MI, NJ>(p, acc, img, img1, y0, x0, PAIR ? 0 : (ty * tilesX + tx) * 2, nblk, wave_m, wblk * (4 / WM) + wave_n, half, l31);
+}
+
+constexpr int LAT_BD = 5, LAT_WM = 2;
 
 
 constexpr int S2_PH = 2 * TH + 1, S2_PW = 2 * TW + 1;
@@ -659,14 +663,16 @@
     }
 }
 
-template <bool UP2, bool PRO, bool SWISH, bool PAIR>
+template <bool UP2, bool PRO, bool SWISH, bool PAIR, bool LATENCY = false>
 int launch_halo(const vf_igemm_args& a, hipStream_t stream) {
     using G = Geo<UP2, PAIR>;
     const size_t smem = (size_t)2 * G::BUF;
     const int n_img = a.M / (a.Hout * a.Wout);
-    const long long blocks = PAIR ? (long long)((n_img + 1) / 2) * (a.Cout / BN)
+    const long long blocks = PAIR ? (long long)((n_img + 1) / 2) * (a.Cout / BN) * (LATENCY ? LAT_WM : 1)
                                   : (long long)n_img * (a.Hout / TH) * (a.Wout / TW) * (a.Cout / BN);
-    hipLaunchKernelGGL((conv3_halo_x3h_kernel<UP2, PRO, SWISH, PAIR>), dim3((unsigned)blocks), dim3(256), smem, stream, a);
+    static_assert(!LATENCY || (PAIR && !UP2), "the latency form: pair tiles only");
+    if constexpr (LATENCY) hipLaunchKernelGGL((conv3_halo_x3h_kernel<UP2, PRO, SWISH, PAIR, LAT_BD, LAT_WM>), dim3((unsigned)blocks), dim3(256), smem, stream, a);
+    else hipLaunchKernelGGL((conv3_halo_x3h_kernel<UP2, PRO, SWISH, PAIR>), dim3((unsigned)blocks), dim3(256), smem, stream, a);
     return vf_last_status();
 }
 
@@ -688,8 +694,17 @@
     return vf_last_status();
 }
 
+static int x3h_pair_form(const vf_igemm_args& a) {
+    const long long blocks = (long long)((a.M / 64 + 1) / 2) * (a.Cout / BN);
+    return blocks * 2 <= vf_device_cus() ? 1 : 0;
+}
+
 template <bool UP2, bool PAIR>
-int dispatch_pro(const vf_igemm_args& a, hipStream_t s) {
+int dispatch_pro(const vf_igemm_args& a, hipStream_t s, int form = 0) {
+    if (PAIR && form == 1) {
+        if (!a.pro_mean) return launch_halo<false, false, false, true, true>(a, s);
+        return a.pro_swish ? launch_halo<false, true, true, true, true>(a, s) : launch_halo<false, true, false, true, true>(a, s);
+    }
     if (!UP2 && !PAIR && (a.Cin / CK) % 2 == 0 && (!a.gn_part || a.Cout / 32 <= 16) && vf_x3h16_lds_bytes(a.pro_mean ? a.Cin : 0) <= 80 * 1024 &&
         vf_selected(VF_SEL_CONV_X3H_K32)) {
         if (!a.pro_mean) return launch_halo16<false, false>(a, s);
@@ -723,9 +738,26 @@
     return vf_last_status();
 }
 
+static int x3h_route(const vf_igemm_args& a, void* stream, int form, bool plan_only);
+
 int vf_conv3_halo_x3h(const vf_igemm_args* args, void* stream) {
     if (!args) return VF_ERR_BAD_ARG;
-    const vf_igemm_args& a = *args;
+    return x3h_route(*args, stream, -1, false);
+}
+
+int vf_conv3_halo_x3h_form(const vf_igemm_args* args, int form, void* stream) {
+    if (!args || (form != 0 && form != 1)) return VF_ERR_BAD_ARG;
+    return x3h_route(*args, stream, form, false);
+}
+
+int vf_conv3_halo_x3h_plan(const vf_igemm_args* args) {
+    if (!args) return VF_ERR_BAD_ARG;
+    return x3h_route(*args, nullptr, -1, true);
+}
+
+}
+
+static int x3h_route(const vf_igemm_args& a, void* stream, int form, bool plan_only) {
     if (!a.x || !a.w_packed || !a.out || a.M <= 0) return VF_ERR_BAD_ARG;
     if (a.drop_rate != 0.f || a.out_aux) return VF_ERR_UNSUPPORTED;
     if (a.mode == VF_MODE_CONV3_S2PAD) {
@@ -735,6 +767,8 @@
         if (a.batch > 1 || a.epilogue != VF_EPI_NONE || a.ldc < a.Cout || (a.res && a.ldr < a.Cout)) return VF_ERR_BAD_ARG;
         if ((long long)a.Hin * a.Win * a.Cin >= (1ll << 31)) return VF_ERR_UNSUPPORTED;
         if (int st = vf_halo_gn_check(a)) return st;
+        if (form == 1) return VF_ERR_UNSUPPORTED;
+        if (plan_only) return 0;
         if (p8) {
             const long long blocks = (long long)((a.M / 64 + 1) / 2) * (a.Cout / BN);
             hipLaunchKernelGGL(conv3_s2_x3h_kernel<true>, dim3((unsigned)blocks), dim3(256), (size_t)(S2_PH * 34 + 1) * S2_LDB, (hipStream_t)stream, a);
@@ -755,8 +789,9 @@
     if ((long long)a.Hin * a.Win * a.Cin >= (1ll << 31)) return VF_ERR_UNSUPPORTED;
     if (int st = vf_halo_gn_check(a)) return st;
     hipStream_t s = (hipStream_t)stream;
-    if (pair) return dispatch_pro<false, true>(a, s);
+    if (form >= 1 && !pair) return VF_ERR_UNSUPPORTED;
+    if (pair && form < 0) form = x3h_pair_form(a);
+    if (plan_only) return pair ? form : 0;
+    if (pair) return dispatch_pro<false, true>(a, s, form);
     return (a.mode == VF_MODE_CONV3_UP2) ? dispatch_pro<true, false>(a, s) : dispatch_pro<false, false>(a, s);
 }
-
-}
diff --git a/viewformer_amd/csrc/gemm_bf16.hip b/viewformer_amd/csrc/gemm_bf16.hip
--- a/viewformer_amd/csrc/gemm_bf16.hip
+++ b/viewformer_amd/csrc/gemm_bf16.hip
@@ -388,7 +388,11 @@
 
 }
 
-int vf_gemm_bf16_g256_launch(const vf_igemm_args& a, hipStream_t stream);
+int vf_gemm_bf16_g256_launch(const vf_igemm_args& a, hipStream_t stream, bool plan_only = false);
+int vf_gemm_bf16_small_launch(const vf_igemm_args& a, int tn, hipStream_t stream);
+bool vf_gemm_bf16_small_preferred(const vf_igemm_args& a);
+
+static int gemm_bf16_route(const vf_igemm_args& a, void* stream, bool plan_only);
 
 extern "C" {
 
@@ -416,7 +420,17 @@
 
 int vf_gemm_bf16(const vf_igemm_args* args, void* stream) {
     if (!args) return VF_ERR_BAD_ARG;
-    const vf_igemm_args& a = *args;
+    return gemm_bf16_route(*args, stream, false);
+}
+
+int vf_gemm_bf16_plan(const vf_igemm_args* args) {
+    if (!args) return VF_ERR_BAD_ARG;
+    return gemm_bf16_route(*args, nullptr, true);
+}
+
+}
+
+static int gemm_bf16_route(const vf_igemm_args& a, void* stream, bool plan_only) {
     if (!a.x || !a.w_packed || !a.out || a.M <= 0 || a.Cin <= 0 || a.Cout <= 0) return VF_ERR_BAD_ARG;
     if (a.gn_part) return VF_ERR_UNSUPPORTED;
     if (a.mode != VF_MODE_GEMM || a.pro_mean) return VF_ERR_UNSUPPORTED;
@@ -426,16 +440,17 @@
     if (a.lda < a.Cin || (a.lda & 3) || a.ldc < a.Cout || (a.res && a.ldr < a.Cout)) return VF_ERR_BAD_ARG;
     if (a.epilogue == VF_EPI_GELU_DUAL) {
         if (!(a.reserved0 & 1) || a.batch > 1 || a.Cin % (2 * CK) != 0) return VF_ERR_UNSUPPORTED;
-        const int rc = vf_gemm_bf16_g256_launch(a, (hipStream_t)stream);
-        return rc;
+        const int rc = vf_gemm_bf16_g256_launch(a, (hipStream_t)stream, plan_only);
+        return (plan_only && rc == VF_OK) ? 1 : rc;
     }
     if (a.drop_rate != 0.f) {
         if (!(a.reserved0 & 1) || (a.reserved0 & 2) || a.batch > 1 || a.Cin % (2 * CK) != 0) return VF_ERR_UNSUPPORTED;
-        return vf_gemm_bf16_g256_launch(a, (hipStream_t)stream);
+        const int rc = vf_gemm_bf16_g256_launch(a, (hipStream_t)stream, plan_only);
+        return (plan_only && rc == VF_OK) ? 1 : rc;
     }
     const size_t smem = (size_t)2 * (A_BYTES + B_BYTES);
     static unsigned long long attr_devs = 0;
-    if (vf_attr_needed(&attr_devs)) {
+    if (!plan_only && vf_attr_needed(&attr_devs)) {
         hipError_t e = hipFuncSetAttribute(reinterpret_cast<const void*>(gemm_bf16_kernel),
                                            hipFuncAttributeMaxDynamicSharedMemorySize, (int)smem);
         if (e != hipSuccess) return (int)e;
@@ -449,12 +464,15 @@
         if (a.epilogue == VF_EPI_GELU_BWD && !(o16 && a.res && a.ldr >= a.Cout)) return VF_ERR_BAD_ARG;
         if (a.reserved0 & 4) {
             if (a.epilogue != VF_EPI_GELU_BWD) return VF_ERR_BAD_ARG;
-            return vf_gemm_bf16_g256_launch(a, (hipStream_t)stream);
+            const int rc = vf_gemm_bf16_g256_launch(a, (hipStream_t)stream, plan_only);
+            return (plan_only && rc == VF_OK) ? 1 : rc;
         }
         if (vf_selected(VF_SEL_GEMM_G256)) {
-            const int rc = vf_gemm_bf16_g256_launch(a, (hipStream_t)stream);
-            if (rc != VF_ERR_UNSUPPORTED) return rc;
-        }
+            if (vf_gemm_bf16_small_preferred(a)) return plan_only ? 2 : vf_gemm_bf16_small_launch(a, 0, (hipStream_t)stream);
+            const int rc = vf_gemm_bf16_g256_launch(a, (hipStream_t)stream, plan_only);
+            if (rc != VF_ERR_UNSUPPORTED) return (plan_only && rc == VF_OK) ? 1 : rc;
+        }
+        if (plan_only) return 0;
         const dim3 g((unsigned)(mt * nb));
         hipStream_t st = (hipStream_t)stream;
         if (a16 && o16) hipLaunchKernelGGL((gemm_bf16_direct_kernel<true, true>), g, dim3(256), (size_t)2 * A_BYTES, st, a);
@@ -462,6 +480,7 @@
         else hipLaunchKernelGGL((gemm_bf16_direct_kernel<false, true>), g, dim3(256), (size_t)2 * A_BYTES, st, a);
         return vf_last_status();
     }
+    if (plan_only) return 0;
     if (a.Cin % (2 * CK) == 0 && a.batch <= 1) {
         hipLaunchKernelGGL((gemm_bf16_direct_kernel<false, false>), dim3((unsigned)(mt * nb)), dim3(256), (size_t)2 * A_BYTES, (hipStream_t)stream, a);
         return vf_last_status();
@@ -470,5 +489,3 @@
     hipLaunchKernelGGL(gemm_bf16_kernel, grid, dim3(256), smem, (hipStream_t)stream, a);
     return vf_last_status();
 }
-
-}
diff --git a/viewformer_amd/csrc/gemm_bf16_g256.hip b/viewformer_amd/csrc/gemm_bf16_g256.hip
--- a/viewformer_amd/csrc/gemm_bf16_g256.hip
+++ b/viewformer_amd/csrc/gemm_bf16_g256.hip
@@ -344,7 +344,7 @@
     return none;
 }
 
-int vf_gemm_bf16_g256_launch(const vf_igemm_args& a, hipStream_t stream) {
+int vf_gemm_bf16_g256_launch(const vf_igemm_args& a, hipStream_t stream, bool plan_only) {
     const bool a16 = a.reserved0 & 1, o16 = a.reserved0 & 2;
     if (!a16 || a.batch > 1 || a.Cout % GN != 0 || a.Cin % GK != 0 || a.M < GM || (a.lda & 7)) return VF_ERR_UNSUPPORTED;
     if (o16 && ((a.res && a.epilogue != VF_EPI_GELU_BWD) || (a.ldc & 1))) return VF_ERR_UNSUPPORTED;
@@ -359,6 +359,7 @@
                                (((unsigned long long)a.M + (unsigned long long)a.drop_row0 + 3) / 4) * (unsigned long long)a.Cout >= (1ull << 32)))
         return VF_ERR_UNSUPPORTED;
     if ((size_t)a.M * a.lda * 2 >= (1ull << 31) || (size_t)a.Cin * a.Cout * 2 >= (1ull << 31)) return VF_ERR_UNSUPPORTED;
+    if (plan_only) return VF_OK;
     const int mt = (a.M + GM - 1) / GM, nb = a.Cout / GN;
     const G256Tail t = g256_tail_policy(a.M, nb);
     const dim3 g((unsigned)(t.f_rows ? (t.f_rows + t.h_rows) * nb : mt * nb));
diff --git a/viewformer_amd/csrc/gemm_bf16_small.hip b/viewformer_amd/csrc/gemm_bf16_small.hip
--- /dev/null
+++ b/viewformer_amd/csrc/gemm_bf16_small.hip
@@ -0,0 +1,211 @@
+#include "vf_common.h"
+#include "epilogue.h"
+#include "../../include/vf_hip.h"
+
+namespace {
+
+typedef __bf16 bf16x8 __attribute__((ext_vector_type(8)));
+typedef __bf16 bf16x2_t __attribute__((ext_vector_type(2)));
+
+constexpr int SM = 64, SK = 64, SRING = 4;
+constexpr int SA_BYTES = SM * SK * 2;
+static_assert((SRING & (SRING - 1)) == 0, "ring slots are indexed by s & (SRING - 1)");
+
+__device__ __forceinline__ void bufds16(__amdgpu_buffer_rsrc_t r, void* l, unsigned voff, unsigned soff) {
+    __builtin_amdgcn_raw_ptr_buffer_load_lds(r, (__attribute__((address_space(3))) void*)l, 16, voff, soff, 0, 0);
+}
+
+template <int N>
+__device__ __forceinline__ void small_wait() {
+    static_assert(N >= 0 && N <= 63, "vmcnt is a 6-bit count");
+    asm volatile("s_waitcnt vmcnt(%0) lgkmcnt(0)" :: "n"(N) : "memory");
+}
+template <int PER, int MAXL>
+__device__ __forceinline__ void small_wait_later(int later) {
+    if constexpr (MAXL == 0) small_wait<0>();
+    else {
+        if (later >= MAXL) small_wait<MAXL * PER>();
+        else small_wait_later<PER, MAXL - 1>(later);
+    }
+}
+
+template <int TN, bool O16>
+__global__ __launch_bounds__(256, TN == 64 ? 2 : 1) void gemm_bf16_small_kernel(vf_igemm_args p) {
+    extern __shared__ __attribute__((aligned(16))) unsigned char smem_b[];
+    constexpr int NJ = TN / 64;
+    constexpr int SW_BYTES = TN * SK * 2;
+    constexpr int SSTAGE = SA_BYTES + SW_BYTES;
+    constexpr int PER = 2 + 2 * NJ;
+
+    const int tid = threadIdx.x;
+    const int lane = tid & 63;
+    const int wave = __builtin_amdgcn_readfirstlane(tid >> 6);
+    const int wave_m = wave >> 1, wave_n = wave & 1;
+    const int half = lane >> 5, l31 = lane & 31;
+
+    const int mt = (p.M + SM - 1) / SM;
+    const unsigned lbid = vf_xcd_bid();
+    const int mtile = (int)(lbid % (unsigned)mt), nblk = (int)(lbid / (unsigned)mt);
+    const int m_tile0 = mtile * SM, n_tile0 = nblk * TN;
+    const int nstages = p.Cin / SK;
+
+    const __amdgpu_buffer_rsrc_t a_rsrc = __builtin_amdgcn_make_buffer_rsrc(const_cast<float*>(p.x), 0, 0x7fffffff, 0x00020000);
+    const __amdgpu_buffer_rsrc_t w_rsrc = __builtin_amdgcn_make_buffer_rsrc(const_cast<float*>(p.w_packed), 0, 0x7fffffff, 0x00020000);
+    unsigned avoff[2];
+#pragma unroll
+    for (int q = 0; q < 2; ++q) {
+        const int r = wave * 16 + q * 8 + (lane >> 3);
+        const int c = (lane & 7) ^ ((r >> 1) & 7);
+        int m = m_tile0 + r;
+        m = m < p.M ? m : p.M - 1;
+        avoff[q] = (unsigned)(((size_t)m * p.lda) * 2 + c * 16);
+    }
+    unsigned wvoff[2 * NJ];
+#pragma unroll
+    for (int q = 0; q < 2 * NJ; ++q) {
+        if (TN == 128) wvoff[q] = (unsigned)((size_t)nblk * 16384 + wave * 4096 + q * 1024 + lane * 16);
+        else wvoff[q] = (unsigned)((size_t)(nblk >> 1) * 16384 + (wave * 2 + q) * 2048 + (nblk & 1) * 1024 + lane * 16);
+    }
+    const unsigned w_stage_stride = (unsigned)(p.Cout / 128) * 16384u;
+    auto issue = [&](int s) {
+        unsigned char* dst = smem_b + (s & (SRING - 1)) * SSTAGE;
+#pragma unroll
+        for (int q = 0; q < 2; ++q) bufds16(a_rsrc, dst + (wave * 16 + q * 8) * 128, avoff[q], (unsigned)(s * (SK * 2)));
+#pragma unroll
+        for (int q = 0; q < 2 * NJ; ++q) bufds16(w_rsrc, dst + SA_BYTES + (wave * 2 * NJ + q) * 1024, wvoff[q], (unsigned)s * w_stage_stride);
+    };
+
+    const unsigned a_row_off = (unsigned)((wave_m * 32 + l31) * 128);
+    const unsigned a_swz = (unsigned)((l31 >> 1) & 7);
+    unsigned a_off[4];
+#pragma unroll
+    for (int ks = 0; ks < 4; ++ks) a_off[ks] = a_row_off + ((((unsigned)(ks * 2 + half)) ^ a_swz) << 4);
+    const unsigned b_off = (unsigned)(SA_BYTES + (half * TN + wave_n * (TN / 2) + l31) * 16);
+
+    f32x16 acc[NJ];
+#pragma unroll
+    for (int j = 0; j < NJ; ++j)
+#pragma unroll
+        for (int r = 0; r < 16; ++r) acc[j][r] = 0.f;
+
+#pragma unroll
+    for (int s = 0; s < SRING - 1; ++s)
+        if (s < nstages) issue(s);
+    for (int s = 0; s < nstages; ++s) {
+        small_wait_later<PER, SRING - 2>(nstages - 1 - s);
+        __builtin_amdgcn_s_barrier();
+        if (s + SRING - 1 < nstages) issue(s + SRING - 1);
+        const unsigned char* buf = smem_b + (s & (SRING - 1)) * SSTAGE;
+        bf16x8 a[4], b[4][NJ];
+#pragma unroll
+        for (int ks = 0; ks < 4; ++ks) {
+            a[ks] = *reinterpret_cast<const bf16x8*>(buf + a_off[ks]);
+#pragma unroll
+            for (int j = 0; j < NJ; ++j) b[ks][j] = *reinterpret_cast<const bf16x8*>(buf + b_off + (ks * 2 * TN + j * 32) * 16);
+        }
+#pragma unroll
+        for (int ks = 0; ks < 4; ++ks)
+#pragma unroll
+            for (int j = 0; j < NJ; ++j) acc[j] = __builtin_amdgcn_mfma_f32_32x32x16_bf16(a[ks], b[ks][j], acc[j], 0, 0, 0);
+    }
+
+    const int m0 = m_tile0 + wave_m * 32 + 4 * half;
+    const bool gelu = p.epilogue == VF_EPI_GELU_ERF;
+    if constexpr (O16) {
+        __bf16* __restrict__ O = reinterpret_cast<__bf16*>(p.out);
+        const int odd = l31 & 1;
+#pragma unroll
+        for (int j = 0; j < NJ; ++j) {
+            const int n = n_tile0 + wave_n * (TN / 2) + j * 32 + l31;
+            const float bias = p.bias ? p.bias[n] : 0.f;
+            float t[16];
+#pragma unroll
+            for (int r = 0; r < 16; ++r) {
+                t[r] = acc[j][r] + bias;
+                if (gelu) t[r] = vf_gelu_erf_fast(t[r]);
+            }
+#pragma unroll
+            for (int r = 0; r < 16; r += 2) {
+                const float give = odd ? t[r] : t[r + 1];
+                const float got = vf_lane_xor1(give);
+                const int m = m0 + ((r + odd) & 3) + 8 * ((r + odd) >> 2);
+                bf16x2_t v;
+                v[0] = (__bf16)(odd ? got : t[r]);
+                v[1] = (__bf16)(odd ? t[r + 1] : got);
+                if (m < p.M) *reinterpret_cast<bf16x2_t*>(O + (size_t)m * p.ldc + (n - odd)) = v;
+            }
+        }
+    } else {
+        const bool full = m_tile0 + SM <= p.M;
+        const long long ldc = p.ldc, ldr = p.ldr;
+        const int rows_left = p.M - m0;
+#pragma unroll
+        for (int j = 0; j < NJ; ++j) {
+            const int n = n_tile0 + wave_n * (TN / 2) + j * 32 + l31;
+            const float bias = p.bias ? p.bias[n] : 0.f;
+            float* o = p.out + (size_t)(rows_left > 0 ? m0 : 0) * ldc + n;
+            const float* rs = p.res ? p.res + (size_t)(rows_left > 0 ? m0 : 0) * ldr + n : nullptr;
+            if (full) {
+                auto oo = [&](int r) { return (long long)((r & 3) + 8 * (r >> 2)) * ldc; };
+                auto ro = [&](int r) { return (long long)((r & 3) + 8 * (r >> 2)) * ldr; };
+                if (rs) vf_store_tile<0, true>(acc[j], bias, o, rs, oo, ro);
+                else vf_store_tile<0, false>(acc[j], bias, o, rs, oo, ro);
+            } else {
+                if (rs) vf_store_tile_ragged<0, true>(acc[j], bias, o, rs, ldc, ldr, rows_left);
+                else vf_store_tile_ragged<0, false>(acc[j], bias, o, rs, ldc, ldr, rows_left);
+            }
+        }
+    }
+}
+
+bool small_supported(const vf_igemm_args& a) {
+    const bool a16 = a.reserved0 & 1, o16 = a.reserved0 & 2;
+    if (a.mode != VF_MODE_GEMM || a.pro_mean || a.gn_part || a.out_aux || a.drop_rate != 0.f || a.batch > 1) return false;
+    if (!a16 || (a.reserved0 & ~3) || a.M < 1 || a.Cin < 128 || a.Cin % 128 != 0 || a.Cout < 128 || a.Cout % 128 != 0) return false;
+    if (a.lda < a.Cin || (a.lda & 7) || a.ldc < a.Cout || (a.res && a.ldr < a.Cout)) return false;
+    if (o16 ? (a.res != nullptr || (a.ldc & 1) || (a.epilogue != VF_EPI_NONE && a.epilogue != VF_EPI_GELU_ERF)) : a.epilogue != VF_EPI_NONE) return false;
+    if ((size_t)a.M * a.lda * 2 >= (1ull << 31) || (size_t)a.Cin * a.Cout * 2 >= (1ull << 31)) return false;
+    return true;
+}
+
+template <int TN, bool O16>
+int small_launch(const vf_igemm_args& a, hipStream_t stream) {
+    constexpr size_t smem = (size_t)SRING * (SA_BYTES + TN * SK * 2);
+    static unsigned long long devs = 0;
+    if (vf_attr_needed(&devs)) {
+        const hipError_t e = hipFuncSetAttribute(reinterpret_cast<const void*>(gemm_bf16_small_kernel<TN, O16>), hipFuncAttributeMaxDynamicSharedMemorySize, (int)smem);
+        if (e != hipSuccess) return (int)e;
+        vf_attr_done(&devs);
+    }
+    const unsigned g = (unsigned)((a.M + SM - 1) / SM) * (unsigned)(a.Cout / TN);
+    hipLaunchKernelGGL((gemm_bf16_small_kernel<TN, O16>), dim3(g), dim3(256), smem, stream, a);
+    return vf_last_status();
+}
+
+int small_tile_n(const vf_igemm_args& a) { return (long long)a.M * a.Cin * 2 > (8ll << 20) ? 128 : 64; }
+
+}
+
+int vf_gemm_bf16_small_launch(const vf_igemm_args& a, int tn, hipStream_t stream) {
+    if (!small_supported(a)) return VF_ERR_UNSUPPORTED;
+    const bool o16 = a.reserved0 & 2;
+    if (tn == 0) tn = small_tile_n(a);
+    if (tn == 64) return o16 ? small_launch<64, true>(a, stream) : small_launch<64, false>(a, stream);
+    if (tn == 128) return o16 ? small_launch<128, true>(a, stream) : small_launch<128, false>(a, stream);
+    return VF_ERR_BAD_ARG;
+}
+
+bool vf_gemm_bf16_small_preferred(const vf_igemm_args& a) {
+    if (!small_supported(a)) return false;
+    const long long t256 = (long long)((a.M + 255) / 256) * ((a.Cout + 255) / 256);
+    return t256 * 8 <= (long long)vf_device_cus() * 3;
+}
+
+extern "C" int vf_gemm_bf16_small(const vf_igemm_args* args, void* stream) {
+    if (!args) return VF_ERR_BAD_ARG;
+    if (!args->x || !args->w_packed || !args->out) return VF_ERR_BAD_ARG;
+    vf_igemm_args a = *args;
+    const int tn = (a.reserved0 >> 8) & 0xff;
+    a.reserved0 &= 0xff;
+    return vf_gemm_bf16_small_launch(a, tn, (hipStream_t)stream);
+}
diff --git a/viewformer_amd/csrc/vf_common.h b/viewformer_amd/csrc/vf_common.h
--- a/viewformer_amd/csrc/vf_common.h
+++ b/viewformer_amd/csrc/vf_common.h
@@ -25,6 +25,17 @@
     int d = 0;
     (void)hipGetDevice(&d);
     __atomic_fetch_or(mask, 1ull << (d & 63), __ATOMIC_RELAXED);
+}
+
+static inline int vf_device_cus() {
+    static int cached[64];
+    int d = 0;
+    if (hipGetDevice(&d) != hipSuccess) { (void)hipGetLastError(); return 256; }
+    int v = __atomic_load_n(&cached[d & 63], __ATOMIC_RELAXED);
+    if (v > 0) return v;
+    if (hipDeviceGetAttribute(&v, hipDeviceAttributeMultiprocessorCount, d) != hipSuccess || v <= 0) { (void)hipGetLastError(); return 256; }
+    __atomic_store_n(&cached[d & 63], v, __ATOMIC_RELAXED);
+    return v;
 }
 
 __device__ __forceinline__ float vf_swish(float v) {
diff --git a/viewformer_amd/ops.py b/viewformer_amd/ops.py
--- a/viewformer_amd/ops.py
+++ b/viewformer_amd/ops.py
@@ -256,7 +256,7 @@
 def igemm(x, w_packed, M, Cin, Cout, out, bias=None, res=None, mode=MODE_GEMM, epilogue=EPI_NONE,
           pro=None, pro_swish=False, pro_rows_per_img=0, Hin=0, Win=0, Hout=0, Wout=0,
           lda=None, ldc=None, ldr=None, batch=1, stride_x=0, stride_w=0, stride_out=0, stride_res=0, bf16=False, x6=False, gn_part=None, split_k=0,
-          x3h=False, a16=False, o16=False, out_aux=None, res16=False, drop=None, gelu_grad=False):
+          x3h=False, a16=False, o16=False, out_aux=None, res16=False, drop=None, gelu_grad=False, _entry=None):
     lib = _lib.load()
     if not 0 <= M < 2 ** 31 or max(Cin, Cout, Hin, Win, Hout, Wout, batch) >= 2 ** 31:
         raise _lib.VfError(f'igemm: M = {M} rows do not fit the int32 fields of vf_igemm_args — split the launch '
@@ -319,6 +319,12 @@
     for t in ((None if a16 else x), (None if o16 else out), bias, (None if (res16 or conv16) else res)):
         if t is not None:
             _f32(t)
+    if _entry is not None:
+        name, flags, extra = _entry
+        _chk(w_packed, torch.float16 if x3h else torch.bfloat16, 'w_packed')
+        a.reserved0 |= flags
+        check(getattr(lib, name)(ctypes.byref(a), *extra, _stream()), name)
+        return out
     if x3h:
         _chk(w_packed, torch.float16, 'w_packed')
         if mode == MODE_GEMM:
@@ -343,6 +349,39 @@
     _f32(w_packed)
     check(lib.vf_igemm_f32(ctypes.byref(a), _stream()), 'vf_igemm_f32')
     return out
+
+
+def gemm_bf16_small(x, w_packed, M, Cin, Cout, out, bias=None, res=None, epilogue=EPI_NONE, lda=None, ldc=None, ldr=None, tile_n=0):
+    return igemm(x, w_packed, M, Cin, Cout, out, bias=bias, res=res, epilogue=epilogue, lda=lda, ldc=ldc, ldr=ldr, bf16=True, a16=True,
+                 o16=out.dtype == torch.bfloat16, _entry=('vf_gemm_bf16_small', int(tile_n) << 8, ()))
+
+
+def conv3_halo_x3h_form(x, w_packed, M, Cin, Cout, out, form, **kw):
+    return igemm(x, w_packed, M, Cin, Cout, out, x3h=True, _entry=('vf_conv3_halo_x3h_form', 0, (int(form),)), **kw)
+
+
+def _plan_args(M, Cin, Cout, mode, epilogue, lda, ldc, ldr, has_res):
+    a = VfIgemmArgs()
+    a.x = a.w_packed = a.out = 256
+    a.res = 256 if has_res else None
+    a.mode, a.epilogue, a.M, a.Cin, a.Cout, a.batch = mode, epilogue, M, Cin, Cout, 1
+    a.lda, a.ldc, a.ldr = (Cin if lda is None else lda), (Cout if ldc is None else ldc), (Cout if ldr is None else ldr)
+    return a
+
+
+def gemm_bf16_plan(M, Cin, Cout, epilogue=EPI_NONE, a16=True, o16=False, has_res=False, lda=None, ldc=None, ldr=None):
+    a = _plan_args(M, Cin, Cout, MODE_GEMM, epilogue, lda, ldc, ldr, has_res)
+    a.reserved0 = (1 if a16 else 0) | (2 if o16 else 0)
+    if epilogue == EPI_GELU_DUAL:
+        a.out_aux = 256
+    return int(_lib.load().vf_gemm_bf16_plan(ctypes.byref(a)))
+
+
+def conv3_halo_x3h_plan(n_img, H, W, Cin, Cout, mode=MODE_CONV3_S1):
+    a = _plan_args(n_img * H * W, Cin, Cout, mode, EPI_NONE, None, None, None, False)
+    a.Hout, a.Wout = H, W
+    a.Hin, a.Win = (H // 2, W // 2) if mode == MODE_CONV3_UP2 else (H * 2, W * 2) if mode == MODE_CONV3_S2PAD else (H, W)
+    return int(_lib.load().vf_conv3_halo_x3h_plan(ctypes.byref(a)))
 
 
 def conv3_small_cout_supported(mode, Cin, Cout, H, W):
```
